# seobbro/TTA-depth-completion

Measured on AMD Instinct MI355X. Metric: TTA frames/sec (fwd+loss+bwd+Adam) at 352x1216, higher is better.
Workload: dtype mixed: real frames' forward (the scored depth) f32 storage + bf16x3 MFMA arithmetic; no_grad proxy pass and all data gradients bf16 storage + single bf16 MFMA; fp32 accumulate everywhere; loss / Adam / adapted parameters fp32 (include/ptta.h PTTA_DTYPE_MIXED)

## Files before the change

include/ptta.h:

```cpp
#ifndef PTTA_H
#define PTTA_H
#include <stdint.h>
#ifdef __cplusplus
extern "C" {
#endif

typedef struct ptta_ctx* ptta_handle;
typedef void* ptta_stream;

enum { PTTA_BACKBONE_MSG_CHN = 0, PTTA_BACKBONE_NLSPN = 1, PTTA_BACKBONE_COSTDCNET = 2 };
enum { PTTA_DTYPE_F32 = 0, PTTA_DTYPE_MIXED = 1,
       PTTA_MIXED_KEEP_PROXY = 0x100, PTTA_MIXED_KEEP_BACKWARD = 0x200, PTTA_MIXED_KEEP_HEADS = 0x400,
       PTTA_MIXED_BWD_ROUNDED_W = 0x800 };
enum { PTTA_META_1LAYER = 0, PTTA_META_2LAYERS = 1, PTTA_META_NONE = 2 };
enum { PTTA_NLSPN_LEGACY_OFFSET = 0x100,
       PTTA_NLSPN_SYNCBN_ADAPT = 0x200,
       PTTA_SYNCBN_ADAPT = 0x200,
       PTTA_ADAPT_META_ONLY = 0x400 };

typedef struct {
    float lr, beta1, beta2, eps, weight_decay;
    float w_sparse_depth, w_smoothness, w_cos;
    float max_input_depth;
    float max_predict_depth;
// ... 47 lines not shown
              const float* validity, float* depth_out, float* loss_info_out, ptta_stream s);

int ptta_outlier_removal(const float* sparse_depth, const float* validity, float* sparse_out, float* validity_out,
                         int n, int height, int width, int kernel_size, float threshold, float* scratch, ptta_stream s);

int ptta_eval_metrics(const float* depth, const float* ground_truth, int64_t numel, float min_evaluate_depth,
                      float max_evaluate_depth, void* scratch, float* metrics_out, ptta_stream s);

int ptta_mdconv_forward(const float* input, const float* weight, const float* bias, const float* offset, const float* mask,
                        float* output, int b, int c, int h, int w, int c_out, int kh, int kw, int sh, int sw, int ph, int pw,
                        int dh, int dw, int group, int deformable_group, ptta_stream s);
int ptta_mdconv_backward(const float* input, const float* weight, const float* bias, const float* offset, const float* mask,
                         const float* grad_output, float* grad_input, float* grad_offset, float* grad_mask, float* grad_weight,
                         float* grad_bias, int b, int c, int h, int w, int c_out, int kh, int kw, int sh, int sw, int ph, int pw,
                         int dh, int dw, int group, int deformable_group, ptta_stream s);

int ptta_set_image_norm(ptta_handle h, float divisor, const float* mean, const float* stdv);

int ptta_head_bind(ptta_handle h, const char* name, float* param, float* exp_avg, float* exp_avg_sq);
int ptta_head_set_hparams(ptta_handle h, float lr, float beta1, float beta2, float eps, float weight_decay, float tau,
                          int adam_step, ptta_stream s);
int ptta_head_reload(ptta_handle h, ptta_stream s);
int ptta_head_forward(ptta_handle h, const float* image, const float* sparse_depth, int reverse, float* emb_out, float* ref_out,
                      ptta_stream s);
int ptta_head_backward(ptta_handle h, float* loss_out, ptta_stream s);
int ptta_head_adam_step(ptta_handle h, ptta_stream s);
int ptta_head_step(ptta_handle h, const float* image, const float* sparse_depth, int reverse, float* loss_out, ptta_stream s);
int ptta_head_get_grad(ptta_handle h, const char* name, float* dst, int64_t capacity, int* has_grad_host, ptta_stream s);

enum { PTTA_HEAD_FORM_PLAIN = 0, PTTA_HEAD_FORM_SYNCBN = 1 };
int ptta_head_set_form(ptta_handle h, int form);

int ptta_crop_flip(const float* src, float* dst, int n, int channels, int height, int width, int crop_height, int crop_width,
                   const int32_t* start_y, const int32_t* start_x, const uint8_t* hflip, const uint8_t* vflip, ptta_stream s);

int ptta_rotate(const float* src, float* dst, int n, int channels, int height, int width, const uint8_t* do_rotate, const float* angle_deg,
                int bilinear, ptta_stream s);
int ptta_resize_crop(const float* src, float* dst, int n, int channels, int height, int width, const uint8_t* do_resize,
                     const int32_t* resize_height, const int32_t* resize_width, const int32_t* start_y, const int32_t* start_x,
                     int bilinear, int scale_depth, ptta_stream s);
int ptta_photometric(const float* src, float* dst, int n, int height, int width, const uint8_t* do_brightness, const float* f_brightness,
                     const uint8_t* do_contrast, const float* f_contrast, const uint8_t* do_saturation, const float* f_saturation,
                     double* scratch, ptta_stream s);

int ptta_photometric_full(const float* src, float* dst, int n, int height, int width, const uint8_t* do_brightness, const float* f_brightness,
                          const uint8_t* do_contrast, const float* f_contrast, const uint8_t* do_gamma, const float* f_gamma,
                          const uint8_t* do_hue, const float* f_hue, const uint8_t* do_saturation, const float* f_saturation,
                          double* scratch, ptta_stream s);
int ptta_add_noise(const float* src, const float* noise, float* dst, int n, int channels, int height, int width, const uint8_t* do_noise,
                   float spread, int uniform, ptta_stream s);
int ptta_remove_patches(const float* src, float* dst, int n, int channels, int height, int width, const uint8_t* do_remove,
                        const uint8_t* selected, const int32_t* patch_height, const int32_t* patch_width, ptta_stream s);
int ptta_crop_pad(const float* src, float* dst, int n, int channels, int height, int width, const uint8_t* do_crop_pad,
                  const int32_t* start_y, const int32_t* start_x, const int32_t* end_y, const int32_t* end_x,
                  const int32_t* pad_top, const int32_t* pad_left, int padding_mode, float fill, ptta_stream s);
int ptta_resize_pad(const float* src, float* dst, int n, int channels, int height, int width, const uint8_t* do_resize_pad,
                    const int32_t* resize_height, const int32_t* resize_width, const int32_t* pad_top, const int32_t* pad_left,
                    int bilinear, int padding_mode, float fill, ptta_stream s);

typedef int (*ptta_allreduce_fn)(void* user, double* exchange_buf, long long count, ptta_stream s);
int ptta_set_stat_sync(ptta_handle h, ptta_allreduce_fn fn, void* user, double* exchange_buf, int64_t capacity, int world_size);

int ptta_rccl_unique_id(void* id128_host);
int ptta_rccl_comm_create(const void* id128_host, int rank, int world_size, void** comm_out_host);
int ptta_rccl_comm_destroy(void* comm);
int ptta_rccl_allreduce_mean_f32(void* comm, float* buf, int64_t count, ptta_stream s);
const char* ptta_rccl_last_error(void);
int ptta_set_stat_sync_rccl(ptta_handle h, void* comm, double* exchange_buf, int64_t capacity, int world_size);
int ptta_set_grad_sync_rccl(ptta_handle h, void* comm);

int ptta_set_graph(ptta_handle h, int enable);

int ptta_set_option(ptta_handle h, const char* key, int value);
int ptta_get_option(ptta_handle h, const char* key, int* value_host);

int ptta_profile(ptta_handle h, int enable);
int ptta_profile_read(ptta_handle h, int klass, double* ms_total_host, double* alg_bytes_host, double* macs_host,
                      int64_t* launches_host, ptta_stream s);

int ptta_debug_tensor(ptta_handle h, const char* name, float* dst, int64_t capacity, int64_t* numel_host, ptta_stream s);
int ptta_op_conv32(const float* in_nhwc, const float* weight, const float* bias, float* out_nhwc,
                   int b, int hin, int win, int mode, int relu_in, int in_major, int flip, int dtype, int naive,
                   ptta_stream s);
int ptta_op_gwgrad(const float* x_nhwc, const float* gy_nhwc, float* gw, float* gb, int b, int h, int w, int ci, int co, int impl,
                   int reps, float* us_per_call_host, ptta_stream s);
#define PTTA_GCONV_S1 0
#define PTTA_GCONV_S2 1
#define PTTA_GCONV_T2 2
#define PTTA_GCONV_VERT 1
#define PTTA_GCONV_X1_W2 2
#define PTTA_GCONV_DGRAD 4
#define PTTA_GCONV_AFF_ACT_FIRST 8
#define PTTA_GCONV_AFF_RES_PLAIN 16
int ptta_op_gconv(const float* x0, int c0, int ld0, const float* x1, int c1, int ld1, const float* weight, const float* bias, float* y,
                  int co, int ldy, int b, int hin, int win, int hout, int wout, int k, int geom, int act, int accumulate, int impl,
                  int flags, int six_b, int x1_from_b, int stat_npass, double* stat_host, int* form_host, ptta_stream s);
int ptta_op_gconv_affine(const float* x0, int c0, int ld0, const float* x1, int c1, int ld1, const float* weight, const float* bias, float* y,
                         int co, int ldy, int b, int hin, int win, int hout, int wout, int k, int geom, int act, int accumulate, int impl,
                         int flags, int six_b, int x1_from_b, int stat_npass, double* stat_host, int* form_host, const float* scale,
                         const float* shift, const float* res, int ld_res, ptta_stream s);
#define PTTA_GBN_TRAIN 0
#define PTTA_GBN_EVAL 1
#define PTTA_GBN_BACKWARD 2
typedef struct ptta_gbn_view { float* p; int c; int ld; } ptta_gbn_view;
typedef struct ptta_gbn_args {
    int mode, b, h, w, npass, act, act_first, res_relu, acc_gx, acc_gres, world, nblocks_in, repeats;
    float eps, momentum;
    ptta_gbn_view x, res, y, g, gx, gres;
    const float* gamma; const float* beta; const float* part_in;
    float* st; float* rm; float* rv; long long* nbt; float* st_eval; float* dgamma; float* dbeta;
} ptta_gbn_args;
int ptta_op_gbn(const ptta_gbn_args* a, ptta_stream s);
typedef struct ptta_cd_sparse ptta_cd_sparse;
int ptta_cd_sparse_create(ptta_cd_sparse** out, int n, int h, int w);
void ptta_cd_sparse_destroy(ptta_cd_sparse* q);
int ptta_cd_sparse_build(ptta_cd_sparse* q, const float* sparse, float z_step, ptta_stream s);
int ptta_cd_sparse_read(ptta_cd_sparse* q, int level, int* cnt_host, int* coords_host, long long coords_cap, int* vol_host, float* feat_in_host,
                        ptta_stream s);
int ptta_op_cd_sparse_conv(ptta_cd_sparse* q, const float* x, const float* wk, float* y, int lin, int lout, int ksize, int ci, int co, int backward,
                           int acc, ptta_stream s);
typedef struct ptta_cd_sbn_args {
    int mode, level, c, relu, repeats, world, acc_res;
    const float* f; const float* res; const float* y; const float* g; const float* gamma; const float* beta;
    float* rm; float* rv; long long* nbt; float* out; float* st; float* dgamma; float* dbeta; float* gx; float* gres;
} ptta_cd_sbn_args;
int ptta_op_cd_sbn(ptta_cd_sparse* q, const ptta_cd_sbn_args* a, ptta_stream s);
int ptta_op_cd_densify(ptta_cd_sparse* q, const float* in, float* out, int c, int backward, int ldv, int c0, ptta_stream s);
#define PTTA_CD_PAD_DUAL 0
#define PTTA_CD_CROP_AVG 1
#define PTTA_CD_SCATTER_DUAL_GRAD 2
#define PTTA_CD_STAGE 3
#define PTTA_CD_CLAMP 4
#define PTTA_CD_FUSION_FWD 5
#define PTTA_CD_FUSION_BWD 6
#define PTTA_CD_POOL_FWD 7
#define PTTA_CD_POOL_BWD 8
#define PTTA_CD_UP_FWD 9
#define PTTA_CD_UP_BWD 10
#define PTTA_CD_REGRESS_FWD 11
#define PTTA_CD_REGRESS_BWD 12
#define PTTA_CD_ROWS_FWD 13
#define PTTA_CD_ROWS_BWD 14
int ptta_op_cd_dense(int op, const float* a, const float* b, float* out, float* out2, const int* d, const float* f, ptta_stream s);
int ptta_op_conv32_chain(const float* in_nhwc, const float* weight, const float* bias, float* buf_a, float* buf_b, const float* aux,
                         int b, int h, int w, int relu_in, int epi_flags, int reps, int replays, float* us_per_launch_host, ptta_stream s);
#define PTTA_ABI_VERSION 2
int ptta_version(void);

#ifdef __cplusplus
}
#endif
#endif
```

tta-depth-completion_amd/csrc/conv32.hip:

```cpp
#include <cstdlib>
#include <cstring>
#include "ptta_common.h"
#include "ptta_kernels.h"

template <typename T>
struct Conv32P {
    const T* in; int in_nb;
    const void* wpack;
    const void* wpack2;
    Epi<T> epi;
    int B, Hin, Win, Hout, Wout;
};

template <typename T> struct Frag;
template <> struct Frag<float> { typedef float4 A; };
template <> struct Frag<bf16_t> { typedef uint4 A; };

__device__ __forceinline__ float4 relu4(float4 v) {
    v.x = fmaxf(v.x, 0.f); v.y = fmaxf(v.y, 0.f); v.z = fmaxf(v.z, 0.f); v.w = fmaxf(v.w, 0.f);
    return v;
}
__device__ __forceinline__ unsigned relu_bf2(unsigned v) {
    unsigned neg = (v >> 15) & 0x00010001u;
    return v & ~(neg * 0xffffu);
}
__device__ __forceinline__ uint4 relu8(uint4 v) {
    v.x = relu_bf2(v.x); v.y = relu_bf2(v.y); v.z = relu_bf2(v.z); v.w = relu_bf2(v.w);
    return v;
}

template <typename T, int MODE, bool RELU, bool UP, bool MASK, bool ADD>
__global__ __launch_bounds__(256) void conv32_mfma_kernel(Conv32P<T> p) {
    constexpr bool F32 = sizeof(T) == 4;
    constexpr int NA = F32 ? 4 : 2;
    typedef typename Frag<T>::A AF;
    const int lane = threadIdx.x & 63;
    const int i = lane & 31, h = lane >> 5;
    const float biasv = epi_bias(p.epi, i);
    const int wave = __builtin_amdgcn_readfirstlane((int)(threadIdx.x >> 6));

    AF w[9][NA];
    {
        const AF* wp = (const AF*)p.wpack;
#pragma unroll
        for (int t = 0; t < 9; ++t)
#pragma unroll
            for (int g = 0; g < NA; ++g) w[t][g] = wp[(t * NA + g) * 64 + lane];
    }

    const int Wt = (MODE == CONV_T2) ? p.Win : p.Wout;
    const int nseg = (Wt + 31) >> 5;
    const int npar = (MODE == CONV_T2) ? 2 : 1;
    const long nitems = (long)p.B * nseg * npar * p.Hout;
    const float sy = up_scale(p.Hout >> 1, p.Hout), sx = up_scale(p.Wout >> 1, p.Wout);

    for (long item = (long)blockIdx.x * 4 + wave; item < nitems; item += (long)gridDim.x * 4) {
        long t_ = item;
        const int y = (int)(t_ % p.Hout); t_ /= p.Hout;
        int xpar = 0;
        if (MODE == CONV_T2) { xpar = (int)(t_ & 1); t_ >>= 1; }
        const int seg = (int)(t_ % nseg);
        const int b = (int)(t_ / nseg);
        const int x0 = seg << 5;
        const bool lane_in = (x0 + i) < Wt;
        const T* inb = p.in + (size_t)(b % p.in_nb) * p.Hin * p.Win * 32;

        f32x16 acc;
#pragma unroll
        for (int r = 0; r < 16; ++r) acc[r] = 0.f;

#pragma unroll
        for (int tap = 0; tap < 9; ++tap) {
            const int ky = tap / 3, kx = tap % 3;
            bool active = true;
            int yi, xi;
            if (MODE == CONV_S1) { yi = y + ky - 1; xi = x0 + i + kx - 1; }
            else if (MODE == CONV_S2) { yi = 2 * y + ky - 1; xi = 2 * (x0 + i) + kx - 1; }
            else {
                const int ty = y + 1 - ky, tx = xpar + 1 - kx;
                active = ((ty & 1) == 0) && ((tx & 1) == 0);
                yi = ty >> 1; xi = x0 + i + (tx >> 1);
            }
            active = active && (yi >= 0) && (yi < p.Hin);
            if (!active) continue;
            const bool ok = lane_in && (xi >= 0) && (xi < p.Win);
            const T* src = inb + ((size_t)yi * p.Win + (ok ? xi : 0)) * 32;
            AF a[NA];
#pragma unroll
            for (int g = 0; g < NA; ++g) {
                if (F32) {
                    float4 v = make_float4(0.f, 0.f, 0.f, 0.f);
                    if (ok) v = *(const float4*)((const float*)src + 8 * g + 4 * h);
                    if (RELU) v = relu4(v);
                    a[g] = *(AF*)&v;
                } else {
                    uint4 v = make_uint4(0, 0, 0, 0);
                    if (ok) v = *(const uint4*)((const bf16_t*)src + 16 * g + 8 * h);
                    if (RELU) v = relu8(v);
                    a[g] = *(AF*)&v;
                }
            }
#pragma unroll
            for (int g = 0; g < NA; ++g) {
                if (F32) {
                    const float4 av = *(float4*)&a[g];
                    const float4 wv = *(float4*)&w[tap][g];
                    acc = __builtin_amdgcn_mfma_f32_32x32x2f32(av.x, wv.x, acc, 0, 0, 0);
                    acc = __builtin_amdgcn_mfma_f32_32x32x2f32(av.y, wv.y, acc, 0, 0, 0);
                    acc = __builtin_amdgcn_mfma_f32_32x32x2f32(av.z, wv.z, acc, 0, 0, 0);
                    acc = __builtin_amdgcn_mfma_f32_32x32x2f32(av.w, wv.w, acc, 0, 0, 0);
                } else {
                    acc = __builtin_amdgcn_mfma_f32_32x32x16_bf16(__builtin_bit_cast(bf16x8, a[g]),
                                                                  __builtin_bit_cast(bf16x8, w[tap][g]),
                                                                  acc, 0, 0, 0);
                }
            }
        }

        epi_tile<T, UP, MASK, ADD>(p.epi, b, y, p.Hout, p.Wout, i, acc, x0, h, Wt, MODE == CONV_T2 ? 2 : 1, xpar, sy, sx, nullptr, 0, 0, &biasv);
    }
}


#define X3_TH 8
#define X3_PW 34
#define X3_PH 10

typedef __bf16 bf16x2_t __attribute__((ext_vector_type(2)));
typedef float float2_t __attribute__((ext_vector_type(2)));
typedef short short2_t __attribute__((ext_vector_type(2)));

__device__ __forceinline__ void split2(float a, float b, unsigned& hi, unsigned& lo) {
    float2_t v = {a, b};
    const bf16x2_t h = __builtin_convertvector(v, bf16x2_t);
    hi = __builtin_bit_cast(unsigned, h);
    float2_t r = {a - __uint_as_float(hi << 16), b - __uint_as_float(hi & 0xffff0000u)};
    lo = __builtin_bit_cast(unsigned, __builtin_convertvector(r, bf16x2_t));
}
__device__ __forceinline__ unsigned relu_pk(unsigned v) {
    const short2_t z = {0, 0};
    return __builtin_bit_cast(unsigned, __builtin_elementwise_max(__builtin_bit_cast(short2_t, v), z));
}

template <typename T> struct Px;
template <> struct Px<float> { float4 a, b; };
template <> struct Px<bf16_t> { uint4 a; };
template <typename T> __device__ __forceinline__ Px<T> px_zero();
template <> __device__ __forceinline__ Px<float> px_zero<float>() { Px<float> r; r.a = make_float4(0.f, 0.f, 0.f, 0.f); r.b = r.a; return r; }
template <> __device__ __forceinline__ Px<bf16_t> px_zero<bf16_t>() { Px<bf16_t> r; r.a = make_uint4(0u, 0u, 0u, 0u); return r; }
__device__ __forceinline__ Px<float> px_load(const float* src) { Px<float> r; r.a = *(const float4*)src; r.b = *(const float4*)(src + 4); return r; }
__device__ __forceinline__ Px<bf16_t> px_load(const bf16_t* src) { Px<bf16_t> r; r.a = *(const uint4*)src; return r; }
template <bool RELU>
__device__ __forceinline__ void px_stage(const Px<float>& v, unsigned char* dst, int lo_off) {
    float4 a0 = v.a, a1 = v.b;
#ifdef X3_TIMING_NOSPLIT
    *(float4*)dst = a0; *(float4*)(dst + lo_off) = a1; return;
#endif
    if (RELU) { a0 = relu4(a0); a1 = relu4(a1); }
    uint4 hi, lo;
    split2(a0.x, a0.y, hi.x, lo.x); split2(a0.z, a0.w, hi.y, lo.y);
    split2(a1.x, a1.y, hi.z, lo.z); split2(a1.z, a1.w, hi.w, lo.w);
    *(uint4*)dst = hi;
    *(uint4*)(dst + lo_off) = lo;
}
template <bool RELU>
__device__ __forceinline__ void px_stage(const Px<bf16_t>& v, unsigned char* dst, int) {
    uint4 hi = v.a;
    if (RELU) { hi.x = relu_pk(hi.x); hi.y = relu_pk(hi.y); hi.z = relu_pk(hi.z); hi.w = relu_pk(hi.w); }
    *(uint4*)dst = hi;
}
template <typename T> struct Geo;
template <> struct Geo<float> { static constexpr int STR = 144, LO = 64, WL = 18 * 64 * 16, UPPX = 128, UPPC = 8; };
template <> struct Geo<bf16_t> { static constexpr int STR = 80, LO = 0, WL = 0, UPPX = 64, UPPC = 4; };

__device__ __forceinline__ int x3_stage_pix(int idx) { return ((idx >> 5) << 3) + (((idx >> 2) & 1) << 2) + ((idx >> 3) & 3); }

template <typename T, bool W2 = false>
__device__ __forceinline__ void mma_step(f32x16& acc, const unsigned char* a, const uint4& wh, const unsigned char* wl) {
    const bf16x8 ah = __builtin_bit_cast(bf16x8, *(const uint4*)a);
    const bf16x8 bh = __builtin_bit_cast(bf16x8, wh);
    if constexpr (sizeof(T) == 2 && W2) {
        const bf16x8 bl = __builtin_bit_cast(bf16x8, *(const uint4*)wl);
        acc = __builtin_amdgcn_mfma_f32_32x32x16_bf16(ah, bl, acc, 0, 0, 0);
    }
    if constexpr (sizeof(T) == 4) {
        const bf16x8 al = __builtin_bit_cast(bf16x8, *(const uint4*)(a + Geo<T>::LO));
        const bf16x8 bl = __builtin_bit_cast(bf16x8, *(const uint4*)wl);
        acc = __builtin_amdgcn_mfma_f32_32x32x16_bf16(al, bh, acc, 0, 0, 0);
        acc = __builtin_amdgcn_mfma_f32_32x32x16_bf16(ah, bl, acc, 0, 0, 0);
    }
    acc = __builtin_amdgcn_mfma_f32_32x32x16_bf16(ah, bh, acc, 0, 0, 0);
}
template <typename T, bool W2 = false>
__device__ __forceinline__ void load_weights(uint4 (&wh)[9][2], unsigned char* wl_lds, const void* wpack, const void* wpack2, int tid, int lane) {
    const uint4* ph = (const uint4*)wpack;
#pragma unroll
    for (int t = 0; t < 9; ++t)
#pragma unroll
        for (int k = 0; k < 2; ++k) wh[t][k] = ph[(t * 2 + k) * 64 + lane];
    if constexpr (sizeof(T) == 4 || W2) {
        const uint4* pl = (const uint4*)wpack2;
        for (int idx = tid; idx < 18 * 64; idx += 256) *(uint4*)(wl_lds + idx * 16) = pl[idx];
    }
}

template <typename T, bool W2> struct FragSet { uint4 ah, al, bl; };
template <typename T, bool W2>
__device__ __forceinline__ void frag_load(FragSet<T, W2>& f, const unsigned char* a, const unsigned char* wl) {
    f.ah = *(const uint4*)a;
    if constexpr (sizeof(T) == 4) { f.al = *(const uint4*)(a + Geo<T>::LO); f.bl = *(const uint4*)wl; }
    else if constexpr (W2) f.bl = *(const uint4*)wl;
}
template <typename T, bool W2>
__device__ __forceinline__ void frag_mma(f32x16& acc, const FragSet<T, W2>& f, const uint4& wh) {
    const bf16x8 ah = __builtin_bit_cast(bf16x8, f.ah), bh = __builtin_bit_cast(bf16x8, wh);
    if constexpr (sizeof(T) == 2 && W2) acc = __builtin_amdgcn_mfma_f32_32x32x16_bf16(ah, __builtin_bit_cast(bf16x8, f.bl), acc, 0, 0, 0);
    if constexpr (sizeof(T) == 4) {
        acc = __builtin_amdgcn_mfma_f32_32x32x16_bf16(__builtin_bit_cast(bf16x8, f.al), bh, acc, 0, 0, 0);
        acc = __builtin_amdgcn_mfma_f32_32x32x16_bf16(ah, __builtin_bit_cast(bf16x8, f.bl), acc, 0, 0, 0);
    }
    acc = __builtin_amdgcn_mfma_f32_32x32x16_bf16(ah, bh, acc, 0, 0, 0);
}

template <typename T, int UPH, int UPW>
__device__ __forceinline__ void up_window_dma(const T* ub, int Hu, int Wu, int uy0, int ux0, unsigned char* up_lds, int tid, int wave) {
    constexpr int PC = Geo<T>::UPPC, N = UPH * UPW * PC;
#pragma unroll
    for (int k = 0; k < (N + 255) / 256; ++k) {
        const int idx = tid + 256 * k;
        if (idx < N) {
            const int q = idx % PC, pix = idx / PC;
            const int r = pix / UPW, cc = pix - r * UPW;
            const int gy = min(uy0 + r, Hu - 1), gx = min(ux0 + cc, Wu - 1);
            __builtin_amdgcn_global_load_lds((const __attribute__((address_space(1))) void*)(ub + ((size_t)gy * Wu + gx) * 32 + (32 / PC) * q),
                                             (__attribute__((address_space(3))) void*)(up_lds + (size_t)(256 * k + 64 * wave) * 16), 16, 0, 0);
        }
    }
}

#define X3STAMP(v) do { if constexpr (TIMING) { unsigned long long t_; asm volatile("s_memtime %0\n\ts_waitcnt lgkmcnt(0)" : "=s"(t_) :: "memory"); v = t_; } } while (0)
template <typename T, bool RELU, bool UP, bool MASK, bool ADD, bool W2 = false, bool TIMING = false>
__global__ __launch_bounds__(256, 2) void conv32_s1_x3_kernel(Conv32P<T> p) {
    unsigned long long T0 = 0, ta = 0, tb = 0, tc = 0, td = 0, te = 0, tf = 0, tg = 0, th = 0;
    unsigned long long dWait = 0, dSplit = 0, dIssue = 0, dBar1 = 0, dMfma = 0, dEpi = 0, dBar2 = 0, dPro = 0;
    int ntl = 0;
    X3STAMP(T0);
    constexpr int STR = Geo<T>::STR, WL = (sizeof(T) == 4 || W2) ? 18 * 64 * 16 : 0;
    constexpr int UPH = 6, UPW = 18;
    __shared__ __attribute__((aligned(16))) unsigned char lds[X3_PH * X3_PW * STR + WL + (UP ? UPH * UPW * Geo<T>::UPPX : 0)];
    unsigned char* const wl_lds = lds + X3_PH * X3_PW * STR;
    unsigned char* const up_lds = wl_lds + WL;
    const int tid = threadIdx.x, lane = tid & 63;
    const int i = lane & 31, h = lane >> 5;
    const float biasv = epi_bias(p.epi, i);
    const int wave = __builtin_amdgcn_readfirstlane(tid >> 6);
    const int H = p.Hout, W = p.Wout;
    const int ntx = (W + 31) >> 5, nty = (H + X3_TH - 1) / X3_TH;
    const long ntiles = (long)p.B * ntx * nty;
// ... 1070 lines not shown
```

tta-depth-completion_amd/csrc/msgchn_backward.hip:

```cpp
#include "msgchn_ctx.h"

using namespace msgchn;

namespace msgchn {

static int meta2_backward(ptta_ctx* c, hipStream_t s) {
    auto& m2 = c->m2;
    ptta_ctx::Adapted* A = c->adapted.data();
    const int H4 = c->H4, W4 = c->W4, Nn = c->Nn;
    const long P = (long)Nn * H4 * W4;
    if (m2.generic) {
        const int npass = 2;
        GView x; x.p = (float*)c->c2; x.B = Nn; x.H = H4; x.W = W4; x.C = 32; x.ld = 32;
        GView hv = x; hv.p = m2.gh; hv.C = 128; hv.ld = 128;
        GView av = hv; av.p = m2.ga1;
        GView tv = x; tv.p = m2.gt;
        GView gm = x; gm.p = c->nar_bwd ? c->dm_f32 : (float*)c->dm_total;
        GView dt = x; dt.p = m2.gdt;
        GView da1 = hv; da1.p = m2.gda1;
        GView dh = hv; dh.p = m2.gdh;
        RUN(ptta_launch_gbn_backward(tv, gm, tv, dt, GView(), npass, GACT_NONE, 0, 0, 0, A[5].p, m2.gst2, m2.gpart, m2.gbw, A[5].g, A[6].g, s, 0, &c->stat_sync));
        RUN(ptta_launch_gwgrad_mfma(av, dt, m2.wgp, A[3].g, A[4].g, s));
        GX3Args a;
        a.x0 = dt.p; a.C0 = 32; a.ld0 = 32; a.B = Nn; a.H = H4; a.W = W4;
// ... 26 lines not shown

int heads_backward(ptta_ctx* c, const float* gref, hipStream_t s) {
    const double esh = (c->nar_heads && heads_v2_on(c)) ? 2.0 : 4.0;
    ProfScope ps_(c, 6, s, (double)c->Rg * 32 * (c->nar_bwd ? 2 : 4) + ((double)c->Rg * (1024 + 512) + 16384.0 + 262144.0) * esh,
                  (double)c->Rg * (16384.0 + 262144.0), 3);
    const Lin& l0 = c->fc["proj.0"]; const Lin& l3 = c->fc["proj.3"]; BNorm& bn = c->bn["proj.1"];
    const int R = (int)c->Rg;
    if (c->nar_heads && heads_v2_on(c)) {
        HnGemmArgs g; g.epi = 3; g.R = R; g.W = l3.Wtsl;
        if (c->cos_in_gemm) { g.pro = 4; g.A = c->emb_n; g.Bref = c->ref_n; g.rowstats = c->loss_ws + ptta_loss_ws_rows_off(c->N); g.coef = c->loss_ws; }
        else { g.pro = 5; g.Af = gref; }
        g.X = c->feat; g.x_bf16 = 0; g.W0 = l0.Whi; g.W0t = l0.Wthi; g.b0 = l0.bias;
        g.escale = bn.scale; g.eshift = bn.shift; g.emean = bn.mean; g.einv = bn.inv; g.part = c->bn_part; g.P = c->headP;
        RUN(ptta_launch_hn_gemm(g, s));
        const int nb = ptta_hn_row_blocks(R);
        RUN(ptta_stat_sync(&c->stat_sync, c->bn_part, nb, 512, 1, s));
        RUN(ptta_launch_bn_bwd_finalize(c->bn_part, nb, R * (c->stat_sync.world > 1 ? c->stat_sync.world : 1), 512, bn.gamma, bn.inv, c->bnb_gscale, c->bnb_c1, c->bnb_c2, s,
                                        nullptr, nullptr, c->head_k12, l0.bias, bn.mean));
        RUN(ptta_launch_head_bwd_finish(c->head_k12, l0.W, c->headP, (const float*)c->feat, R, c->g_feat, s, 1, c->nar_bwd ? 1 : 0));
        return 0;
    }
    if (heads_v2_on(c)) {
        GemmArgs g; g.A = gref; g.W = l3.Wt; g.R = R; g.K = 512; g.N = 512; g.epi = 3;
        if (c->cos_in_gemm) {
            g.A = c->emb; g.Bref = c->ref; g.rowstats = c->loss_ws + ptta_loss_ws_rows_off(c->N); g.coef = c->loss_ws; g.pro = 4;
        }
        g.escale = bn.scale; g.eshift = bn.shift; g.emean = bn.mean; g.einv = bn.inv; g.part = c->bn_part;
        g.x3 = 1; g.Whi = l3.Wthi; g.Wlo = l3.Wtlo; g.Wil = l3.Wtil;
        g.X = (const float*)c->feat; g.b0 = l0.bias; g.W0hi = l0.Whi; g.W0lo = l0.Wlo; g.W0thi = l0.Wthi; g.W0tlo = l0.Wtlo; g.P = c->headP;
        RUN(ptta_launch_gemm(g, s));
        RUN(ptta_stat_sync(&c->stat_sync, c->bn_part, ptta_gemm_part_blocks(g), 512, 1, s));
        RUN(ptta_launch_bn_bwd_finalize(c->bn_part, ptta_gemm_part_blocks(g), R * (c->stat_sync.world > 1 ? c->stat_sync.world : 1), 512, bn.gamma, bn.inv, c->bnb_gscale, c->bnb_c1, c->bnb_c2, s,
                                        nullptr, nullptr, c->head_k12, l0.bias, bn.mean));
        RUN(ptta_launch_head_bwd_finish(c->head_k12, l0.W, c->headP, (const float*)c->feat, R, c->nar_bwd ? c->g_feat_f32 : (float*)c->g_feat, s));
        if (c->nar_bwd) RUN(to_narrow(c, c->g_feat_f32, c->g_feat, c->Rg * 32, s));
        return 0;
    }
    GemmArgs g; g.A = gref; g.W = l3.Wt; g.C = c->gmask; g.R = R; g.K = 512; g.N = 512; g.epi = 2;
    g.eH = c->h1; g.escale = bn.scale; g.eshift = bn.shift; g.emean = bn.mean; g.einv = bn.inv; g.part = c->bn_part;
    g.x3 = c->x3; g.Whi = l3.Wthi; g.Wlo = l3.Wtlo; g.Wil = l3.Wtil;
    RUN(ptta_launch_gemm(g, s));
    RUN(ptta_stat_sync(&c->stat_sync, c->bn_part, ptta_gemm_part_blocks(g), 512, 1, s));
    RUN(ptta_launch_bn_bwd_finalize(c->bn_part, ptta_gemm_part_blocks(g), R * (c->stat_sync.world > 1 ? c->stat_sync.world : 1), 512, bn.gamma, bn.inv, c->bnb_gscale, c->bnb_c1, c->bnb_c2, s));
    GemmArgs g2; g2.A = c->gmask; g2.A2 = c->h1; g2.W = l0.Wt; g2.C = (c->bf16 || c->nar_bwd) ? c->g_feat_f32 : (float*)c->g_feat; g2.R = R; g2.K = 512; g2.N = 32; g2.pro = 2;
    g2.pscale = c->bnb_gscale; g2.pmean = bn.mean; g2.pinv = bn.inv; g2.pc1 = c->bnb_c1; g2.pc2 = c->bnb_c2;
    g2.x3 = c->x3; g2.Whi = l0.Wthi; g2.Wlo = l0.Wtlo;
    RUN(ptta_launch_gemm(g2, s));
    if (c->bf16 || c->nar_bwd) from_f32_launch(c->g_feat_f32, (bf16_t*)c->g_feat, c->Rg * 32, s);
    return 0;
}

int backbone_backward(ptta_ctx* c, const float* g_net, hipStream_t s, bool join_aux) {
    const int Nn = c->Nn, B2 = 2 * Nn;
    const int nbf = c->nar_bwd ? 1 : c->bf16;
    const int H1 = c->Hp, W1 = c->Wp, H2 = c->H2, W2 = c->W2, H4 = c->H4, W4 = c->W4, H8 = c->H8, W8 = c->W8;
    auto out1_args = [&](const std::string& layer, const float* g, const void* mask, void* out, int H, int W) {
        const LOut& lo = c->lout[layer];
        ConvInArgs a; a.cin = 1; a.pl[0].p = g; a.pl[0].nb = Nn; a.pl[0].bstride = (long)H * W;
        a.wfrag = lo.bfrag; a.wcanon = lo.bcanon; a.mask = mask; a.mask_nb = B2; a.out_raw = out;
        a.B = Nn; a.H = H; a.W = W; a.bf16 = c->nar_bwd ? 1 : c->bf16; a.naive = c->naive;
        return a;
    };
    auto dgrad_out1 = [&](const std::string& layer, const float* g, const void* mask, void* out, int H, int W) -> int {
        ConvInArgs a = out1_args(layer, g, mask, out, H, W);
        return conv_in_p(c, a, s);
    };
    auto head_bwd = [&](const std::string& l3, const std::string& l1, const float* g, const void* v, void* dv, int H, int W, const E& e) -> int {
        ConvInArgs a = out1_args(l3, g, v, dv, H, W);
        return conv32_first_bwd(c, s, l1, a, Nn, H, W, e);
    };
    auto dgrad_in_ch1 = [&](const std::string& layer, const void* g, const float* add, float* out, int H, int W) -> int {
        const LIn& li = c->lin_in[layer];
        ConvOut1Args a; a.in = g; a.in_nb = Nn; a.w = li.bw; a.add = add; a.add_nb = Nn; a.out = out;
        a.B = Nn; a.H = H; a.W = W; a.relu_in = 0; a.bf16 = c->nar_bwd ? 1 : c->bf16;
        return conv_out1_p(c, a, s);
    };
    auto em = [](void* raw, const void* mask, int mask_nb) { E e; e.raw = raw; e.mask = mask; e.mask_nb = mask_nb; return e; };
    RUN(head_bwd("depth_decoder3.prdct.3", "depth_decoder3.prdct.1", g_net, c->v3, c->dv3, H1, W1, em(c->ds0_3, c->s0_3, Nn)));
    CV("depth_decoder3.dec1.3", true, CONV_S1, c->ds0_3, Nn, Nn, H1, W1, false, em(c->du3, c->u3, Nn));
    CV("depth_decoder3.dec1.1", true, CONV_S2, c->du3, Nn, Nn, H1, W1, false, em(c->ds1_3, c->s1_3, Nn));
    CV("depth_decoder3.dec2.3", true, CONV_S1, c->ds1_3, Nn, Nn, H2, W2, false, em(c->dt3, c->t3, Nn));
    if (join_aux) HIPCHK(hipStreamWaitEvent(s, c->ev_join, 0));
    { E e; e.raw = c->dw2; e.mask = c->w2; e.mask_nb = B2; e.sum = c->dfeat_tot; e.add1 = c->g_feat; e.add1_nb = Nn;
      CV("depth_decoder3.dec2.1", true, CONV_S2, c->dt3, Nn, Nn, H2, W2, false, e); }
    hipStream_t sd = join_aux ? c->aux(s) : nullptr;
    if (!sd) sd = s;
    CV("depth_encoder3.enc2.3", true, CONV_S1, c->dfeat_tot, Nn, Nn, H4, W4, false, em(c->de3_2a, c->e3_2a, B2));
    { E e; e.sum = c->de3_1; e.mask = c->e3_1; e.mask_nb = B2; e.add1 = c->ds1_3; e.add1_nb = Nn;
      CV("depth_encoder3.enc2.1", true, CONV_T2, c->de3_2a, Nn, Nn, H4, W4, false, e); }
    CV("depth_encoder3.enc1.3", true, CONV_S1, c->de3_1, Nn, Nn, H2, W2, false, em(c->de3_1a, c->e3_1a, B2));
    { E e; e.sum = c->de3_0; e.mask = c->e3_0; e.mask_nb = B2; e.add1 = c->ds0_3; e.add1_nb = Nn;
      CV("depth_encoder3.enc1.1", true, CONV_T2, c->de3_1a, Nn, Nn, H2, W2, false, e); }
    if (sd != s) { HIPCHK(hipEventRecord(c->ev_side[0], s)); HIPCHK(hipStreamWaitEvent(sd, c->ev_side[0], 0)); }
    REST_(sd, ptta_launch_up2T_32(c->de3_0, nullptr, c->up4_t, Nn, H2, W2, nbf, sd));
    REST_(sd, ptta_launch_up2T_32(c->de3_1, nullptr, c->up3_t, Nn, H4, W4, nbf, sd));
    REST_(sd, ptta_launch_up2T_32(c->dfeat_tot, nullptr, c->dz2_up, Nn, H8, W8, nbf, sd));
    if (sd != s) HIPCHK(hipEventRecord(c->ev_side[3], sd));
    if (c->loss_report.on) {
        REST_(sd, ptta_launch_loss_depth_part(final_depth(c), c->loss_report.image, c->loss_report.sparse, c->loss_report.validity, c->hp.max_input_depth,
                                              c->N, c->H, c->W, c->loss_ws, sd));
        REST_(sd, ptta_launch_loss_finalize(c->loss_ws, c->N, c->H, c->W, c->Rg, 1, c->hyper + 5, c->loss_info_dst ? c->loss_info_dst : c->loss_info, sd));
        HIPCHK(hipEventRecord(c->ev_loss, sd));
    }
    CV("depth_encoder3.init.2", true, CONV_S1, c->de3_0, Nn, Nn, H1, W1, false, em(c->de3_0a, c->e3_0a, B2));
    RUN(dgrad_in_ch1("depth_encoder3.init.0", c->de3_0a, g_net, c->dp11, H1, W1));
    REST_(s, ptta_launch_up2T_1ch(c->dp11, c->dq, Nn, H2, W2, s));
    if (sd != s) HIPCHK(hipStreamWaitEvent(s, c->ev_side[3], 0));
    { E e = em(c->ds0_2, c->s0_2, B2); e.sum = c->dz4; e.add1 = c->up4_t; e.add1_nb = Nn;
      RUN(head_bwd("depth_decoder2.prdct.3", "depth_decoder2.prdct.1", c->dq, c->v2, c->dv2, H2, W2, e)); }
    CV("depth_decoder2.dec1.3", true, CONV_S1, c->dz4, Nn, Nn, H2, W2, false, em(c->du2, c->u2, B2));
    { E e = em(c->ds1_2, c->s1_2, B2); e.sum = c->dz3; e.add1 = c->up3_t; e.add1_nb = Nn;
      CV("depth_decoder2.dec1.1", true, CONV_S2, c->du2, Nn, Nn, H2, W2, false, e); }
    CV("depth_decoder2.dec2.3", true, CONV_S1, c->dz3, Nn, Nn, H4, W4, false, em(c->dt2, c->t2, B2));
    { E e; e.sum = c->dz2; e.mask = c->z2; e.mask_nb = B2; e.add1 = c->dz2_up; e.add1_nb = Nn;
      CV("depth_decoder2.dec2.1", true, CONV_S2, c->dt2, Nn, Nn, H4, W4, false, e); }
    CV("depth_encoder2.enc2.3", true, CONV_S1, c->dz2, Nn, Nn, H8, W8, false, em(c->de2_2a, c->e2_2a, B2));
    { E e; e.sum = c->de2_1; e.mask = c->e2_1; e.mask_nb = B2; e.add1 = c->ds1_2; e.add1_nb = Nn;
      CV("depth_encoder2.enc2.1", true, CONV_T2, c->de2_2a, Nn, Nn, H8, W8, false, e); }
    CV("depth_encoder2.enc1.3", true, CONV_S1, c->de2_1, Nn, Nn, H4, W4, false, em(c->de2_1a, c->e2_1a, B2));
    { E e; e.sum = c->de2_0; e.mask = c->e2_0; e.mask_nb = B2; e.add1 = c->ds0_2; e.add1_nb = Nn;
      CV("depth_encoder2.enc1.1", true, CONV_T2, c->de2_1a, Nn, Nn, H4, W4, false, e); }
    CV("depth_encoder2.init.2", true, CONV_S1, c->de2_0, Nn, Nn, H2, W2, false, em(c->de2_0a, c->e2_0a, B2));
    RUN(dgrad_in_ch1("depth_encoder2.init.0", c->de2_0a, c->dq, c->dp12, H2, W2));
    REST_(s, ptta_launch_up2T_1ch(c->dp12, c->dout1, Nn, H4, W4, s));
    RUN(dgrad_out1("depth_decoder1.prdct.3", c->dout1, c->v1, c->dv1, H4, W4));
    { E e; e.sum = c->dm_total; e.mask = c->s0_1; e.mask_nb = B2; e.add1 = c->dw2; e.add1_nb = Nn; e.add2 = c->ds1_2; e.add2_nb = Nn;
      CV("depth_decoder1.prdct.1", true, CONV_S1, c->dv1, Nn, Nn, H4, W4, false, e); }
    if (sd != s && c->loss_report.on) HIPCHK(hipStreamWaitEvent(s, c->ev_loss, 0));
    if (c->nar_bwd && c->meta_mode == PTTA_META_2LAYERS) RUN(to_wide(c, c->dm_total, c->dm_f32, (long)Nn * H4 * W4 * 32, s));
    if (c->meta_mode == PTTA_META_2LAYERS) return meta2_backward(c, s);
    if (!c->bf16 && c->x3 && !c->naive) {
        GView xv; xv.p = (float*)c->c2; xv.B = Nn; xv.H = H4; xv.W = W4; xv.C = 32; xv.ld = 32;
        GView gv; gv.p = (float*)c->dm_total; gv.B = Nn; gv.H = H4; gv.W = W4; gv.C = 32; gv.ld = 32;
        GwAdam ga;
        const bool fuse = c->adam_fuse_req && c->adam_in_wgrad && !c->grad_comm && c->adapted.size() == 2 && c->adapted[0].p && c->adapted[0].m && c->adapted[0].v &&
                          c->adapted[1].p && c->adapted[1].m && c->adapted[1].v && c->adapted[0].g == c->gW && c->adapted[1].g == c->gB;
        if (fuse) { ga.pw = c->adapted[0].p; ga.mw = c->adapted[0].m; ga.vw = c->adapted[0].v; ga.pb = c->adapted[1].p; ga.mb = c->adapted[1].m; ga.vb = c->adapted[1].v;
                    ga.hyper = c->hyper; ga.step = c->step_dev; ga.ticket = c->adam_ticket; }
        REST_(s, ptta_launch_gwgrad_mfma(xv, gv, c->wgrad_part, c->gW, c->gB, s, c->nar_bwd ? 1 : 0, fuse ? &ga : nullptr));
        c->adam_fused = fuse;
        return 0;
    }
    REST_(s, ptta_launch_wgrad32(c->c2, c->dm_total, c->bf16, Nn, H4, W4, c->wgrad_part, c->gW, c->gB, s));
    return 0;
}

}
```

tta-depth-completion_amd/csrc/msgchn_ctx.h:

```cpp
#pragma once
#include <cstdio>
#include <cstdlib>
#include <cstring>
#include <map>
#include <string>
#include <unordered_map>
#include <vector>

#include "../../include/ptta.h"
#include "ptta_common.h"
#include "ptta_kernels.h"
#include "nlspn.h"

#pragma GCC visibility push(hidden)

#define HIPCHK(x) do { hipError_t e_ = (x); if (e_ != hipSuccess) return c->fail(std::string(#x) + ": " + hipGetErrorString(e_), -100 - (int)e_); } while (0)
#define RUN(x) do { int r_ = (x); if (r_ != 0) return c->fail_chain(std::string(#x) + " failed", r_ < 0 ? r_ : -r_); } while (0)

#define NLFWD(call) do { if (c && c->nl) { c->err.clear(); return (call); } } while (0)

struct ImgNorm { int on; float div; float mean[3]; float stdv[3]; };

namespace msgchn {
hipError_t d2d_copy(void* dst, const void* src, size_t bytes, hipStream_t s);
// ... 11 lines not shown
static constexpr unsigned kStepEvent = hipEventDisableTiming | hipEventDisableSystemFence;
struct L32 { ConvW f{}, b{}; float* bias = nullptr; int transposed = 0; };
struct LIn { float *wfrag = nullptr, *wcanon = nullptr, *bias = nullptr, *bw = nullptr; int cin = 1; };
struct LOut { float *w = nullptr, *bias = nullptr, *bfrag = nullptr, *bcanon = nullptr; };
struct Lin { float *W = nullptr, *Wt = nullptr, *bias = nullptr; bf16_t *Whi = nullptr, *Wlo = nullptr, *Wthi = nullptr, *Wtlo = nullptr, *Wil = nullptr, *Wtil = nullptr;
             bf16_t *Wsl = nullptr, *Wtsl = nullptr;
             int N = 0, K = 0; };
struct BNorm { float *gamma = nullptr, *beta = nullptr, *rm = nullptr, *rv = nullptr; long long* nbt = nullptr;
               float *mean = nullptr, *inv = nullptr, *scale = nullptr, *shift = nullptr; };
struct Dbg { const void* p; long numel; int is_act; };

struct PrefixBufs {
    void *c0 = nullptr, *c1 = nullptr, *c2 = nullptr, *c3 = nullptr, *c4 = nullptr, *e1_0a = nullptr, *e1_0 = nullptr, *e1_1a = nullptr;
    void *c0a = nullptr, *c1a = nullptr, *c2a = nullptr, *c3a = nullptr, *c4a = nullptr;
    void *e1_1 = nullptr, *y1 = nullptr, *e1_2a = nullptr, *y2 = nullptr, *t1 = nullptr, *y3 = nullptr, *s1_1 = nullptr, *u1 = nullptr;
    float *dclamp = nullptr, *d12 = nullptr, *d14 = nullptr, *in_image = nullptr, *in_loss_image = nullptr, *in_sparse = nullptr, *in_validity = nullptr;
    bool proxy_valid = false;
};

struct ptta_ctx : PrefixBufs {
    GNet* nl = nullptr;
    int N = 1, H = 0, W = 0, Hp = 0, Wp = 0, pt = 0, pr = 0, dual = 0, Nn = 1;
    int bf16 = 0, naive = 0, es = 4, x3 = 1;
    int mixed = 0;
    int nar_proxy = 0, nar_bwd = 0, nar_heads = 0;
    std::unordered_map<const void*, void*> ntwin;
    void* tw(const void* p) const { auto it = ntwin.find(p); return it == ntwin.end() ? nullptr : it->second; }
    void twin_alloc(const void* p, int nb, int h, int w) { if (nar_proxy && p) ntwin[p] = dalloc((size_t)nb * h * w * 32 * 2); }
    float *dm_f32 = nullptr;
    ptta_hparams hp{};
    std::string err;
    std::vector<void*> allocs;
    std::map<std::string, L32> l32;
    std::map<std::string, LIn> lin_in;
    std::map<std::string, LOut> lout;
    std::map<std::string, Lin> fc;
    std::map<std::string, BNorm> bn;
    std::map<std::string, Dbg> dbg;
    int meta_mode = 0;
    struct Adapted { std::string name; long n = 0; float *p = nullptr, *m = nullptr, *v = nullptr, *g = nullptr; };
    std::vector<Adapted> adapted;
    struct HeadT { bool ready = false; std::vector<Adapted> prm, tgt; bool has_grad[12] = {};
                   float *hyper = nullptr, *tau2 = nullptr, *loss = nullptr, *loss_part = nullptr, *wpart = nullptr, *bpart = nullptr, *dp = nullptr;
                   float *sv_mean = nullptr, *sv_inv = nullptr, *sv_scale = nullptr, *sv_shift = nullptr;
                   int* step = nullptr; unsigned* ticket = nullptr; PttaAdamEntry *tab = nullptr, *etab = nullptr;
                   std::vector<PttaAdamEntry> tab_host, etab_host; int tab_n = 0; long tab_total = 0, etab_total = 0; int tab_mode = -1; bool etab_dirty = true;
                   int reverse = 1; bool fwd_ok = false, bwd_ok = false;
                   float* garena = nullptr; long garena_n = 0;
                   int form = 0; bool stepped = false; } head;
    int skip_dec3 = 0;
    int head_swap = 0;
    float *meta_w = nullptr, *meta_b = nullptr;
    float *gW = nullptr, *gB = nullptr;
    struct Meta2 {
        ConvW w1f[4], w2f[4], w2b[4];
        void *h[4] = {}, *a1[4] = {}, *t = nullptr, *dt = nullptr, *da1 = nullptr, *dh = nullptr;
        float *st1 = nullptr, *st2 = nullptr;
        float *rm1 = nullptr, *rv1 = nullptr, *rm2 = nullptr, *rv2 = nullptr; long long *nbt1 = nullptr, *nbt2 = nullptr;
        float *cs_part = nullptr, *bw = nullptr;
        bool generic = false;
        float *gh = nullptr, *ga1 = nullptr, *gt = nullptr, *gdt = nullptr, *gda1 = nullptr, *gdh = nullptr;
        float *w1c = nullptr, *w2c = nullptr, *w2bc = nullptr;
        bf16_t *w1hi = nullptr, *w1lo = nullptr, *w2hi = nullptr, *w2lo = nullptr, *w2bhi = nullptr, *w2blo = nullptr;
        float *gst1 = nullptr, *gst2 = nullptr, *part1 = nullptr, *part2 = nullptr, *gbw = nullptr, *gpart = nullptr, *wgp = nullptr;
    } m2;
    float* hyper = nullptr;
    float* w3_tmp = nullptr;
    int* step_dev = nullptr; float* stamp_f = nullptr; unsigned long long* stamp_base = nullptr; int stamps = 0;
    void stamp(int i, hipStream_t s) { if (stamps) msgchn::stamp_launch(stamp_f, stamp_base, i, s); }
    PttaAdamEntry* adam_tab = nullptr; unsigned* adam_ticket = nullptr; bool adam_tab_dirty = true;
    std::vector<PttaAdamEntry> adam_host;
    bool fwd_valid = false;
    PttaStatSync stat_sync;
    Lin fused_pp; bool fused_pp_valid = false; int fuse_heads = 1;
    int heads_v2 = 1;
    int thru = 1; bool thru_active = false;
    int adam_in_wgrad = 1; bool adam_fuse_req = false, adam_fused = false;
    int bwd_w2 = 1;
    const float *cnt_sparse = nullptr, *cnt_validity = nullptr;
    struct { const float *image = nullptr, *sparse = nullptr, *validity = nullptr; bool on = false; } loss_report;
    hipEvent_t ev_loss = nullptr;
    hipEvent_t ev_dpart = nullptr;
    int fuse_first = 1, fuse_head_bwd = 1;
    int cos_grad_fused = 1;
    bool cos_in_gemm = false;
    void* w0frag = nullptr; float *hm_part = nullptr, *headP = nullptr; double* head_k12 = nullptr;
    struct ProfClass { std::vector<std::pair<hipEvent_t, hipEvent_t>> ev; size_t used = 0; double bytes = 0, macs = 0; long launches = 0; };
    bool prof_on = false;
    static constexpr int NPROF = 9;
    ProfClass prof[NPROF];
    std::vector<std::pair<int, size_t>> prof_seq;
    int use_graph = 0;
    void* grad_comm = nullptr;
    float* grad_arena = nullptr; long grad_arena_n = 0;
    int pre_sync_graph = -1, pre_sync_aux = -1;
    hipGraphExec_t gexec[4] = {nullptr, nullptr, nullptr, nullptr};
    hipGraph_t graph[4] = {nullptr, nullptr, nullptr, nullptr};
    hipStream_t cap_stream = nullptr;
    struct PreSet : PrefixBufs {
        bool prepared = false, rest_recorded = false;
        uint64_t prep_token = 0;
        uint64_t last_token = 0;
    };
    PreSet pset[2];
    int cur_set = 0, pipe_cur = 0, pipe_last = 0;
    bool pipe_ready = false, pipe_active = false, skip_prefix = false;
    const float *fb_image = nullptr, *fb_sparse = nullptr;
    hipStream_t pre_stream = nullptr;
    hipEvent_t ev_prefix[2] = {nullptr, nullptr}, ev_rest[2] = {nullptr, nullptr}, ev_entry = nullptr;
    hipStream_t pipe_stream = nullptr; bool pipe_stream_set = false;
    hipGraph_t pgraph[2] = {nullptr, nullptr}, rgraph[4][2] = {{nullptr, nullptr}, {nullptr, nullptr}, {nullptr, nullptr}, {nullptr, nullptr}};
    hipGraphExec_t pexec[2] = {nullptr, nullptr}, rexec[4][2] = {{nullptr, nullptr}, {nullptr, nullptr}, {nullptr, nullptr}, {nullptr, nullptr}};
    int use_aux = 1;
    hipStream_t aux_stream = nullptr;
    hipEvent_t ev_fork = nullptr, ev_join = nullptr, ev_real = nullptr;
    hipEvent_t ev_side[4] = {nullptr, nullptr, nullptr, nullptr};
    hipStream_t aux(hipStream_t caller) {
        if (!use_aux) return nullptr;
        if (!aux_stream) {
            if (hipStreamCreateWithFlags(&aux_stream, hipStreamNonBlocking) != hipSuccess) return nullptr;
            if (hipEventCreateWithFlags(&ev_fork, kStepEvent) != hipSuccess ||
                hipEventCreateWithFlags(&ev_join, kStepEvent) != hipSuccess ||
                hipEventCreateWithFlags(&ev_real, kStepEvent) != hipSuccess ||
                hipEventCreateWithFlags(&ev_side[0], kStepEvent) != hipSuccess || hipEventCreateWithFlags(&ev_side[1], kStepEvent) != hipSuccess ||
                hipEventCreateWithFlags(&ev_side[2], kStepEvent) != hipSuccess || hipEventCreateWithFlags(&ev_side[3], kStepEvent) != hipSuccess) { (void)hipStreamDestroy(aux_stream); aux_stream = nullptr; return nullptr; }
        }
        return prof_on ? caller : aux_stream;
    }
    hipEvent_t ev_replay = nullptr;
    void drop_graphs() {
        if (ev_replay) (void)hipEventSynchronize(ev_replay);
        if (pre_stream) (void)hipStreamSynchronize(pre_stream);
        for (int k = 0; k < 4; ++k) {
            if (gexec[k]) { (void)hipGraphExecDestroy(gexec[k]); gexec[k] = nullptr; }
            if (graph[k]) { (void)hipGraphDestroy(graph[k]); graph[k] = nullptr; }
            for (int p = 0; p < 2; ++p) {
                if (rexec[k][p]) { (void)hipGraphExecDestroy(rexec[k][p]); rexec[k][p] = nullptr; }
                if (rgraph[k][p]) { (void)hipGraphDestroy(rgraph[k][p]); rgraph[k][p] = nullptr; }
            }
        }
        for (int p = 0; p < 2; ++p) {
            if (pexec[p]) { (void)hipGraphExecDestroy(pexec[p]); pexec[p] = nullptr; }
            if (pgraph[p]) { (void)hipGraphDestroy(pgraph[p]); pgraph[p] = nullptr; }
            pset[p].prepared = false; pset[p].prep_token = pset[p].last_token = 0;
        }
        fb_image = fb_sparse = nullptr;
    }

    int err_code = 0;
    int fail(const std::string& m, int code) { err = m; err_code = code; return code; }
    int fail_chain(const std::string& m, int code) { err = (err_code == code && !err.empty() && err.size() < 600) ? m + " <- " + err : m; err_code = code; return code; }

    bool oom = false;
    void* dalloc(size_t bytes) {
        void* p = nullptr;
        if (hipMalloc(&p, bytes ? bytes : 16) != hipSuccess) { oom = true; return nullptr; }
        allocs.push_back(p);
        if (hipMemset(p, 0, bytes ? bytes : 16) != hipSuccess) { oom = true; return nullptr; }
        return p;
    }
    float* falloc(size_t n) { return (float*)dalloc(n * sizeof(float)); }
    void* act(const char* name, int nb, int h, int w) {
        void* p = dalloc((size_t)nb * h * w * 32 * es);
        dbg[name] = Dbg{p, (long)nb * h * w * 32, 1};
        if (nar_proxy && nb == 2 * Nn) twin_alloc(p, Nn, h, w);
        return p;
    }
    void* gact(const char* name, int nb, int h, int w) {
        const int e = nar_bwd ? 2 : es;
        void* p = dalloc((size_t)nb * h * w * 32 * e);
        dbg[name] = Dbg{p, (long)nb * h * w * 32, nar_bwd ? 2 : 1};
        return p;
    }
    int mask_bits_on = 1;
    std::unordered_map<const void*, uint32_t*> mbits;
    void mask_plane(const void* map, int nb, int h, int w) {
        if (bf16 || naive) return;
        if (mbits.count(map)) return;
        mbits[map] = (uint32_t*)dalloc((size_t)nb * h * w * sizeof(uint32_t));
    }
    uint32_t* bits_of(const void* map) const {
        if (!map || !mask_bits_on) return nullptr;
        auto it = mbits.find(map);
        return it == mbits.end() ? nullptr : it->second;
    }
    float* map1(const char* name, int nb, int h, int w) {
        float* p = falloc((size_t)nb * h * w);
        dbg[name] = Dbg{p, (long)nb * h * w, 0};
        return p;
    }

    int H2, W2, H4, W4, H8, W8, H16, W16;
    long Rg = 0;
    float *img_pad = nullptr, *sp_pad = nullptr, *zero_plane = nullptr;
    ImgNorm img_norm = ImgNorm{0, 1.f, {0.f, 0.f, 0.f}, {1.f, 1.f, 1.f}};
    float *out1, *p12, *q, *p11, *depth_net, *depth_final, *validity_tmp;
    void *m, *y4, *s0_1, *v1;
    void *e2_0a, *e2_0, *e2_1a, *e2_1, *e2_2a, *z2, *t2, *z3, *s1_2, *u2, *z4, *s0_2, *v2;
    void *e3_0a, *e3_0, *e3_1a, *e3_1, *e3_2a, *feat, *w2, *t3, *s1_3, *u3, *s0_3, *v3;
    float *h1z, *pz, *h2, *emb, *h1, *ref, *gref_buf, *gmask, *bn_part;
    double* hn_msc = nullptr;
    float* hn_rs = nullptr;
    bool cos_rows_done = false;
    bf16_t *emb_n = nullptr, *ref_n = nullptr, *h2_n = nullptr;
    float *bnb_gscale, *bnb_c1, *bnb_c2;
    float *loss_ws, *loss_info, *g_final, *g_net;
    float* loss_info_dst = nullptr;
    void *dv3, *ds0_3, *du3, *ds1_3, *dt3, *dw2, *dfeat_tot, *dz2_up, *de3_2a, *de3_1, *de3_1a, *de3_0, *de3_0a;
    void *up4_t, *up3_t, *dv2, *ds0_2, *dz4, *du2, *ds1_2, *dz3, *dt2, *dz2, *de2_2a, *de2_1, *de2_1a, *de2_0, *de2_0a, *dv1, *dm_total, *g_feat;
    float *dp11, *dq, *dp12, *dout1, *g_feat_f32;
    float* wgrad_part;
};

struct ProfScope {
    ptta_ctx::ProfClass* pc = nullptr; hipStream_t s;
    ProfScope(ptta_ctx* c, int klass, hipStream_t s_, double bytes, double macs, int launches) : s(s_) {
        if (!c->prof_on) return;
        pc = &c->prof[klass];
        if (pc->used == pc->ev.size()) {
            hipEvent_t e0, e1;
            if (hipEventCreate(&e0) != hipSuccess || hipEventCreate(&e1) != hipSuccess) { pc = nullptr; return; }
            pc->ev.push_back({e0, e1});
        }
        pc->bytes += bytes; pc->macs += macs; pc->launches += launches;
        c->prof_seq.push_back({klass, pc->used});
        (void)hipEventRecord(pc->ev[pc->used].first, s);
    }
    ~ProfScope() { if (pc) { (void)hipEventRecord(pc->ev[pc->used].second, s); pc->used++; } }
};
#define REST_(s_, call) do { ProfScope ps_(c, 8, (s_), 0, 0, 1); RUN(call); } while (0)
#define CV(...) RUN(conv32(c, s, __VA_ARGS__))

struct E { const void* up = nullptr; int up_nb = 1; const void* mask = nullptr; int mask_nb = 1;
           const void* add1 = nullptr; int add1_nb = 1; const void* add2 = nullptr; int add2_nb = 1;
           void* raw = nullptr; void* sum = nullptr;
           bool nar = false; };

inline float* st_ptr(float* base, int C, int pass, int kind) { return base + ((size_t)pass * 4 + kind) * C; }

namespace msgchn {
int pad16(int n);
void build_registry(ptta_ctx* c);
void build_workspace(ptta_ctx* c);
int load_weight(ptta_ctx* c, const std::string& name, const void* tensor, const int64_t* shape, int ndim, hipStream_t s);
int conv_in_p(ptta_ctx* c, const ConvInArgs& a_, hipStream_t s);
int conv_out1_p(ptta_ctx* c, const ConvOut1Args& a, hipStream_t s);
int conv32(ptta_ctx* c, hipStream_t s, const std::string& layer, bool bwd, int mode, const void* in, int in_nb,
           int B, int Hin, int Win, bool relu, const E& e);
int conv32w(ptta_ctx* c, hipStream_t s, const ConvW* w, const float* bias, const void* in, int in_nb, int B, int H, int W, const E& e);
int conv32_first_bwd(ptta_ctx* c, hipStream_t s, const std::string& layer, ConvInArgs& f, int B, int H, int W, const E& e);
int to_narrow(ptta_ctx* c, const void* src_f32, void* dst, long n, hipStream_t s);
int to_wide(ptta_ctx* c, const void* src_nar, float* dst, long n, hipStream_t s);
int rgb_encoder(ptta_ctx* c, const float* image, int nb, int boff, int zero_from_b, hipStream_t s);
int ensure_fused_heads(ptta_ctx* c, hipStream_t s);
int ensure_proxy_rgb(ptta_ctx* c, const float* any_image, hipStream_t s);
int enc1_head_fn(ptta_ctx* c, hipStream_t st);
int stage1_independent(ptta_ctx* c, int B2, hipStream_t s);
bool heads_v2_on(const ptta_ctx* c);
int heads_forward(ptta_ctx* c, hipStream_t s, int part = 0);
int push_hparams(ptta_ctx* c, hipStream_t s);
int forward_common(ptta_ctx* c, const float* image, const float* sparse, bool train, hipStream_t s);
const float* final_depth(ptta_ctx* c);
int heads_backward(ptta_ctx* c, const float* gref, hipStream_t s);
int backbone_backward(ptta_ctx* c, const float* g_net, hipStream_t s, bool join_aux);
void pipe_use(ptta_ctx* c, int p);
void pipe_overwritten(ptta_ctx* c, int p);
int pipe_quiesce(ptta_ctx* c);
int ensure_adam_table(ptta_ctx* c, hipStream_t s);
}
#pragma GCC visibility pop
```

tta-depth-completion_amd/csrc/msgchn_forward.hip:

```cpp
#include "msgchn_ctx.h"

using namespace msgchn;

namespace msgchn {

int conv_in_p(ptta_ctx* c, const ConvInArgs& a_, hipStream_t s) {
    ConvInArgs a = a_;
    const double px = (double)a.B * a.H * a.W;
    ProfScope ps(c, 7, s, px * (a.cin * 4 + 32 * (a.bf16 ? 2 : c->es)) + 9.0 * a.cin * 32 * 4, px * 9.0 * a.cin * 32, 1);
    if (!c->mbits.empty()) {
        if (!a.mask_bits) a.mask_bits = c->bits_of(a.mask);
        if (!a.bf16 && !a.a_bits) { a.a_bits = c->bits_of(a.out_raw); a.a_bits_nb = c->Nn; }
    }
    return ptta_launch_conv_in(a, s);
}
int conv_out1_p(ptta_ctx* c, const ConvOut1Args& a, hipStream_t s) {
    const double px = (double)a.B * a.H * a.W;
    ProfScope ps(c, 7, s, px * (32 * (a.bf16 ? 2 : c->es) + 4) + 288 * 4, px * 288.0, 1);
    return ptta_launch_conv_out1(a, s);
}

int conv32(ptta_ctx* c, hipStream_t s, const std::string& layer, bool bwd, int mode, const void* in, int in_nb,
           int B, int Hin, int Win, bool relu, const E& e) {
    auto it = c->l32.find(layer);
    if (it == c->l32.end()) return c->fail("unknown 32->32 layer " + layer, -2);
    Conv32Args a;
    a.in = in; a.in_nb = in_nb; a.w = bwd ? &it->second.b : &it->second.f;
    a.bias = bwd ? nullptr : (layer == "conv1_rgb_meta" ? c->meta_b : it->second.bias);
    a.up = e.up; a.up_nb = e.up_nb; a.mask = e.mask; a.mask_nb = e.mask_nb;
    a.add1 = e.add1; a.add1_nb = e.add1_nb; a.add2 = e.add2; a.add2_nb = e.add2_nb;
    a.out_raw = e.raw; a.out_sum = e.sum;
    const bool nar = e.nar || (bwd && c->nar_bwd);
    const int es_l = nar ? 2 : c->es;
    a.B = B; a.Hin = Hin; a.Win = Win; a.mode = mode; a.relu_in = relu ? 1 : 0; a.bf16 = nar ? 1 : c->bf16; a.naive = c->naive; a.x3 = c->x3;
    a.w2 = (bwd && c->nar_bwd && c->bwd_w2) ? 1 : 0;
    if (!c->mbits.empty()) {
        a.mask_bits = c->bits_of(e.mask);
        if (!bwd && !nar) {
            uint32_t* bs = c->bits_of(e.sum); uint32_t* br = c->bits_of(e.raw);
            if (bs && br) return c->fail("conv32: both outputs of " + layer + " are registered masks", -22);
            if (bs || br) { a.bits_out = bs ? bs : br; a.bits_sum = bs ? 1 : 0; a.bits_nb = c->Nn; }
        }
    }
    const long pin = (long)B * Hin * Win;
    const long pout = mode == CONV_S1 ? pin : (mode == CONV_S2 ? pin / 4 : pin * 4);
    const bool small = (long)Hin * Win <= (long)c->H4 * c->W4 * (mode == CONV_S2 ? 4 : 1);
#ifdef PTTA_EXP_SKIP_PAIRED_S1
    if (mode == CONV_S1 && small && layer.size() > 2 && layer.compare(layer.size() - 2, 2, ".3") == 0 && layer.find("prdct") == std::string::npos) return 0;
#endif
    ProfScope ps(c, (mode == CONV_S1 ? (relu ? 0 : 2) : 4) + (small ? 1 : 0), s, (double)((pin + pout) * 32 + 9216) * es_l,
                 (double)(mode == CONV_T2 ? pin : pout) * 9.0 * 32.0 * 32.0, 1);
    return ptta_launch_conv32(a, s);
}

int conv32w(ptta_ctx* c, hipStream_t s, const ConvW* w, const float* bias, const void* in, int in_nb, int B, int H, int W, const E& e) {
    Conv32Args a;
    a.in = in; a.in_nb = in_nb; a.w = w; a.bias = bias;
    a.add1 = e.add1; a.add1_nb = e.add1_nb; a.out_raw = e.raw; a.out_sum = e.sum;
    a.B = B; a.Hin = H; a.Win = W; a.mode = CONV_S1; a.relu_in = 0; a.bf16 = c->bf16; a.naive = c->naive; a.x3 = c->x3;
    return ptta_launch_conv32(a, s);
}

static int conv32_first(ptta_ctx* c, hipStream_t s, const std::string& layer, ConvInArgs& f, int a_nb, int B, int H, int W, const E& e) {
    auto it = c->l32.find(layer);
    if (it == c->l32.end()) return c->fail("unknown 32->32 layer " + layer, -2);
    const long tiles = (long)B * ((W + 31) / 32) * ((H + 7) / 8);
    const bool nar = e.nar;
    f.bf16 = nar ? 1 : c->bf16;
    if (c->fuse_first >= (f.cin == 3 ? 2 : 1) && !c->bf16 && !c->naive && c->x3 && tiles > 256 && !e.mask && !e.add1 && !e.add2 && !e.sum) {
        Conv32Args a;
        a.in = nullptr; a.in_nb = B; a.w = &it->second.f; a.bias = it->second.bias;
        a.up = e.up; a.up_nb = e.up_nb; a.out_raw = e.raw;
        a.B = B; a.Hin = H; a.Win = W; a.mode = CONV_S1; a.relu_in = 1; a.bf16 = nar ? 1 : 0; a.naive = 0; a.x3 = 1;
        const double px = (double)B * H * W;
        const int es_l = nar ? 2 : c->es;
        ProfScope ps(c, 0, s, (px * f.cin + 9.0 * f.cin * 32) * 4 + (px * 96 + 9216) * es_l, px * 9.0 * (f.cin * 32 + 1024), 1);
        f.a_bits = (a_nb > 0 && !nar) ? c->bits_of(f.out_raw) : nullptr;
        if (!c->mbits.empty() && !nar) { uint32_t* br = c->bits_of(e.raw); if (br) { a.bits_out = br; a.bits_nb = c->Nn; } }
        const int rc = ptta_launch_conv32_first(a, f, (a_nb > 0 && !nar && !f.a_bits) ? f.out_raw : nullptr, a_nb, s);
        return rc == 1 ? c->fail("conv32_first: fused form refused a case its caller accepted", -22) : rc;
    }
    RUN(conv_in_p(c, f, s));
    return conv32(c, s, layer, false, CONV_S1, f.out_raw, B, B, H, W, true, e);
}

int conv32_first_bwd(ptta_ctx* c, hipStream_t s, const std::string& layer, ConvInArgs& f, int B, int H, int W, const E& e) {
    auto it = c->l32.find(layer);
    if (it == c->l32.end()) return c->fail("unknown 32->32 layer " + layer, -2);
    const long tiles = (long)B * ((W + 31) / 32) * ((H + 7) / 8);
    const bool nar = c->nar_bwd != 0;
    f.bf16 = nar ? 1 : c->bf16;
    if (c->fuse_head_bwd && c->bits_of(f.mask) && c->bits_of(e.mask) && c->fuse_first >= 1 && !c->bf16 && !c->naive && c->x3 && tiles > 256 && e.mask && e.raw && (e.add1 != nullptr) == (e.sum != nullptr) && !e.add2 && !e.up) {
        Conv32Args a;
        a.in = nullptr; a.in_nb = B; a.w = &it->second.b; a.bias = nullptr;
        a.mask = e.mask; a.mask_nb = e.mask_nb; a.out_raw = e.raw; a.add1 = e.add1; a.add1_nb = e.add1_nb; a.out_sum = e.sum;
        a.mask_bits = c->bits_of(e.mask); f.mask_bits = c->bits_of(f.mask);
        a.B = B; a.Hin = H; a.Win = W; a.mode = CONV_S1; a.relu_in = 0; a.bf16 = nar ? 1 : 0; a.naive = 0; a.x3 = 1;
        a.w2 = (nar && c->bwd_w2) ? 1 : 0;
        const double px = (double)B * H * W;
        const int es_l = nar ? 2 : c->es;
        ProfScope ps(c, 2, s, (px + 9.0 * 32) * 4 + (px * 96 + 9216) * es_l, px * 9.0 * (32 + 1024), 1);
        const int rc = ptta_launch_conv32_first(a, f, nullptr, 0, s);
        return rc == 1 ? c->fail("conv32_first_bwd: fused form refused a case its caller accepted", -22) : rc;
    }
    RUN(conv_in_p(c, f, s));
    return conv32(c, s, layer, true, CONV_S1, f.out_raw, B, B, H, W, false, e);
}


static int meta_forward(ptta_ctx* c, bool train, int B, hipStream_t s) {
    const int H4 = c->H4, W4 = c->W4, Nn = c->Nn;
    if (c->meta_mode == PTTA_META_1LAYER) {
        E e; e.raw = c->m;
        if (c->nar_proxy && train && B == 2 * Nn) {
            return conv32(c, s, "conv1_rgb_meta", false, CONV_S1, c->c2, Nn, Nn, H4, W4, false, e);
        }
        return conv32(c, s, "conv1_rgb_meta", false, CONV_S1, c->c2, B, B, H4, W4, false, e);
    }
    auto& m2 = c->m2;
    const ptta_ctx::Adapted* A = c->adapted.data();
    const long P = (long)Nn * H4 * W4;
    const int npass = train ? B / Nn : 1;
    if (m2.generic) {
        if (!train && (!m2.rm1 || !m2.rv1 || !m2.rm2 || !m2.rv2)) return c->fail("meta BatchNorm running statistics not loaded", -3);
        GView x; x.p = (float*)c->c2; x.B = B; x.H = H4; x.W = W4; x.C = 32; x.ld = 32;
        GView hv = x; hv.p = m2.gh; hv.C = 128; hv.ld = 128;
        GView av = hv; av.p = m2.ga1;
        GView tv = x; tv.p = m2.gt;
        GView mv = x; mv.p = (float*)c->m;
        const int tiles_pp = ptta_gconv_x3_tiles(B / npass, H4, W4);
        auto finalize = [&](float* part, int C, const float* gamma, const float* beta, float* rm, float* rv, long long* nbt, float* st) -> int {
            if (!train) return ptta_launch_bn_eval_affine(gamma, beta, rm, rv, 1e-5f, st + 2 * C, st + 3 * C, C, s);
            if (ptta_stat_sync(&c->stat_sync, part, tiles_pp, C, npass, s)) return -5;
            const int wmul = c->stat_sync.world > 1 ? c->stat_sync.world : 1;
            for (int pass = 0; pass < npass; ++pass)
// ... 130 lines not shown
            RUN(to_narrow(c, (const float*)m_.p + half, c->tw(m_.p), half, s));
        }
    }
    c->proxy_valid = true;
    return 0;
}

int enc1_head_fn(ptta_ctx* c, hipStream_t st) {
    const int Nn = c->Nn, H4 = c->H4, W4 = c->W4;
    const LIn& li = c->lin_in["depth_encoder1.init.0"];
    ConvInArgs a; a.cin = 1; a.pl[0].p = c->d14; a.pl[0].nb = Nn; a.pl[0].bstride = (long)H4 * W4;
    a.wfrag = li.wfrag; a.wcanon = li.wcanon; a.bias = li.bias; a.out_raw = c->e1_0a;
    a.B = Nn; a.H = H4; a.W = W4; a.bf16 = c->bf16; a.naive = c->naive;
    RUN(conv_in_p(c, a, st));
    { E e; e.raw = c->e1_0; RUN(conv32(c, st, "depth_encoder1.init.2", false, CONV_S1, c->e1_0a, Nn, Nn, H4, W4, true, e)); }
    { E e; e.raw = c->e1_1a; RUN(conv32(c, st, "depth_encoder1.enc1.1", false, CONV_S2, c->e1_0, Nn, Nn, H4, W4, true, e)); }
    return 0;
}

int stage1_independent(ptta_ctx* c, int B2, hipStream_t s) {
    const int Nn = c->Nn, H4 = c->H4, W4 = c->W4, H8 = c->H8, W8 = c->W8, H16 = c->H16, W16 = c->W16;
    const bool two = c->nar_proxy && B2 == 2 * Nn;
    const int Bf = two ? Nn : B2;
    { E e; e.raw = c->e1_1; e.sum = c->y1; e.add1 = c->c3; e.add1_nb = B2;
      RUN(conv32(c, s, "depth_encoder1.enc1.3", false, CONV_S1, c->e1_1a, Nn, Bf, H8, W8, true, e)); }
    { E e; e.raw = c->e1_2a; RUN(conv32(c, s, "depth_encoder1.enc2.1", false, CONV_S2, c->e1_1, B2, Nn, H8, W8, true, e)); }
    { E e; e.sum = c->y2; e.add1 = c->c4; e.add1_nb = B2;
      RUN(conv32(c, s, "depth_encoder1.enc2.3", false, CONV_S1, c->e1_2a, Nn, Bf, H16, W16, true, e)); }
    { E e; e.raw = c->t1; RUN(conv32(c, s, "depth_decoder1.dec2.1", false, CONV_T2, c->y2, B2, Bf, H16, W16, true, e)); }
    { E e; e.raw = c->y3; e.sum = c->s1_1; e.add1 = c->y1; e.add1_nb = B2;
      RUN(conv32(c, s, "depth_decoder1.dec2.3", false, CONV_S1, c->t1, B2, Bf, H8, W8, true, e)); }
    { E e; e.raw = c->u1; RUN(conv32(c, s, "depth_decoder1.dec1.1", false, CONV_T2, c->s1_1, B2, Bf, H8, W8, true, e)); }
    if (!two) return 0;
    RUN(to_narrow(c, c->e1_0, c->tw(c->e1_0), (long)Nn * H4 * W4 * 32, s));
    RUN(to_narrow(c, c->e1_1a, c->tw(c->e1_1a), (long)Nn * H8 * W8 * 32, s));
    RUN(to_narrow(c, c->e1_2a, c->tw(c->e1_2a), (long)Nn * H16 * W16 * 32, s));
    { E e; e.nar = true; e.sum = c->tw(c->y1); e.add1 = c->tw(c->c3); e.add1_nb = Nn;
      RUN(conv32(c, s, "depth_encoder1.enc1.3", false, CONV_S1, c->tw(c->e1_1a), Nn, Nn, H8, W8, true, e)); }
    { E e; e.nar = true; e.sum = c->tw(c->y2); e.add1 = c->tw(c->c4); e.add1_nb = Nn;
      RUN(conv32(c, s, "depth_encoder1.enc2.3", false, CONV_S1, c->tw(c->e1_2a), Nn, Nn, H16, W16, true, e)); }
    { E e; e.nar = true; e.raw = c->tw(c->t1); RUN(conv32(c, s, "depth_decoder1.dec2.1", false, CONV_T2, c->tw(c->y2), Nn, Nn, H16, W16, true, e)); }
    { E e; e.nar = true; e.raw = c->tw(c->y3); e.sum = c->tw(c->s1_1); e.add1 = c->tw(c->y1); e.add1_nb = Nn;
      RUN(conv32(c, s, "depth_decoder1.dec2.3", false, CONV_S1, c->tw(c->t1), Nn, Nn, H8, W8, true, e)); }
    { E e; e.nar = true; e.raw = c->tw(c->u1); RUN(conv32(c, s, "depth_decoder1.dec1.1", false, CONV_T2, c->tw(c->s1_1), Nn, Nn, H8, W8, true, e)); }
    return 0;
}

static int backbone(ptta_ctx* c, const float* image, bool train, hipStream_t s) {
    hipStream_t s2 = train ? c->aux(s) : nullptr;
    const int Nn = c->Nn, B2 = train ? 2 * Nn : Nn;
    const bool two = train && c->nar_proxy;
    const int H1 = c->Hp, W1 = c->Wp, H2 = c->H2, W2 = c->W2, H4 = c->H4, W4 = c->W4, H8 = c->H8, W8 = c->W8, H16 = c->H16, W16 = c->W16;
    auto e_raw = [](void* raw) { E e; e.raw = raw; return e; };
    if (!c->skip_prefix) RUN(rgb_encoder(c, image, Nn, 0, Nn, s));
    RUN(meta_forward(c, train, B2, s));
    if (!c->skip_prefix) { RUN(enc1_head_fn(c, s)); RUN(stage1_independent(c, B2, s)); }

    auto region = [&](hipStream_t st, int b0, int Bl, bool nar) -> int {
        auto A = [&](void* p_, int h, int w) -> void* { return nar ? c->tw(p_) : (void*)((char*)p_ + (size_t)b0 * h * w * 32 * c->es); };
        auto P1 = [&](float* p_, int h, int w) { return p_ + (size_t)b0 * h * w; };
        auto raw = [&](void* r) { E e; e.raw = r; e.nar = nar; return e; };
        const void* e1_0 = nar ? c->tw(c->e1_0) : c->e1_0;
#define CR(...) RUN(conv32(c, st, __VA_ARGS__))
        { E e; e.nar = nar; e.raw = A(c->y4, H4, W4); e.sum = A(c->s0_1, H4, W4); e.add1 = e1_0; e.add1_nb = Nn; e.add2 = A(c->m, H4, W4); e.add2_nb = Bl;
          CR("depth_decoder1.dec1.3", false, CONV_S1, A(c->u1, H4, W4), Bl, Bl, H4, W4, true, e); }
        CR("depth_decoder1.prdct.1", false, CONV_S1, A(c->s0_1, H4, W4), Bl, Bl, H4, W4, true, raw(A(c->v1, H4, W4)));
        {
            const LOut& lo = c->lout["depth_decoder1.prdct.3"];
            ConvOut1Args a; a.in = A(c->v1, H4, W4); a.in_nb = Bl; a.w = lo.w; a.bias = lo.bias; a.out = P1(c->out1, H4, W4);
            a.B = Bl; a.H = H4; a.W = W4; a.relu_in = 1; a.bf16 = nar ? 1 : c->bf16;
            RUN(conv_out1_p(c, a, st));
        }
        REST_(st, ptta_launch_up2_1ch(P1(c->out1, H4, W4), P1(c->p12, H2, W2), Bl, H4, W4, st));
        {
            const LIn& li = c->lin_in["depth_encoder2.init.0"];
            ConvInArgs a; a.cin = 2;
            a.pl[0].p = c->d12; a.pl[0].nb = Nn; a.pl[0].bstride = (long)H2 * W2;
            a.pl[1].p = P1(c->p12, H2, W2); a.pl[1].nb = Bl; a.pl[1].bstride = (long)H2 * W2;
            a.wfrag = li.wfrag; a.wcanon = li.wcanon; a.bias = li.bias; a.out_raw = A(c->e2_0a, H2, W2);
            a.B = Bl; a.H = H2; a.W = W2; a.bf16 = c->bf16; a.naive = c->naive;
            E e; e.nar = nar; e.raw = A(c->e2_0, H2, W2); e.up = A(c->y4, H4, W4); e.up_nb = Bl;
            RUN(conv32_first(c, st, "depth_encoder2.init.2", a, (b0 == 0 && !nar) ? Nn : 0, Bl, H2, W2, e));
        }
        CR("depth_encoder2.enc1.1", false, CONV_S2, A(c->e2_0, H2, W2), Bl, Bl, H2, W2, true, raw(A(c->e2_1a, H4, W4)));
        { E e; e.nar = nar; e.raw = A(c->e2_1, H4, W4); e.up = A(c->y3, H8, W8); e.up_nb = Bl; CR("depth_encoder2.enc1.3", false, CONV_S1, A(c->e2_1a, H4, W4), Bl, Bl, H4, W4, true, e); }
        CR("depth_encoder2.enc2.1", false, CONV_S2, A(c->e2_1, H4, W4), Bl, Bl, H4, W4, true, raw(A(c->e2_2a, H8, W8)));
        { E e; e.nar = nar; e.sum = A(c->z2, H8, W8); e.up = A(c->y2, H16, W16); e.up_nb = Bl; e.add1 = A(c->c3, H8, W8); e.add1_nb = Bl;
          CR("depth_encoder2.enc2.3", false, CONV_S1, A(c->e2_2a, H8, W8), Bl, Bl, H8, W8, true, e); }
        CR("depth_decoder2.dec2.1", false, CONV_T2, A(c->z2, H8, W8), Bl, Bl, H8, W8, true, raw(A(c->t2, H4, W4)));
        { E e; e.nar = nar; e.raw = A(c->z3, H4, W4); e.sum = A(c->s1_2, H4, W4); e.add1 = A(c->e2_1, H4, W4); e.add1_nb = Bl; e.add2 = A(c->m, H4, W4); e.add2_nb = Bl;
          CR("depth_decoder2.dec2.3", false, CONV_S1, A(c->t2, H4, W4), Bl, Bl, H4, W4, true, e); }
        CR("depth_decoder2.dec1.1", false, CONV_T2, A(c->s1_2, H4, W4), Bl, Bl, H4, W4, true, raw(A(c->u2, H2, W2)));
        { E e; e.nar = nar; e.raw = A(c->z4, H2, W2); e.sum = A(c->s0_2, H2, W2); e.add1 = A(c->e2_0, H2, W2); e.add1_nb = Bl; e.add2 = A(c->c1, H2, W2); e.add2_nb = Bl;
          CR("depth_decoder2.dec1.3", false, CONV_S1, A(c->u2, H2, W2), Bl, Bl, H2, W2, true, e); }
        CR("depth_decoder2.prdct.1", false, CONV_S1, A(c->s0_2, H2, W2), Bl, Bl, H2, W2, true, raw(A(c->v2, H2, W2)));
        {
            const LOut& lo = c->lout["depth_decoder2.prdct.3"];
            ConvOut1Args a; a.in = A(c->v2, H2, W2); a.in_nb = Bl; a.w = lo.w; a.bias = lo.bias; a.add = P1(c->p12, H2, W2); a.add_nb = Bl; a.out = P1(c->q, H2, W2);
            a.B = Bl; a.H = H2; a.W = W2; a.relu_in = 1; a.bf16 = nar ? 1 : c->bf16;
            RUN(conv_out1_p(c, a, st));
        }
        REST_(st, ptta_launch_up2_1ch(P1(c->q, H2, W2), P1(c->p11, H1, W1), Bl, H2, W2, st));
        {
            const LIn& li = c->lin_in["depth_encoder3.init.0"];
            ConvInArgs a; a.cin = 2;
            a.pl[0].p = c->dclamp; a.pl[0].nb = Nn; a.pl[0].bstride = (long)H1 * W1;
            a.pl[1].p = P1(c->p11, H1, W1); a.pl[1].nb = Bl; a.pl[1].bstride = (long)H1 * W1;
            a.wfrag = li.wfrag; a.wcanon = li.wcanon; a.bias = li.bias; a.out_raw = A(c->e3_0a, H1, W1);
            a.B = Bl; a.H = H1; a.W = W1; a.bf16 = c->bf16; a.naive = c->naive;
            E e; e.nar = nar; e.raw = A(c->e3_0, H1, W1); e.up = A(c->z4, H2, W2); e.up_nb = Bl;
            RUN(conv32_first(c, st, "depth_encoder3.init.2", a, (b0 == 0 && !nar) ? Nn : 0, Bl, H1, W1, e));
        }
        CR("depth_encoder3.enc1.1", false, CONV_S2, A(c->e3_0, H1, W1), Bl, Bl, H1, W1, true, raw(A(c->e3_1a, H2, W2)));
        { E e; e.nar = nar; e.raw = A(c->e3_1, H2, W2); e.up = A(c->z3, H4, W4); e.up_nb = Bl; CR("depth_encoder3.enc1.3", false, CONV_S1, A(c->e3_1a, H2, W2), Bl, Bl, H2, W2, true, e); }
        CR("depth_encoder3.enc2.1", false, CONV_S2, A(c->e3_1, H2, W2), Bl, Bl, H2, W2, true, raw(A(c->e3_2a, H4, W4)));
        { E e; e.nar = nar; e.raw = A(c->feat, H4, W4); e.up = A(c->z2, H8, W8); e.up_nb = Bl; e.add1 = A(c->m, H4, W4); e.add1_nb = Bl;
          if (!nar) e.sum = A(c->w2, H4, W4); else e.add1 = nullptr;
          CR("depth_encoder3.enc2.3", false, CONV_S1, A(c->e3_2a, H4, W4), Bl, Bl, H4, W4, true, e); }
#undef CR
        return 0;
    };
    if (two) {
        hipStream_t sp = s2 ? s2 : s;
        if (s2) { HIPCHK(hipEventRecord(c->ev_fork, s)); HIPCHK(hipStreamWaitEvent(s2, c->ev_fork, 0)); }
        c->stamp(3, sp);
        if (s2 && c->thru_active && c->cnt_sparse) REST_(s2, ptta_launch_loss_valid_count(c->cnt_sparse, c->cnt_validity, c->N, c->H, c->W, c->loss_ws, s2));
        RUN(meta_forward_proxy(c, sp));
        c->stamp(1, s);
        RUN(region(s, 0, Nn, false));
        c->stamp(2, s);
        RUN(region(sp, Nn, Nn, true));
        c->stamp(4, sp);
        const bool hn = c->nar_heads && heads_v2_on(c);
        if (!hn) RUN(to_wide(c, c->tw(c->feat), (float*)c->feat + (size_t)c->Rg * 32, c->Rg * 32, sp));
        if (s2) {
            if (hn) RUN(heads_forward(c, s2, 1));
            c->stamp(5, s2);
            HIPCHK(hipEventRecord(c->ev_real, s)); HIPCHK(hipStreamWaitEvent(s2, c->ev_real, 0));
            RUN(heads_forward(c, s2, hn ? 2 : 0));
            c->stamp(6, s2);
            HIPCHK(hipEventRecord(c->ev_join, s2));
        }
    } else {
        RUN(region(s, 0, B2, false));
        if (train && s2) {
            HIPCHK(hipEventRecord(c->ev_fork, s)); HIPCHK(hipStreamWaitEvent(s2, c->ev_fork, 0));
            if (c->thru_active && c->cnt_sparse) REST_(s2, ptta_launch_loss_valid_count(c->cnt_sparse, c->cnt_validity, c->N, c->H, c->W, c->loss_ws, s2));
            RUN(heads_forward(c, s2));
            HIPCHK(hipEventRecord(c->ev_join, s2));
        }
    }
    if (!c->skip_dec3) {
    CV("depth_decoder3.dec2.1", false, CONV_T2, c->w2, B2, Nn, H4, W4, true, e_raw(c->t3));
    { E e; e.sum = c->s1_3; e.add1 = c->e3_1; e.add1_nb = B2; e.add2 = c->c1; e.add2_nb = B2;
      CV("depth_decoder3.dec2.3", false, CONV_S1, c->t3, Nn, Nn, H2, W2, true, e); }
    CV("depth_decoder3.dec1.1", false, CONV_T2, c->s1_3, Nn, Nn, H2, W2, true, e_raw(c->u3));
    { E e; e.sum = c->s0_3; e.add1 = c->e3_0; e.add1_nb = B2; e.add2 = c->c0; e.add2_nb = B2;
      CV("depth_decoder3.dec1.3", false, CONV_S1, c->u3, Nn, Nn, H1, W1, true, e); }
    CV("depth_decoder3.prdct.1", false, CONV_S1, c->s0_3, Nn, Nn, H1, W1, true, e_raw(c->v3));
    {
        const LOut& lo = c->lout["depth_decoder3.prdct.3"];
        ConvOut1Args a; a.in = c->v3; a.in_nb = Nn; a.w = lo.w; a.bias = lo.bias; a.add = c->p11; a.add_nb = B2; a.out = c->depth_net;
        a.B = Nn; a.H = H1; a.W = W1; a.relu_in = 1; a.bf16 = c->bf16;
        RUN(conv_out1_p(c, a, s));
    }
    }
    c->stamp(7, s);
    if (train) {
        if (s2) { if (!c->thru_active) HIPCHK(hipStreamWaitEvent(s, c->ev_join, 0)); }
        else RUN(heads_forward(c, s));
    }
    return 0;
}

bool heads_v2_on(const ptta_ctx* c) {
    return c->heads_v2 && c->fuse_heads && c->fused_pp_valid && c->x3 && !c->bf16 && !c->naive && !c->skip_dec3 && !c->head_swap;
}

static int mlp_forward(ptta_ctx* c, const std::string& name, const void* A, int a_bf16, int K, float* hidden, float* out, hipStream_t s) {
    const Lin& l0 = c->fc[name + ".0"]; const Lin& l3 = c->fc[name + ".3"]; BNorm& bn = c->bn[name + ".1"];
    const int R = (int)c->Rg;
    GemmArgs g; g.A = A; g.a_bf16 = a_bf16; g.W = l0.W; g.bias = l0.bias; g.C = hidden; g.R = R; g.K = K; g.N = 512; g.epi = 1; g.part = c->bn_part;
    g.x3 = c->x3; g.Whi = l0.Whi; g.Wlo = l0.Wlo; g.Wil = l0.Wil;
    RUN(ptta_launch_gemm(g, s));
    RUN(ptta_stat_sync(&c->stat_sync, c->bn_part, ptta_gemm_part_blocks(g), 512, 1, s));
    RUN(ptta_launch_bn_finalize(c->bn_part, ptta_gemm_part_blocks(g), R * (c->stat_sync.world > 1 ? c->stat_sync.world : 1), 512, bn.gamma, bn.beta, 1e-5f, 0.1f, bn.rm, bn.rv, bn.nbt,
                                bn.mean, bn.inv, bn.scale, bn.shift, s));
    GemmArgs g2; g2.A = hidden; g2.W = l3.W; g2.bias = l3.bias; g2.C = out; g2.R = R; g2.K = 512; g2.N = 512; g2.pro = 1;
    g2.pscale = bn.scale; g2.pshift = bn.shift;
    g2.x3 = c->x3; g2.Whi = l3.Whi; g2.Wlo = l3.Wlo; g2.Wil = l3.Wil;
    RUN(ptta_launch_gemm(g2, s));
    return 0;
}

int heads_forward(ptta_ctx* c, hipStream_t s, int part) {
    if (part != 1) c->cos_rows_done = false;
    const double esh = (c->nar_heads && heads_v2_on(c)) ? 2.0 : 4.0;
    ProfScope ps_(c, 6, s, (double)c->Rg * 2 * 32 * 4 + ((double)c->Rg * (2 * 512 + 4 * 1024) + 2 * 16384.0 + 4 * 262144.0) * esh,
                  (double)c->Rg * (2 * 16384.0 + 4 * 262144.0), heads_v2_on(c) ? 7 : 8);
    const size_t half = (size_t)c->Rg * 32 * c->es;
    const void* feat_zero = (const char*)c->feat + half;
// ... 171 lines not shown
```

tta-depth-completion_amd/csrc/msgchn_step.hip:

```cpp
#include "msgchn_ctx.h"

using namespace msgchn;

namespace msgchn {

void pipe_overwritten(ptta_ctx* c, int p) {
    ptta_ctx::PreSet& P = c->pset[p];
    if (c->pipe_cur == p) { P.prepared = false; P.prep_token = 0; }
    P.last_token = 0;
}

static void pipe_save(ptta_ctx* c, ptta_ctx::PreSet& P) { static_cast<PrefixBufs&>(P) = *c; }
void pipe_use(ptta_ctx* c, int p) {
    if (p == c->cur_set) return;
    pipe_save(c, c->pset[c->cur_set]);
    static_cast<PrefixBufs&>(*c) = c->pset[p];
    c->cur_set = p;
}
static int pipe_init(ptta_ctx* c) {
    if (c->pipe_ready) return 0;
    const int Nn = c->Nn, B2 = 2 * Nn, H1 = c->Hp, W1 = c->Wp;
    const size_t es = c->es;
    auto A = [&](int nb, int h, int w) { return c->dalloc((size_t)nb * h * w * 32 * es); };
    pipe_save(c, c->pset[c->cur_set]);
// ... 42 lines not shown
    c->stamp(12, s);
    RUN(enc1_head_fn(c, s));
    RUN(stage1_independent(c, 2 * c->Nn, s));
    c->stamp(13, s);
    return 0;
}
template <class F>
static int pipe_capture(ptta_ctx* c, hipGraph_t* g_out, hipGraphExec_t* e_out, F body) {
    if (!c->cap_stream) HIPCHK(hipStreamCreateWithFlags(&c->cap_stream, hipStreamNonBlocking));
    HIPCHK(hipStreamBeginCapture(c->cap_stream, hipStreamCaptureModeThreadLocal));
    const int rc = body(c->cap_stream);
    hipGraph_t g = nullptr;
    const hipError_t e = hipStreamEndCapture(c->cap_stream, &g);
    if (rc != 0) { if (g) (void)hipGraphDestroy(g); return rc; }
    if (e != hipSuccess || !g) return c->fail(std::string("hipStreamEndCapture: ") + hipGetErrorString(e), -100 - (int)e);
    *g_out = g;
    HIPCHK(hipGraphInstantiate(e_out, g, nullptr, nullptr, 0));
    return 0;
}

}

static int step_tail(ptta_handle c, const float* loss_image, const float* sparse, const float* validity, ptta_stream s_) {
    hipStream_t s = (hipStream_t)s_;
    auto sync_and_adam = [&](bool stamp9) -> int {
        if (c->grad_comm && ptta_rccl_allreduce_mean_f32(c->grad_comm, c->grad_arena, c->grad_arena_n, s_)) return c->fail(std::string("gradient all-reduce: ") + ptta_rccl_last_error(), -5);
        if (stamp9) c->stamp(9, s);
        if (!c->adam_fused) RUN(ptta_adam_step(c, nullptr, nullptr, s_));
        return 0;
    };
    if (c->thru_active) {
        hipStream_t s2 = c->aux(s);
        if (!c->ev_dpart) HIPCHK(hipEventCreateWithFlags(&c->ev_dpart, kStepEvent));
        if (!(c->nar_heads && heads_v2_on(c) && c->cos_rows_done)) REST_(s2, ptta_launch_loss_cos_part(c->emb, c->ref, c->Rg, 512, c->N, c->loss_ws, s2));
        HIPCHK(hipEventRecord(c->ev_dpart, s2));
        REST_(s2, ptta_launch_loss_cos_coef(c->loss_ws, c->N, c->Rg, c->hyper + 5, s2));
        HIPCHK(hipStreamWaitEvent(s, c->ev_dpart, 0));
        if (!c->ev_loss) HIPCHK(hipEventCreateWithFlags(&c->ev_loss, kStepEvent));
        c->loss_report.image = loss_image; c->loss_report.sparse = sparse; c->loss_report.validity = validity; c->loss_report.on = true;
        REST_(s, ptta_launch_loss_backward(final_depth(c), loss_image, sparse, validity, c->hp.max_input_depth, nullptr, nullptr, c->Rg, 512,
                                           c->N, c->H, c->W, c->loss_ws, c->g_final, nullptr, s, c->hyper + 5, nullptr, 1, 1));
        c->cos_in_gemm = true;
        const int rc_h = heads_backward(c, c->gref_buf, s2);
        c->cos_in_gemm = false;
        if (rc_h) return rc_h;
        c->stamp(8, s2);
        HIPCHK(hipEventRecord(c->ev_join, s2));
        const float* g_net = c->g_final;
        if (c->dual) {
            scatter_dual_grad_launch(c->g_final, c->g_net, c->N, c->H, c->W, c->Hp, c->Wp, c->pt, c->pr, s);
            g_net = c->g_net;
        }
        c->adam_fuse_req = true; c->adam_fused = false;
        const int rc_bb = backbone_backward(c, g_net, s, true);
        c->adam_fuse_req = false;
        if (rc_bb) return rc_bb;
        const int rc_a = sync_and_adam(true);
        if (rc_a) return rc_a;
        c->stamp(10, s);
        return 0;
    }
    if (c->nar_heads && heads_v2_on(c)) {
        RUN(ptta_launch_hn_untile(c->emb_n, c->emb, c->Rg, s));
        RUN(ptta_launch_hn_untile(c->ref_n, c->ref, c->Rg, s));
    }
    REST_(s, ptta_launch_loss_forward(final_depth(c), loss_image, sparse, validity, c->hp.max_input_depth, c->emb, c->ref, c->Rg, 512,
                                      c->hyper + 5, c->N, c->H, c->W, c->loss_ws, c->loss_info_dst ? c->loss_info_dst : c->loss_info, s, 1));
    const bool cig = c->cos_grad_fused && heads_v2_on(c) && c->N <= 16;
    REST_(s, ptta_launch_loss_backward(final_depth(c), loss_image, sparse, validity, c->hp.max_input_depth, c->emb, c->ref, c->Rg, 512,
                                       c->N, c->H, c->W, c->loss_ws, c->g_final, cig ? nullptr : c->gref_buf, s, c->hyper + 5, c->loss_info_dst ? c->loss_info_dst : c->loss_info));
    c->cos_in_gemm = cig;
    c->adam_fuse_req = true; c->adam_fused = false;
    const int rc_b = ptta_backward(c, c->g_final, c->gref_buf, nullptr, nullptr, s_);
    c->cos_in_gemm = false; c->adam_fuse_req = false;
    if (rc_b) return rc_b;
    return sync_and_adam(false);
}

static bool thru_ok(ptta_ctx* c, hipStream_t s) {
    return c->thru && c->cos_grad_fused && heads_v2_on(c) && c->N <= 16 && c->aux(s) != nullptr;
}
static int step_body(ptta_handle c, const float* image, const float* loss_image, const float* sparse, const float* validity,
                     ptta_stream s_) {
    RUN(ensure_fused_heads(c, (hipStream_t)s_));
    c->thru_active = thru_ok(c, (hipStream_t)s_);
    c->cnt_sparse = c->thru_active ? sparse : nullptr; c->cnt_validity = validity;
    const int rc = ptta_forward_train(c, image, sparse, nullptr, nullptr, nullptr, s_);
    if (rc) { c->thru_active = false; c->cnt_sparse = nullptr; return rc; }
    const int rc2 = step_tail(c, loss_image, sparse, validity, s_);
    c->thru_active = false; c->cnt_sparse = nullptr; c->loss_report.on = false;
    return rc2;
}

extern "C" {

int ptta_step(ptta_handle c, const float* image, const float* loss_image, const float* sparse, const float* validity,
              float* depth_out, float* loss_info_out, ptta_stream s_) {
    if (c) c->err_code = 0;
    if (!c || !image || !sparse) return -1;
    if (c->nl) return c->nl->step(image, loss_image, sparse, validity, depth_out, loss_info_out, (hipStream_t)s_);
    RUN(pipe_quiesce(c));
    hipStream_t s = (hipStream_t)s_;
    if (!loss_image) loss_image = image;
    const size_t ibytes = (size_t)c->N * 3 * c->H * c->W * 4, pbytes = (size_t)c->N * c->H * c->W * 4;
    if (c->use_graph && !c->prof_on) {
        const int key = (validity ? 2 : 0) | (loss_image != image ? 1 : 0);
        HIPCHK(d2d_copy(c->in_image, image, ibytes, s));
        HIPCHK(d2d_copy(c->in_sparse, sparse, pbytes, s));
        if (key & 1) HIPCHK(d2d_copy(c->in_loss_image, loss_image, ibytes, s));
        if (key & 2) HIPCHK(d2d_copy(c->in_validity, validity, pbytes, s));
        RUN(ensure_fused_heads(c, s));
        if (!c->gexec[key]) {
            RUN(ensure_proxy_rgb(c, c->in_image, s));
            RUN(ensure_adam_table(c, s));
            const int rc = pipe_capture(c, &c->graph[key], &c->gexec[key], [&](hipStream_t cs) {
                return step_body(c, c->in_image, (key & 1) ? c->in_loss_image : c->in_image, c->in_sparse, (key & 2) ? c->in_validity : nullptr, (ptta_stream)cs);
            });
            if (rc) return rc;
        }
        HIPCHK(hipGraphLaunch(c->gexec[key], s));
        if (!c->ev_replay) HIPCHK(hipEventCreateWithFlags(&c->ev_replay, hipEventDisableTiming));
        HIPCHK(hipEventRecord(c->ev_replay, s));
        c->fwd_valid = true;
    } else {
        c->loss_info_dst = loss_info_out;
        const int rc = step_body(c, image, loss_image, sparse, validity, s_);
        c->loss_info_dst = nullptr;
        if (rc) return rc;
        if (depth_out) HIPCHK(d2d_copy(depth_out, final_depth(c), pbytes, s));
        return 0;
    }
    if (depth_out) HIPCHK(d2d_copy(depth_out, final_depth(c), pbytes, s));
    if (loss_info_out) HIPCHK(d2d_copy(loss_info_out, c->loss_info, 16, s));
    return 0;
}

int ptta_pipeline_stream(ptta_handle c, ptta_stream* out) {
    if (!c || !out) return -1;
    if (c->nl) return c->fail("frame pipelining is built for MSG_CHN handles", -38);
    RUN(pipe_init(c));
    *out = (ptta_stream)c->pre_stream;
    return 0;
}

int ptta_step_pipelined(ptta_handle c, const float* image, const float* loss_image, const float* sparse, const float* validity, uint64_t frame_token,
                        const float* next_image, const float* next_sparse, uint64_t next_token, float* depth_out, float* loss_info_out, ptta_stream s_) {
    if (c) c->err_code = 0;
    if (!c || !image || !sparse) return -1;
    if (c->nl || c->prof_on || c->dual || c->stat_sync.on() || c->grad_comm || c->naive || c->bf16) {
        const int rc = ptta_step(c, image, loss_image, sparse, validity, depth_out, loss_info_out, s_);
        if (!c->nl) { c->fb_image = rc ? nullptr : image; c->fb_sparse = rc ? nullptr : sparse; }
        return rc;
    }
    hipStream_t s = (hipStream_t)s_;
    if (!loss_image) loss_image = image;
    RUN(pipe_init(c));
    c->pipe_active = true;
    const size_t ibytes = (size_t)c->N * 3 * c->H * c->W * 4, pbytes = (size_t)c->N * c->H * c->W * 4;
    const int p = c->pipe_cur, q = 1 - p;
    const int key = (validity ? 2 : 0) | (loss_image != image ? 1 : 0);
    if (c->pipe_stream_set && c->pipe_stream != s) { HIPCHK(hipEventRecord(c->ev_rest[0], c->pipe_stream)); HIPCHK(hipStreamWaitEvent(s, c->ev_rest[0], 0)); }
    c->pipe_stream = s; c->pipe_stream_set = true;
    HIPCHK(hipEventRecord(c->ev_entry, s));
    pipe_use(c, p);
    RUN(ensure_fused_heads(c, s));
    if (!c->proxy_valid) RUN(ensure_proxy_rgb(c, c->in_image, s));
// ... 67 lines not shown
```

tta-depth-completion_amd/csrc/ptta_api.hip:

```cpp
#include "msgchn_ctx.h"

using namespace msgchn;

int msgchn::ensure_adam_table(ptta_ctx* c, hipStream_t s) {
    if (!c->adam_tab_dirty) return 0;
    for (auto& ad : c->adapted) if (!ad.p || !ad.m || !ad.v) return 0;
    c->adam_host.resize(c->adapted.size());
    long off = 0;
    for (size_t k = 0; k < c->adapted.size(); ++k) { auto& ad = c->adapted[k]; c->adam_host[k] = PttaAdamEntry{ad.p, ad.m, ad.v, ad.g, ad.n, off}; off += ad.n; }
    HIPCHK(hipMemcpyAsync(c->adam_tab, c->adam_host.data(), c->adam_host.size() * sizeof(PttaAdamEntry), hipMemcpyHostToDevice, s));
    c->adam_tab_dirty = false;
    return 0;
}

extern "C" {

int ptta_version(void) { return PTTA_ABI_VERSION; }

static thread_local std::string g_create_err;
static int create_refused(const std::string& why) { g_create_err = why; return -38; }

const char* ptta_last_error(ptta_handle h) {
    if (!h) return g_create_err.empty() ? "null handle" : g_create_err.c_str();
    return h->nl && h->err.empty() ? h->nl->err.c_str() : h->err.c_str();
// ... 302 lines not shown
    for (auto& ad : c->adapted) if (!ad.p || !ad.m || !ad.v) return c->fail("Adam state of " + ad.name + " not bound", -3);
    if ((gw || gb) && c->meta_mode != PTTA_META_1LAYER) return c->fail("explicit gradients are a 1layer convenience; use the internal ones", -22);
    hipStream_t s = (hipStream_t)s_;
    if (!gw && !gb) {
        RUN(ensure_adam_table(c, s));
        long total = 0; for (auto& ad : c->adapted) total += ad.n;
        REST_(s, ptta_launch_adam_multi(c->adam_tab, (int)c->adapted.size(), total, c->hyper, c->step_dev, c->adam_ticket, s));
        return 0;
    }
    RUN(ptta_launch_step_inc(c->step_dev, s));
    for (size_t k = 0; k < c->adapted.size(); ++k) {
        auto& ad = c->adapted[k];
        const float* g = ad.g;
        if (c->meta_mode == PTTA_META_1LAYER) { if (k == 0 && gw) g = gw; if (k == 1 && gb) g = gb; }
        RUN(ptta_launch_adam(ad.p, ad.m, ad.v, g, ad.n, c->hyper, c->step_dev, s));
    }
    return 0;
}

int ptta_set_image_norm(ptta_handle c, float divisor, const float* mean, const float* stdv) {
    NLFWD(c->nl->set_image_norm(divisor, mean, stdv));

    if (!c) return -1;
    if (!(divisor > 0.f)) return c->fail("ptta_set_image_norm: divisor must be positive", -22);
    ImgNorm nm = ImgNorm{0, divisor, {0.f, 0.f, 0.f}, {1.f, 1.f, 1.f}};
    for (int k = 0; k < 3; ++k) {
        if (mean) nm.mean[k] = mean[k];
        if (stdv) { if (!(stdv[k] > 0.f)) return c->fail("ptta_set_image_norm: std must be positive", -22); nm.stdv[k] = stdv[k]; }
    }
    nm.on = !(divisor == 1.f && nm.mean[0] == 0.f && nm.mean[1] == 0.f && nm.mean[2] == 0.f && nm.stdv[0] == 1.f &&
              nm.stdv[1] == 1.f && nm.stdv[2] == 1.f);
    c->img_norm = nm;
    c->drop_graphs();
    return 0;
}

static int set_stat_sync(ptta_ctx* c, const PttaStatSync& sy, bool on, bool keeps_graph) {
    if (c->nl && !c->nl->one_rank_why.empty()) { c->err.clear(); return c->nl->fail(c->nl->one_rank_why, -38); }
    if (c->nl && c->nl->meta_only) { c->err.clear(); return c->nl->fail("the SyncBatchNorm form of the meta-only adaptation mode is not offered (PTTA_ADAPT_META_ONLY)", -38); }
    if (c->nl) { c->err.clear(); c->nl->drop_graphs(); c->nl->stat_sync = sy; return 0; }
    if (on && c->meta_mode == PTTA_META_2LAYERS && !c->m2.generic) return c->fail("SyncBatchNorm needs the default arithmetic for the 2layers meta layer", -38);
    c->stat_sync = sy;
    c->drop_graphs();
    if (on) {
        if (c->pre_sync_graph < 0) { c->pre_sync_graph = c->use_graph; c->pre_sync_aux = c->use_aux; }
        else if (keeps_graph) c->use_graph = c->pre_sync_graph;
        if (!keeps_graph) c->use_graph = 0;
        c->use_aux = 0;
    } else if (c->pre_sync_graph >= 0) {
        c->use_graph = c->pre_sync_graph; c->use_aux = c->pre_sync_aux; c->pre_sync_graph = c->pre_sync_aux = -1;
    }
    return 0;
}

int ptta_set_stat_sync(ptta_handle c, ptta_allreduce_fn fn, void* user, double* exchange_buf, int64_t capacity, int world_size) {
    if (!c || world_size < 1 || (world_size > 1 && (!fn || !exchange_buf || capacity < 2 * 1024))) return -22;
    PttaStatSync sy; sy.fn = (ptta_allreduce_cb)fn; sy.user = user; sy.buf = exchange_buf; sy.cap = (long)capacity; sy.world = world_size;
    return set_stat_sync(c, sy, world_size > 1, false);
}

int ptta_set_stat_sync_rccl(ptta_handle c, void* comm, double* exchange_buf, int64_t capacity, int world_size) {
    if (!c || world_size < 1 || (comm && (!exchange_buf || capacity < 2 * 1024))) return -22;
    PttaStatSync sy; sy.comm = comm; sy.buf = exchange_buf; sy.cap = (long)capacity; sy.world = world_size;
    return set_stat_sync(c, sy, comm != nullptr, true);
}

int ptta_set_grad_sync_rccl(ptta_handle c, void* comm) {
    if (!c) return -1;
    if (c->nl && !c->nl->one_rank_why.empty()) { c->err.clear(); return c->nl->fail(c->nl->one_rank_why, -38); }
    if (c->nl && c->nl->meta_only) { c->err.clear(); return c->nl->fail("no gradient exchange in the meta-only adaptation mode: more than one rank is not offered (PTTA_ADAPT_META_ONLY)", -38); }
    if (c->nl) { c->nl->drop_graphs(); c->nl->grad_comm = comm; return 0; }
    c->grad_comm = comm;
    c->drop_graphs();
    return 0;
}

struct Option { const char* key; int ptta_ctx::*member; int hi; bool mixed_free; };
static const Option kOptions[] = {
    {"aux_stream", &ptta_ctx::use_aux, 1, true},        {"thru", &ptta_ctx::thru, 1, true},
    {"adam_in_wgrad", &ptta_ctx::adam_in_wgrad, 1, true}, {"bwd_w2", &ptta_ctx::bwd_w2, 1, true},
    {"fuse_first", &ptta_ctx::fuse_first, 2, false},    {"fuse_head_bwd", &ptta_ctx::fuse_head_bwd, 1, false},
    {"fuse_heads", &ptta_ctx::fuse_heads, 1, false},    {"heads_v2", &ptta_ctx::heads_v2, 1, false},
    {"cos_in_gemm", &ptta_ctx::cos_grad_fused, 1, false}, {"mask_bits", &ptta_ctx::mask_bits_on, 1, false},
    {"stamps", &ptta_ctx::stamps, 1, true},
};
static const Option* find_option(const std::string& k) {
    for (const Option& o : kOptions) if (k == o.key) return &o;
    return nullptr;
}
int ptta_set_option(ptta_handle c, const char* key, int value) {
    if (!c || !key) return -1;
    const std::string k(key);
    if (k == "graph") return ptta_set_graph(c, value);
    if (k == "eval_bn_fused") {
        if (!c->nl || !c->nl->meta_only) return c->nl ? (c->err.clear(), c->nl->fail("ptta_set_option: 'eval_bn_fused' belongs to PTTA_ADAPT_META_ONLY handles", -38))
                                                      : c->fail("ptta_set_option: 'eval_bn_fused' belongs to PTTA_ADAPT_META_ONLY handles", -38);
        c->err.clear();
        if (value < 0 || value > 1) return c->nl->fail("ptta_set_option: value out of range for 'eval_bn_fused'", -22);
        if (c->nl->eval_bn_fused != value) { c->nl->drop_graphs(); c->nl->eval_bn_fused = value; }
        return 0;
    }
    if (k == "head_bn_fused" || k == "head_bn_fused_count") {
        if (!c->nl) return c->fail("ptta_set_option: '" + k + "' belongs to the generic engine's handles (MSG_CHN has no BatchNorm2d)", -38);
        c->err.clear();
        if (k == "head_bn_fused_count") return c->nl->fail("ptta_set_option: 'head_bn_fused_count' is read-only", -22);
        if (value < 0 || value > 1) return c->nl->fail("ptta_set_option: value out of range for 'head_bn_fused'", -22);
        if (c->nl->head_bn_fused != value) { c->nl->drop_graphs(); c->nl->head_bn_fused = value; }
        return 0;
    }
    if (c->nl) return -38;
    const Option* o = find_option(k);
    if (!o) return c->fail("ptta_set_option: unknown key '" + k + "'", -22);
    int* f = &(c->*(o->member));
    if (value < 0 || value > o->hi) return c->fail("ptta_set_option: value out of range for '" + k + "'", -22);
    if (c->mixed && !o->mixed_free && value != 1)
        return c->fail("ptta_set_option: the mixed mode is defined on the default kernels ('" + k + "' stays 1)", -38);
    if (k == "aux_stream" && c->pre_sync_graph >= 0) { c->pre_sync_aux = value; return 0; }
    if (*f == value) return 0;
    RUN(pipe_quiesce(c));
    c->drop_graphs();
    *f = value;
    return 0;
}

int ptta_get_option(ptta_handle c, const char* key, int* value) {
    if (!c || !key || !value) return -1;
    const std::string k(key);
    if (k == "pipelined_active") { *value = !(c->nl || c->prof_on || c->dual || c->stat_sync.on() || c->grad_comm || c->naive || c->bf16); return 0; }
    if (k == "thru_active") { *value = c->nl ? 0 : (c->thru && c->cos_grad_fused && heads_v2_on(c) && c->use_aux); return 0; }
    if (k == "eval_bn_fused") { if (!c->nl || !c->nl->meta_only) return -38; *value = c->nl->eval_bn_fused; return 0; }
    if (k == "head_bn_fused" || k == "head_bn_fused_count") {
        if (!c->nl) return -38;
        *value = k == "head_bn_fused" ? c->nl->head_bn_fused : c->nl->head_bn_fused_count();
        return 0;
    }
    if (c->nl) { if (k != "graph") return -38; *value = c->nl->use_graph; return 0; }
    if (k == "graph") { *value = c->use_graph; return 0; }
    const Option* o = find_option(k);
    if (!o) return -22;
    *value = c->*(o->member);
    return 0;
}

int ptta_set_graph(ptta_handle c, int enable) {
    if (c && c->nl) { c->nl->use_graph = enable ? 1 : 0; if (!enable) c->nl->drop_graphs(); return 0; }

    if (!c) return -1;
    if (enable && c->stat_sync.on() && !c->stat_sync.comm) return c->fail("graph replay is not available with SyncBatchNorm exchange (ptta_set_stat_sync)", -38);
    c->use_graph = enable ? 1 : 0;
    if (!enable) c->drop_graphs();
    return 0;
}

int ptta_profile(ptta_handle c, int enable) {
    if (c && c->nl) return c->fail("not available for the NLSPN / CostDCNet backbones: use ptta_step / ptta_forward_*", -38);

    if (!c) return -1;
    c->prof_on = enable != 0;
    for (auto& pc : c->prof) { pc.used = 0; pc.bytes = 0; pc.macs = 0; pc.launches = 0; }
    c->prof_seq.clear();
    return 0;
}

int ptta_profile_read(ptta_handle c, int klass, double* ms_total, double* alg_bytes, double* macs, int64_t* launches, ptta_stream s_) {
    if (c && c->nl) return c->fail("not available for the NLSPN / CostDCNet backbones: use ptta_step / ptta_forward_*", -38);

    if (!c || klass < 0 || klass >= ptta_ctx::NPROF) return -1;
    HIPCHK(hipStreamSynchronize((hipStream_t)s_));
    ptta_ctx::ProfClass& pc = c->prof[klass];
    double ms = 0;
    for (size_t k = 0; k < pc.used; ++k) {
        float t = 0.f;
        HIPCHK(hipEventElapsedTime(&t, pc.ev[k].first, pc.ev[k].second));
        ms += t;
    }
    if (ms_total) *ms_total = ms;
    if (alg_bytes) *alg_bytes = pc.bytes;
    if (macs) *macs = pc.macs;
    if (launches) *launches = (int64_t)pc.launches;
    return 0;
}

int ptta_debug_tensor(ptta_handle c, const char* name, float* dst, int64_t capacity, int64_t* numel_host, ptta_stream s_) {
    NLFWD(c->nl->debug_tensor(name, dst, capacity, numel_host, (hipStream_t)s_));

    if (!c || !name) return -1;
    if (std::string(name) == "prof_seq") {
        HIPCHK(hipStreamSynchronize((hipStream_t)s_));
        const int64_t n = 2 * (int64_t)c->prof_seq.size();
        if (numel_host) *numel_host = n;
        if (!dst) return 0;
        if (capacity < n) return c->fail("capacity too small", -22);
        std::vector<float> h((size_t)n);
        for (size_t k = 0; k < c->prof_seq.size(); ++k) {
            const auto& q = c->prof_seq[k];
            float t = 0.f;
            HIPCHK(hipEventElapsedTime(&t, c->prof[q.first].ev[q.second].first, c->prof[q.first].ev[q.second].second));
            h[2 * k] = (float)q.first; h[2 * k + 1] = 1e3f * t;
        }
        HIPCHK(hipMemcpy(dst, h.data(), (size_t)n * 4, hipMemcpyHostToDevice));
        return 0;
    }
    auto it = c->dbg.find(name);
    if (it == c->dbg.end()) return c->fail(std::string("no debug tensor ") + name, -2);
    if (numel_host) *numel_host = it->second.numel;
    if (!dst) return 0;
    if (capacity < it->second.numel) return c->fail("capacity too small", -22);
    hipStream_t s = (hipStream_t)s_;
    const long n = it->second.numel;
    if (it->second.is_act == 3) RUN(ptta_launch_hn_untile(it->second.p, dst, n / 512, s));
    else if ((it->second.is_act == 1 && c->bf16) || it->second.is_act == 2) to_f32_launch((const bf16_t*)it->second.p, dst, n, s);
    else HIPCHK(hipMemcpyAsync(dst, it->second.p, (size_t)n * 4, hipMemcpyDeviceToDevice, s));
    return 0;
}

}
```

tta-depth-completion_amd/csrc/ptta_common.h:

```cpp
#pragma once
#include <hip/hip_runtime.h>
#include <stdint.h>

typedef unsigned short bf16_t;
typedef float f32x16 __attribute__((ext_vector_type(16)));
typedef float f32x4 __attribute__((ext_vector_type(4)));
typedef __bf16 bf16x8 __attribute__((ext_vector_type(8)));

#define PTTA_WAVE 64

__device__ __forceinline__ float bf2f(bf16_t v) { return __uint_as_float(((unsigned)v) << 16); }
__device__ __forceinline__ bf16_t f2bf(float f) {
    unsigned u = __float_as_uint(f);
    if ((u & 0x7fffffffu) > 0x7f800000u) return (bf16_t)((u >> 16) | 0x40);
    return (bf16_t)((u + 0x7fffu + ((u >> 16) & 1u)) >> 16);
}
template <typename T> __device__ __forceinline__ float ld(const T* p);
template <> __device__ __forceinline__ float ld<float>(const float* p) { return *p; }
template <> __device__ __forceinline__ float ld<bf16_t>(const bf16_t* p) { return bf2f(*p); }
template <typename T> __device__ __forceinline__ void st(T* p, float v);
template <> __device__ __forceinline__ void st<float>(float* p, float v) { *p = v; }
template <> __device__ __forceinline__ void st<bf16_t>(bf16_t* p, float v) { *p = f2bf(v); }

typedef __bf16 cbf16x2 __attribute__((ext_vector_type(2)));
// ... 289 lines not shown
                if (two) { const float4 a2 = bf4_to_f4(t2[g]); a.x += a2.x; a.y += a2.y; a.z += a2.z; a.w += a2.w; }
                val.x += a.x; val.y += a.y; val.z += a.z; val.w += a.w;
            }
            if (e.out_sum && okg[g]) *(uint2*)(osum + xq[g]) = f4_to_bf4(val);
        }
        return;
    }
    if (MASK) {
        const T* mrow = e.mask + ((size_t)(b % e.mask_nb) * H * W + rowoff) * 32 + ch;
        float m[16];
#pragma unroll
        for (int r = 0; r < 16; ++r) m[r] = ld(mrow + (size_t)xo[r] * 32);
#pragma unroll
        for (int r = 0; r < 16; ++r) v[r] = m[r] > 0.0f ? v[r] : 0.0f;
    }
    const size_t obase = ((size_t)b * H * W + rowoff) * 32 + ch;
    if (e.out_raw) {
#pragma unroll
        for (int r = 0; r < 16; ++r)
            if (ok[r]) st(e.out_raw + obase + (size_t)xo[r] * 32, v[r]);
    }
    if (ADD) {
        const T* a1 = e.add1 + ((size_t)(b % e.add1_nb) * H * W + rowoff) * 32 + ch;
        float t1[16];
#pragma unroll
        for (int r = 0; r < 16; ++r) t1[r] = ld(a1 + (size_t)xo[r] * 32);
        if (e.add2) {
            const T* a2 = e.add2 + ((size_t)(b % e.add2_nb) * H * W + rowoff) * 32 + ch;
            float t2[16];
#pragma unroll
            for (int r = 0; r < 16; ++r) t2[r] = ld(a2 + (size_t)xo[r] * 32);
#pragma unroll
            for (int r = 0; r < 16; ++r) t1[r] += t2[r];
        }
#pragma unroll
        for (int r = 0; r < 16; ++r) v[r] += t1[r];
    }
    if (e.out_sum) {
#pragma unroll
        for (int r = 0; r < 16; ++r)
            if (ok[r]) st(e.out_sum + obase + (size_t)xo[r] * 32, v[r]);
    }
}

__device__ __forceinline__ float cos_grad_elem(float coef, float e, float r, float ie, float ir, float proj) {
    return coef * (e * ie - proj * r * ir) * ir;
}
__device__ __forceinline__ int acc_row(int r, int h) { return (r & 3) + 8 * (r >> 2) + 4 * h; }

enum { CONV_S1 = 0, CONV_S2 = 1, CONV_T2 = 2 };

struct Corner { int h0, w0; float lh, lw; bool inside; };
__device__ __forceinline__ Corner corner_of(float h, float w, int H, int W) {
    Corner c;
    c.inside = (h > -1.f) && (w > -1.f) && (h < (float)H) && (w < (float)W);
    const float fh = floorf(h), fw = floorf(w);
    c.h0 = (int)fh; c.w0 = (int)fw; c.lh = h - fh; c.lw = w - fw;
    return c;
}
__device__ __forceinline__ float bilinear_at(const float* __restrict__ im, int H, int W, const Corner& c) {
    if (!c.inside) return 0.f;
    const int h1 = c.h0 + 1, w1 = c.w0 + 1;
    const float v1 = (c.h0 >= 0 && c.w0 >= 0) ? im[c.h0 * W + c.w0] : 0.f;
    const float v2 = (c.h0 >= 0 && w1 <= W - 1) ? im[c.h0 * W + w1] : 0.f;
    const float v3 = (h1 <= H - 1 && c.w0 >= 0) ? im[h1 * W + c.w0] : 0.f;
    const float v4 = (h1 <= H - 1 && w1 <= W - 1) ? im[h1 * W + w1] : 0.f;
    const float hh = 1.f - c.lh, hw = 1.f - c.lw;
    return hh * hw * v1 + hh * c.lw * v2 + c.lh * hw * v3 + c.lh * c.lw * v4;
}



__device__ __forceinline__ unsigned xcd_swizzle(unsigned orig, unsigned nwg) {
    const unsigned xcd = orig & 7u, q = nwg >> 3, r = nwg & 7u;
    return (xcd < r ? xcd * (q + 1) : r * (q + 1) + (xcd - r) * q) + (orig >> 3);
}

__device__ __forceinline__ void lds_barrier() {
    asm volatile("s_waitcnt lgkmcnt(0)" ::: "memory");
    __builtin_amdgcn_s_barrier();
    asm volatile("" ::: "memory");
}

#define PTTA_CHECK_LAUNCH() do { hipError_t e_ = hipGetLastError(); if (e_ != hipSuccess) return (int)e_; } while (0)
```

tta-depth-completion_amd/csrc/ptta_kernels.h:

```cpp
#pragma once
#include <hip/hip_runtime.h>
#include <cstdlib>
#include <cstring>
#include "ptta_common.h"

struct PttaCreateEnv { int naive = 0, exact = 0, graph = -1; };
inline PttaCreateEnv ptta_create_env() {
    PttaCreateEnv e;
    const char* v = getenv("PTTA_CONV_IMPL"); e.naive = (v && strcmp(v, "naive") == 0) ? 1 : 0;
    v = getenv("PTTA_ARITH"); e.exact = (v && strcmp(v, "exact") == 0) ? 1 : 0;
    v = getenv("PTTA_GRAPH"); e.graph = (v && (strcmp(v, "0") == 0 || strcmp(v, "1") == 0)) ? (v[0] - '0') : -1;
    return e;
}

struct ConvW {
    float* mf32;
    bf16_t* mbf16;
    bf16_t* mlo;
    float* canon;
};
struct Conv32Args {
    const void* in = nullptr; int in_nb = 1;
    const ConvW* w = nullptr;
    const float* bias = nullptr;
    const void* up = nullptr; int up_nb = 1;
    const void* mask = nullptr; int mask_nb = 1;
    const void* add1 = nullptr; int add1_nb = 1;
    const void* add2 = nullptr; int add2_nb = 1;
    void* out_raw = nullptr; void* out_sum = nullptr;
    int B = 1, Hin = 0, Win = 0;
    int mode = CONV_S1; int relu_in = 0; int bf16 = 0; int naive = 0;
    int x3 = 0;
    int w2 = 0;
    const uint32_t* mask_bits = nullptr;
    uint32_t* bits_out = nullptr; int bits_nb = 0; int bits_sum = 0;
};
void ptta_pack_conv32(const float* src, const ConvW& w, int in_major, int flip, hipStream_t s, int row_stride = 32, int col_off = 0);
int ptta_launch_conv32(const Conv32Args& a, hipStream_t s);
int ptta_launch_conv32_loop(const Conv32Args& a, void* buf_a, void* buf_b, int reps, unsigned* ctr, unsigned* base_io, int* err, int variant, hipStream_t s);

struct Plane { const float* p = nullptr; int nb = 1; long bstride = 0;
               int norm = 0; float div = 1.f, mean = 0.f, stdv = 1.f; };
struct ConvInArgs {
    Plane pl[3]; int cin = 1; int zero_from_b = 1 << 30;
    const float* wfrag = nullptr;
    const float* wcanon = nullptr;
    const float* bias = nullptr;
    const void* up = nullptr; int up_nb = 1;
    const void* mask = nullptr; int mask_nb = 1;
    const void* add1 = nullptr; int add1_nb = 1;
    void* out_raw = nullptr; void* out_sum = nullptr;
    int B = 1, H = 0, W = 0; int bf16 = 0; int naive = 0;
    const uint32_t* mask_bits = nullptr; uint32_t* a_bits = nullptr;
    int a_bits_nb = 0;
};
void ptta_pack_conv_in(const float* src, int cin_total, int cin_first, int cin, int transpose_flip,
                       float* wfrag, float* wcanon, hipStream_t s);
int ptta_launch_conv_in(const ConvInArgs& a, hipStream_t s);
int ptta_launch_conv32_first(const Conv32Args& a, const ConvInArgs& f, void* a_out, int a_nb, hipStream_t s);

struct ConvOut1Args {
    const void* in = nullptr; int in_nb = 1;
    const float* w = nullptr;
    const float* bias = nullptr;
    const float* add = nullptr; int add_nb = 1;
    float* out = nullptr;
    int B = 1, H = 0, W = 0; int relu_in = 0; int bf16 = 0;
};
void ptta_pack_conv_out1(const float* src, int src_cin_total, int src_cin_index, int from_conv_in, float* w, hipStream_t s);
int ptta_launch_conv_out1(const ConvOut1Args& a, hipStream_t s);

int ptta_launch_prep(const float* sparse, float max_input_depth, float* dclamp, float* d12, float* d14,
                     int N, int H, int W, hipStream_t s);
int ptta_launch_up2_1ch(const float* in, float* out, int B, int Hin, int Win, hipStream_t s);
int ptta_launch_up2T_1ch(const float* gout, float* gin, int B, int Hin, int Win, hipStream_t s);
int ptta_launch_up2T_32(const void* gout, const void* add, void* gin, int B, int Hin, int Win, int bf16, hipStream_t s);

int ptta_launch_outlier_removal(const float* sparse, const float* validity, float* sparse_out, float* validity_out,
                                int N, int H, int W, int ksize, float threshold, float* scratch, hipStream_t s);

typedef int (*ptta_allreduce_cb)(void* user, double* dev_buf, long long count, void* stream);
int ptta_rccl_sum_f64(void* comm, double* buf, long long count, hipStream_t s);
struct PttaStatSync {
    ptta_allreduce_cb fn = nullptr; void* user = nullptr;
    void* comm = nullptr;
    double* buf = nullptr; long cap = 0; int world = 1;
    bool on() const { return (fn || comm) && (world > 1 || comm); }
    int exchange(long long count, hipStream_t s) const {
        if (comm) return ptta_rccl_sum_f64(comm, buf, count, s);
        const int rc = fn(user, buf, count, (void*)s);
        return rc ? (rc < 0 ? rc : -rc) : 0;
    }
};
int ptta_stat_sync(const PttaStatSync* sy, float* part, int nblocks, int C, int npass, hipStream_t s);
int ptta_grad_mean_sync(const PttaStatSync* sy, float* g, long n, hipStream_t s);

struct GemmArgs {
    const void* A = nullptr; int a_bf16 = 0;
    const float* A2 = nullptr;
    const float* W = nullptr;
    const float* bias = nullptr;
    float* C = nullptr;
    int R = 0, K = 0, N = 0;
    int pro = 0;
    const float* pscale = nullptr; const float* pshift = nullptr;
    const float* pmean = nullptr; const float* pinv = nullptr;
    const float* pc1 = nullptr; const float* pc2 = nullptr;
    int epi = 0;
    const float* eH = nullptr;
    const float* escale = nullptr; const float* eshift = nullptr; const float* emean = nullptr; const float* einv = nullptr;
    float* part = nullptr;
    int x3 = 0; const bf16_t* Whi = nullptr; const bf16_t* Wlo = nullptr;
    const bf16_t* Wil = nullptr;
    const float* X = nullptr;
    const void* W0frag = nullptr;
    const float* b0 = nullptr;
    const bf16_t* W0hi = nullptr; const bf16_t* W0lo = nullptr;
    const bf16_t* W0thi = nullptr; const bf16_t* W0tlo = nullptr;
    float* P = nullptr;
    const float* Bref = nullptr; const float* rowstats = nullptr; const float* coef = nullptr;
};
// ... 206 lines not shown
```

tta-depth-completion_amd/csrc/ptta_ops.hip:

```cpp
#include "msgchn_ctx.h"
#include "gnet.h"
#include "costdc.h"

using namespace msgchn;

namespace {
struct ScratchConvW {
    ConvW w{};
    bool ok;
    ScratchConvW() {
        ok = hipMalloc((void**)&w.mf32, 9 * 4 * 64 * 4 * 4) == hipSuccess && hipMalloc((void**)&w.mbf16, 9 * 2 * 64 * 8 * 2) == hipSuccess &&
             hipMalloc((void**)&w.canon, 9216 * 4) == hipSuccess && hipMalloc((void**)&w.mlo, 9 * 2 * 64 * 8 * 2) == hipSuccess;
    }
    ~ScratchConvW() { (void)hipFree(w.mf32); (void)hipFree(w.mbf16); (void)hipFree(w.mlo); (void)hipFree(w.canon); }
    ScratchConvW(const ScratchConvW&) = delete;
    ScratchConvW& operator=(const ScratchConvW&) = delete;
};

__global__ void op_scale_f64_kernel(double* buf, long long n, double f) {
    for (long long i = (long long)blockIdx.x * blockDim.x + threadIdx.x; i < n; i += (long long)gridDim.x * blockDim.x) buf[i] *= f;
}
int op_gbn_exchange(void* user, double* buf, long long count, void* stream) {
    long long blocks = (count + 255) / 256; if (blocks > 1024) blocks = 1024; if (blocks < 1) blocks = 1;
    hipLaunchKernelGGL(op_scale_f64_kernel, dim3((int)blocks), dim3(256), 0, (hipStream_t)stream, buf, count, (double)*(const int*)user);
    return hipGetLastError() == hipSuccess ? 0 : -5;
}
}

extern "C" {

int ptta_outlier_removal(const float* sparse, const float* validity, float* sparse_out, float* validity_out, int n, int height,
                         int width, int kernel_size, float threshold, float* scratch, ptta_stream s) {
    if (!sparse || !validity || !sparse_out || !validity_out || !scratch || n < 1 || height < 1 || width < 1 || kernel_size < 1 ||
        (kernel_size & 1) == 0) return -22;
    return ptta_launch_outlier_removal(sparse, validity, sparse_out, validity_out, n, height, width, kernel_size, threshold, scratch,
                                       (hipStream_t)s);
}

int ptta_eval_metrics(const float* depth, const float* ground_truth, int64_t numel, float min_evaluate_depth, float max_evaluate_depth,
                      void* scratch, float* metrics_out, ptta_stream s) {
    if (!depth || !ground_truth || !scratch || !metrics_out || numel < 1) return -22;
    return ptta_launch_eval_metrics(depth, ground_truth, numel, min_evaluate_depth, max_evaluate_depth, (double*)scratch, metrics_out,
                                    (hipStream_t)s);
}

static void dcn_args(DcnArgs& a, const float* input, const float* weight, const float* bias, const float* offset, const float* mask,
                     int b, int c, int h, int w, int c_out, int kh, int kw, int sh, int sw, int ph, int pw, int dh, int dw, int group, int dg) {
    a.in = input; a.weight = weight; a.bias = bias; a.offset = offset; a.mask = mask;
    a.B = b; a.C = c; a.H = h; a.W = w; a.Co = c_out; a.kh = kh; a.kw = kw; a.sh = sh; a.sw = sw; a.ph = ph; a.pw = pw;
    a.dh = dh; a.dw = dw; a.group = group; a.dg = dg;
}

int ptta_mdconv_forward(const float* input, const float* weight, const float* bias, const float* offset, const float* mask, float* output,
                        int b, int c, int h, int w, int c_out, int kh, int kw, int sh, int sw, int ph, int pw, int dh, int dw,
                        int group, int deformable_group, ptta_stream s) {
    if (!input || !weight || !offset || !mask || !output) return -22;
    DcnArgs a; dcn_args(a, input, weight, bias, offset, mask, b, c, h, w, c_out, kh, kw, sh, sw, ph, pw, dh, dw, group, deformable_group);
    a.out = output;
    return ptta_launch_dcn_forward(a, (hipStream_t)s);
}

int ptta_mdconv_backward(const float* input, const float* weight, const float* bias, const float* offset, const float* mask,
                         const float* grad_output, float* grad_input, float* grad_offset, float* grad_mask, float* grad_weight,
                         float* grad_bias, int b, int c, int h, int w, int c_out, int kh, int kw, int sh, int sw, int ph, int pw,
                         int dh, int dw, int group, int deformable_group, ptta_stream s) {
    if (!input || !weight || !offset || !mask || !grad_output) return -22;
    DcnArgs a; dcn_args(a, input, weight, bias, offset, mask, b, c, h, w, c_out, kh, kw, sh, sw, ph, pw, dh, dw, group, deformable_group);
    a.gout = grad_output; a.gin = grad_input; a.goff = grad_offset; a.gmask = grad_mask; a.gweight = grad_weight; a.gbias = grad_bias;
    return ptta_launch_dcn_backward(a, (hipStream_t)s);
}

int ptta_op_conv32(const float* in, const float* weight, const float* bias, float* out, int b, int hin, int win, int mode,
                   int relu_in, int in_major, int flip, int dtype, int naive, ptta_stream s_) {
    hipStream_t s = (hipStream_t)s_;
    ScratchConvW sw; ConvW& w = sw.w;
    void *tin = nullptr, *tout = nullptr;
    const int ho = mode == CONV_S1 ? hin : (mode == CONV_S2 ? hin / 2 : hin * 2), wo = mode == CONV_S1 ? win : (mode == CONV_S2 ? win / 2 : win * 2);
    const long nin = (long)b * hin * win * 32, nout = (long)b * ho * wo * 32;
    int rc = 0;
    if (!sw.ok || hipMalloc(&tin, nin * 2) != hipSuccess || hipMalloc(&tout, nout * 2) != hipSuccess) rc = -12;
    if (rc == 0) {
        ptta_pack_conv32(weight, w, in_major, flip, s);
        Conv32Args a; a.w = &w; a.bias = bias; a.B = b; a.Hin = hin; a.Win = win; a.mode = mode; a.relu_in = relu_in; a.naive = naive & 1; a.x3 = (naive >> 1) & 1;
        if (dtype != PTTA_DTYPE_F32) {
            from_f32_launch(in, (bf16_t*)tin, nin, s);
            a.in = tin; a.in_nb = b; a.out_raw = tout; a.bf16 = 1;
            rc = ptta_launch_conv32(a, s);
            to_f32_launch((const bf16_t*)tout, out, nout, s);
        } else {
            a.in = in; a.in_nb = b; a.out_raw = out; a.bf16 = 0;
            rc = ptta_launch_conv32(a, s);
        }
        (void)hipStreamSynchronize(s);
    }
    (void)hipFree(tin); (void)hipFree(tout);
    return rc;
}

int ptta_op_gwgrad(const float* x, const float* gy, float* gw, float* gb, int b, int h, int w, int ci, int co, int impl, int reps,
                   float* us_per_call_host, ptta_stream s_) {
    hipStream_t s = (hipStream_t)s_;
    if (!x || !gy || !gw || b < 1 || h < 1 || w < 1 || ci < 1 || co < 1 || ci > 256 || co > 256 || impl < 0 || impl > 2 || reps < 0 ||
        (reps > 0 && !us_per_call_host)) return -22;
    GView xv, gv;
    xv.p = (float*)x; xv.B = b; xv.H = h; xv.W = w; xv.C = ci; xv.ld = ci;
    gv.p = (float*)gy; gv.B = b; gv.H = h; gv.W = w; gv.C = co; gv.ld = co;
    const long P = (long)b * h * w;
    const size_t nm = (size_t)ptta_gwgrad_mfma_part_floats(P, ci, co), nn = (size_t)ptta_gwgrad_slabs(P) * (9 * ci * co + co);
    float* part = nullptr;
    if (hipMalloc((void**)&part, (impl == 2 ? nn : nm) * 4) != hipSuccess) return -12;
    auto run = [&]() {
        return impl == 0 ? ptta_launch_gwgrad_mfma(xv, gv, part, gw, gb, s)
                         : (impl == 1 ? ptta_launch_gwgrad_f32mfma(xv, gv, part, gw, gb, s) : ptta_launch_gwgrad(xv, gv, part, gw, gb, s));
    };
    int rc = run();
    if (!rc && reps > 0) {
        hipEvent_t e0 = nullptr, e1 = nullptr;
        if (hipEventCreate(&e0) != hipSuccess || hipEventCreate(&e1) != hipSuccess) rc = -5;
        if (!rc) {
            (void)hipEventRecord(e0, s);
            for (int r = 0; r < reps && !rc; ++r) rc = run();
            (void)hipEventRecord(e1, s);
            (void)hipEventSynchronize(e1);
            float ms = 0.f; (void)hipEventElapsedTime(&ms, e0, e1);
            *us_per_call_host = 1e3f * ms / (float)reps;
        }
        if (e0) (void)hipEventDestroy(e0);
        if (e1) (void)hipEventDestroy(e1);
    }
    if (hipStreamSynchronize(s) != hipSuccess && !rc) rc = -5;
    (void)hipFree(part);
    return rc;
}

static int op_gconv(const float* x0, int c0, int ld0, const float* x1, int c1, int ld1, const float* weight, const float* bias, float* y, int co,
                    int ldy, int b, int hin, int win, int hout, int wout, int k, int geom, int act, int accumulate, int impl, int flags,
                    int six_b, int x1_from_b, int stat_npass, double* stat_host, int* form_host, bool affine, const float* scale, const float* shift,
                    const float* res, int ld_res, ptta_stream s_) {
    hipStream_t s = (hipStream_t)s_;
    if (affine) {
        const int cm = geom == PTTA_GCONV_S1 ? 7 : 15;
        if (!scale || !shift || (((size_t)scale | (size_t)shift) & 15) || (res != nullptr) != (ld_res != 0) || (res && ld_res < co) ||
            impl != 0 || accumulate || stat_npass || six_b < 0 || six_b > b || (flags & PTTA_GCONV_DGRAD) || (act != GACT_NONE && act != GACT_RELU && act != GACT_LRELU) ||
            c0 < 1 || c1 < 0 || (c0 & cm) || (c1 & cm)) return -22;
        const bool af = flags & PTTA_GCONV_AFF_ACT_FIRST, rp = flags & PTTA_GCONV_AFF_RES_PLAIN;
        if ((af && rp) || (af && (!res || act != GACT_RELU || (flags & PTTA_GCONV_VERT))) || (rp && (!res || act != GACT_NONE))) return -22;
        if (geom == PTTA_GCONV_T2 && (af || six_b > 0)) return -22;
    } else if (flags & (PTTA_GCONV_AFF_ACT_FIRST | PTTA_GCONV_AFF_RES_PLAIN)) return -22;
    const bool vert = flags & PTTA_GCONV_VERT, dgrad = flags & PTTA_GCONV_DGRAD;
    if (!x0 || !weight || !y || b < 1 || hin < 1 || win < 1 || hout < 1 || wout < 1 || c0 < 1 || c1 < 0 || co < 1 || ld0 < c0 || ldy < co ||
        (c1 > 0) != (x1 != nullptr) || (c1 > 0 && ld1 < c1) || (k != 1 && k != 3) || geom < PTTA_GCONV_S1 || geom > PTTA_GCONV_T2 ||
        act < GACT_NONE || act > GACT_SIGMOID || impl < 0 || impl > 1 || (flags & ~31) || six_b < 0 || six_b > b || x1_from_b < 0 ||
        stat_npass < 0 || stat_npass > 2 || (accumulate & ~1)) return -22;
    if (vert && (k != 3 || geom != PTTA_GCONV_S1)) return -22;
    if (dgrad && (c1 > 0 || six_b > 0)) return -22;
    if (stat_npass > 0 && (!stat_host || geom != PTTA_GCONV_S1 || impl != 0 || dgrad || (b % stat_npass))) return -22;
    const int run = !dgrad ? geom : (geom == PTTA_GCONV_S2 ? PTTA_GCONV_T2 : (geom == PTTA_GCONV_T2 ? PTTA_GCONV_S2 : PTTA_GCONV_S1));
    const bool size_ok = run == PTTA_GCONV_S1 ? (hout == hin && wout == win)
                       : run == PTTA_GCONV_S2 ? (hout == (hin + 1) / 2 && wout == (win + 1) / 2)
                       : ((hout == 2 * hin || (dgrad && hout == 2 * hin - 1)) && (wout == 2 * win || (dgrad && wout == 2 * win - 1)));
    if (!size_ok) return -22;
    if (impl == 0 && ((((size_t)x0 | (size_t)x1) & 15) || (ld0 & 3) || (ld1 & 3))) return -22;
    if (form_host) *form_host = -1;

    gnet::GConvW cw;
    cw.k = k; cw.stride = geom == PTTA_GCONV_S1 ? 1 : 2; cw.transposed = geom == PTTA_GCONV_T2 ? 1 : 0; cw.vcol = vert ? 1 : 0;
    if (!dgrad) { cw.Ci = c0 + c1; cw.Co = co; cw.C0 = c0; cw.C1 = c1; }
    else { cw.Ci = co; cw.Co = c0; cw.C0 = co; cw.C1 = 0; }
    cw.mf = impl == 0 && !dgrad; cw.mb = impl == 0 && dgrad;
    const int KK = k * k;
    const size_t nw = (size_t)KK * cw.Ci * cw.Co;
    const size_t nfrag = cw.mf ? (size_t)ptta_gfrag_elems(KK, cw.C0, cw.C1, cw.Co) : (cw.mb ? (size_t)ptta_gfrag_elems(KK, cw.Co, 0, cw.Ci) : 0);
    const int tiles_pp = stat_npass ? ptta_gconv_x3_tiles(b / stat_npass, hout, wout) : 0;
    const size_t nstat = (size_t)stat_npass * tiles_pp * 2 * co;
    float* wbuf = nullptr; bf16_t* fbuf = nullptr; float* stat = nullptr;
    int rc = 0;
    if (hipMalloc((void**)&wbuf, 2 * nw * sizeof(float)) != hipSuccess || (nfrag && hipMalloc((void**)&fbuf, 3 * nfrag * sizeof(bf16_t)) != hipSuccess) ||
        (nstat && hipMalloc((void**)&stat, nstat * sizeof(float)) != hipSuccess)) rc = -12;
// ... 390 lines not shown
```

tta-depth-completion_amd/proxytta/_lib.py:

```python
import ctypes
import os
from ctypes import POINTER, byref, c_char_p, c_float, c_int, c_int64, c_uint64, c_void_p


_HERE = os.path.dirname(os.path.abspath(__file__))
LIB_PATH = os.path.join(_HERE, 'libptta_hip.so')

PTTA_BACKBONE_MSG_CHN = 0
PTTA_BACKBONE_NLSPN = 1
PTTA_BACKBONE_COSTDCNET = 2
PTTA_NLSPN_LEGACY_OFFSET = 0x100
PTTA_NLSPN_SYNCBN_ADAPT = 0x200
PTTA_SYNCBN_ADAPT = 0x200
PTTA_ADAPT_META_ONLY = 0x400
PTTA_META_1LAYER = 0
PTTA_META_2LAYERS = 1
PTTA_META_NONE = 2
PTTA_DTYPE_F32 = 0
PTTA_DTYPE_MIXED = 1
PTTA_HEAD_FORM_PLAIN = 0
PTTA_HEAD_FORM_SYNCBN = 1
PTTA_GCONV_VERT = 1
PTTA_GCONV_X1_W2 = 2
PTTA_GCONV_DGRAD = 4
# ... 14 lines not shown


class GbnArgs(ctypes.Structure):
    _fields_ = ([(n, c_int) for n in ('mode', 'b', 'h', 'w', 'npass', 'act', 'act_first', 'res_relu', 'acc_gx', 'acc_gres', 'world',
                                      'nblocks_in', 'repeats')] + [('eps', c_float), ('momentum', c_float)] +
                [(n, GbnView) for n in ('x', 'res', 'y', 'g', 'gx', 'gres')] +
                [(n, c_void_p) for n in ('gamma', 'beta', 'part_in', 'st', 'rm', 'rv', 'nbt', 'st_eval', 'dgamma', 'dbeta')])


class CdSbnArgs(ctypes.Structure):
    _fields_ = ([(n, c_int) for n in ('mode', 'level', 'c', 'relu', 'repeats', 'world', 'acc_res')] +
                [(n, c_void_p) for n in ('f', 'res', 'y', 'g', 'gamma', 'beta', 'rm', 'rv', 'nbt', 'out', 'st', 'dgamma', 'dbeta', 'gx', 'gres')])


CD_OPS = {'pad_dual': 0, 'crop_avg': 1, 'scatter_dual_grad': 2, 'stage': 3, 'clamp': 4, 'fusion_fwd': 5, 'fusion_bwd': 6, 'pool_fwd': 7,
          'pool_bwd': 8, 'up_fwd': 9, 'up_bwd': 10, 'regress_fwd': 11, 'regress_bwd': 12, 'rows_fwd': 13, 'rows_bwd': 14}

_P = c_void_p
SIGNATURES = [
    ('ptta_create', c_int, [POINTER(c_void_p), c_int, c_int, c_int, c_int, c_int, c_int, POINTER(Hparams)]),
    ('ptta_destroy', None, [_P]),
    ('ptta_last_error', c_char_p, [_P]),
    ('ptta_set_hparams', c_int, [_P, POINTER(Hparams), _P]),
    ('ptta_load_weights', c_int, [_P, c_char_p, _P, POINTER(c_int64), c_int, _P]),
    ('ptta_bind_adapted', c_int, [_P, c_char_p, _P, _P, _P]),
    ('ptta_set_adam_step', c_int, [_P, c_int, _P]),
    ('ptta_get_adam_step', c_int, [_P, POINTER(c_int), _P]),
    ('ptta_forward_train', c_int, [_P, _P, _P, _P, _P, _P, _P]),
    ('ptta_embedding_rows', c_int64, [_P]),
    ('ptta_forward_eval', c_int, [_P, _P, _P, _P, _P]),
    ('ptta_loss_forward', c_int, [_P, _P, _P, _P, _P, _P, _P, c_int64, c_float, c_float, c_float, _P, _P]),
    ('ptta_loss_backward', c_int, [_P, _P, _P, _P, _P, _P, _P, c_int64, _P, _P, _P]),
    ('ptta_backward', c_int, [_P, _P, _P, _P, _P, _P]),
    ('ptta_set_grad', c_int, [_P, c_char_p, _P, c_int64, _P]),
    ('ptta_get_grad', c_int, [_P, c_char_p, _P, c_int64, _P]),
    ('ptta_adapted_count', c_int, [_P]),
    ('ptta_adapted_name', c_char_p, [_P, c_int, POINTER(c_int64)]),
    ('ptta_adapted_repeat', c_int, [_P, c_int]),
    ('ptta_adam_step', c_int, [_P, _P, _P, _P]),
    ('ptta_step', c_int, [_P, _P, _P, _P, _P, _P, _P, _P]),
    ('ptta_step_pipelined', c_int, [_P] * 5 + [c_uint64] + [_P] * 2 + [c_uint64] + [_P] * 3),
    ('ptta_pipeline_stream', c_int, [_P, POINTER(c_void_p)]),
    ('ptta_forward_eval_last', c_int, [_P, _P, _P]),
    ('ptta_outlier_removal', c_int, [_P, _P, _P, _P, c_int, c_int, c_int, c_int, c_float, _P, _P]),
    ('ptta_eval_metrics', c_int, [_P, _P, c_int64, c_float, c_float, _P, _P, _P]),
    ('ptta_mdconv_forward', c_int, [_P] * 6 + [c_int] * 15 + [_P]),
    ('ptta_mdconv_backward', c_int, [_P] * 11 + [c_int] * 15 + [_P]),
    ('ptta_set_image_norm', c_int, [_P, c_float, POINTER(c_float), POINTER(c_float)]),
    ('ptta_head_bind', c_int, [_P, c_char_p, _P, _P, _P]),
    ('ptta_head_set_hparams', c_int, [_P, c_float, c_float, c_float, c_float, c_float, c_float, c_int, _P]),
    ('ptta_head_reload', c_int, [_P, _P]),
    ('ptta_head_forward', c_int, [_P, _P, _P, c_int, _P, _P, _P]),
    ('ptta_head_backward', c_int, [_P, _P, _P]),
    ('ptta_head_adam_step', c_int, [_P, _P]),
    ('ptta_head_step', c_int, [_P, _P, _P, c_int, _P, _P]),
    ('ptta_head_get_grad', c_int, [_P, c_char_p, _P, c_int64, POINTER(c_int), _P]),
    ('ptta_head_set_form', c_int, [_P, c_int]),
    ('ptta_crop_flip', c_int, [_P, _P] + [c_int] * 6 + [_P] * 5),
    ('ptta_rotate', c_int, [_P, _P, c_int, c_int, c_int, c_int, _P, _P, c_int, _P]),
    ('ptta_resize_crop', c_int, [_P, _P, c_int, c_int, c_int, c_int, _P, _P, _P, _P, _P, c_int, c_int, _P]),
    ('ptta_photometric', c_int, [_P, _P, c_int, c_int, c_int, _P, _P, _P, _P, _P, _P, _P, _P]),
    ('ptta_photometric_full', c_int, [_P, _P, c_int, c_int, c_int] + [_P] * 12),
    ('ptta_add_noise', c_int, [_P, _P, _P, c_int, c_int, c_int, c_int, _P, c_float, c_int, _P]),
    ('ptta_remove_patches', c_int, [_P, _P, c_int, c_int, c_int, c_int, _P, _P, _P, _P, _P]),
    ('ptta_crop_pad', c_int, [_P, _P, c_int, c_int, c_int, c_int] + [_P] * 7 + [c_int, c_float, _P]),
    ('ptta_resize_pad', c_int, [_P, _P, c_int, c_int, c_int, c_int] + [_P] * 5 + [c_int, c_int, c_float, _P]),
    ('ptta_set_stat_sync', c_int, [_P, _P, _P, _P, c_int64, c_int]),
    ('ptta_rccl_unique_id', c_int, [_P]),
    ('ptta_rccl_comm_create', c_int, [_P, c_int, c_int, POINTER(c_void_p)]),
    ('ptta_rccl_comm_destroy', c_int, [_P]),
    ('ptta_rccl_allreduce_mean_f32', c_int, [_P, _P, c_int64, _P]),
    ('ptta_rccl_last_error', c_char_p, []),
    ('ptta_set_stat_sync_rccl', c_int, [_P, _P, _P, c_int64, c_int]),
    ('ptta_set_grad_sync_rccl', c_int, [_P, _P]),
    ('ptta_set_graph', c_int, [_P, c_int]),
    ('ptta_set_option', c_int, [_P, c_char_p, c_int]),
    ('ptta_get_option', c_int, [_P, c_char_p, POINTER(c_int)]),
    ('ptta_profile', c_int, [_P, c_int]),
    ('ptta_profile_read', c_int, [_P, c_int, POINTER(ctypes.c_double), POINTER(ctypes.c_double), POINTER(ctypes.c_double),
                                  POINTER(c_int64), _P]),
    ('ptta_debug_tensor', c_int, [_P, c_char_p, _P, c_int64, POINTER(c_int64), _P]),
    ('ptta_op_conv32', c_int, [_P, _P, _P, _P, c_int, c_int, c_int, c_int, c_int, c_int, c_int, c_int, c_int, _P]),
    ('ptta_op_conv32_chain', c_int, [_P] * 6 + [c_int] * 7 + [POINTER(c_float), _P]),
    ('ptta_op_gwgrad', c_int, [_P, _P, _P, _P] + [c_int] * 7 + [POINTER(c_float), _P]),
    ('ptta_op_gconv', c_int, [_P, c_int, c_int, _P, c_int, c_int, _P, _P, _P] + [c_int] * 16 + [POINTER(ctypes.c_double), POINTER(c_int), _P]),
    ('ptta_op_gconv_affine', c_int, [_P, c_int, c_int, _P, c_int, c_int, _P, _P, _P] + [c_int] * 16 + [POINTER(ctypes.c_double), POINTER(c_int),
                                     _P, _P, _P, c_int, _P]),
    ('ptta_op_gbn', c_int, [POINTER(GbnArgs), _P]),
    ('ptta_cd_sparse_create', c_int, [POINTER(c_void_p), c_int, c_int, c_int]),
    ('ptta_cd_sparse_destroy', None, [_P]),
    ('ptta_cd_sparse_build', c_int, [_P, _P, c_float, _P]),
    ('ptta_cd_sparse_read', c_int, [_P, c_int, POINTER(c_int), _P, ctypes.c_longlong, _P, _P, _P]),
    ('ptta_op_cd_sparse_conv', c_int, [_P, _P, _P, _P] + [c_int] * 7 + [_P]),
    ('ptta_op_cd_sbn', c_int, [_P, POINTER(CdSbnArgs), _P]),
    ('ptta_op_cd_densify', c_int, [_P, _P, _P, c_int, c_int, c_int, c_int, _P]),
    ('ptta_op_cd_dense', c_int, [c_int, _P, _P, _P, _P, POINTER(c_int), POINTER(c_float), _P]),
    ('ptta_version', c_int, []),
]

_lib = None


def load():
    global _lib
    if _lib is not None:
        return _lib
    import torch
    if not os.path.exists(LIB_PATH):
        raise RuntimeError('libptta_hip.so not found at %s: build it with `python -c "import '
                           '__graft_entry__ as g; g.build()"` — there is no CPU fallback' % LIB_PATH)
    lib = ctypes.CDLL(LIB_PATH)
    for name, res, args in SIGNATURES:
        fn = getattr(lib, name)
        fn.restype = res
        fn.argtypes = args
    have = lib.ptta_version()
    if have != PTTA_ABI_VERSION:
        raise RuntimeError('%s has ABI version %d, this binding is written against %d (include/ptta.h PTTA_ABI_VERSION): rebuild it with '
                           '`make -C tta-depth-completion_amd/csrc`' % (LIB_PATH, have, PTTA_ABI_VERSION))
    _lib = lib
    return lib


def check(lib, handle, rc, what):
    if rc != 0:
        msg = lib.ptta_last_error(handle).decode() if handle else ''
        raise RuntimeError('%s failed (%d): %s' % (what, rc, msg))


def ptr(t):
    if t is None:
        return None
    assert t.is_contiguous()
    return c_void_p(t.data_ptr())


__all__ = ['load', 'check', 'ptr', 'Hparams', 'GbnArgs', 'GbnView', 'CdSbnArgs', 'CD_OPS', 'SIGNATURES', 'LIB_PATH', 'byref']
```

Measured before the change: 826.8.

## Fuse strided conv32 with following 3x3 conv in one pair kernel

```diff
diff --git a/include/ptta.h b/include/ptta.h
--- a/include/ptta.h
+++ b/include/ptta.h
@@ -153,6 +153,11 @@
 int ptta_op_conv32(const float* in_nhwc, const float* weight, const float* bias, float* out_nhwc,
                    int b, int hin, int win, int mode, int relu_in, int in_major, int flip, int dtype, int naive,
                    ptta_stream s);
+int ptta_op_conv32_pair(const float* in_nhwc, const float* weight1, const float* bias1, const float* weight2, const float* bias2,
+                        const float* up_nhwc, const float* add0_nhwc, const float* add1_nhwc, const float* add2_nhwc,
+                        const uint32_t* mask1_bits, const uint32_t* mask2_bits, float* out_raw, float* out_sum, float* mid_raw,
+                        float* mid_sum, uint32_t* mid_bits, int b, int in_nb, int hin, int win, int first_mode, int relu1, int relu2,
+                        int in_major, int flip, int dtype, int w2, int fused, int* fused_host, ptta_stream s);
 int ptta_op_gwgrad(const float* x_nhwc, const float* gy_nhwc, float* gw, float* gb, int b, int h, int w, int ci, int co, int impl,
                    int reps, float* us_per_call_host, ptta_stream s);
 #define PTTA_GCONV_S1 0
diff --git a/tta-depth-completion_amd/csrc/conv32.hip b/tta-depth-completion_amd/csrc/conv32.hip
--- a/tta-depth-completion_amd/csrc/conv32.hip
+++ b/tta-depth-completion_amd/csrc/conv32.hip
@@ -3,23 +3,11 @@
 #include "ptta_common.h"
 #include "ptta_kernels.h"
 
-template <typename T>
-struct Conv32P {
-    const T* in; int in_nb;
-    const void* wpack;
-    const void* wpack2;
-    Epi<T> epi;
-    int B, Hin, Win, Hout, Wout;
-};
 
 template <typename T> struct Frag;
 template <> struct Frag<float> { typedef float4 A; };
 template <> struct Frag<bf16_t> { typedef uint4 A; };
 
-__device__ __forceinline__ float4 relu4(float4 v) {
-    v.x = fmaxf(v.x, 0.f); v.y = fmaxf(v.y, 0.f); v.z = fmaxf(v.z, 0.f); v.w = fmaxf(v.w, 0.f);
-    return v;
-}
 __device__ __forceinline__ unsigned relu_bf2(unsigned v) {
     unsigned neg = (v >> 15) & 0x00010001u;
     return v & ~(neg * 0xffffu);
@@ -122,58 +110,6 @@
 }
 
 
-#define X3_TH 8
-#define X3_PW 34
-#define X3_PH 10
-
-typedef __bf16 bf16x2_t __attribute__((ext_vector_type(2)));
-typedef float float2_t __attribute__((ext_vector_type(2)));
-typedef short short2_t __attribute__((ext_vector_type(2)));
-
-__device__ __forceinline__ void split2(float a, float b, unsigned& hi, unsigned& lo) {
-    float2_t v = {a, b};
-    const bf16x2_t h = __builtin_convertvector(v, bf16x2_t);
-    hi = __builtin_bit_cast(unsigned, h);
-    float2_t r = {a - __uint_as_float(hi << 16), b - __uint_as_float(hi & 0xffff0000u)};
-    lo = __builtin_bit_cast(unsigned, __builtin_convertvector(r, bf16x2_t));
-}
-__device__ __forceinline__ unsigned relu_pk(unsigned v) {
-    const short2_t z = {0, 0};
-    return __builtin_bit_cast(unsigned, __builtin_elementwise_max(__builtin_bit_cast(short2_t, v), z));
-}
-
-template <typename T> struct Px;
-template <> struct Px<float> { float4 a, b; };
-template <> struct Px<bf16_t> { uint4 a; };
-template <typename T> __device__ __forceinline__ Px<T> px_zero();
-template <> __device__ __forceinline__ Px<float> px_zero<float>() { Px<float> r; r.a = make_float4(0.f, 0.f, 0.f, 0.f); r.b = r.a; return r; }
-template <> __device__ __forceinline__ Px<bf16_t> px_zero<bf16_t>() { Px<bf16_t> r; r.a = make_uint4(0u, 0u, 0u, 0u); return r; }
-__device__ __forceinline__ Px<float> px_load(const float* src) { Px<float> r; r.a = *(const float4*)src; r.b = *(const float4*)(src + 4); return r; }
-__device__ __forceinline__ Px<bf16_t> px_load(const bf16_t* src) { Px<bf16_t> r; r.a = *(const uint4*)src; return r; }
-template <bool RELU>
-__device__ __forceinline__ void px_stage(const Px<float>& v, unsigned char* dst, int lo_off) {
-    float4 a0 = v.a, a1 = v.b;
-#ifdef X3_TIMING_NOSPLIT
-    *(float4*)dst = a0; *(float4*)(dst + lo_off) = a1; return;
-#endif
-    if (RELU) { a0 = relu4(a0); a1 = relu4(a1); }
-    uint4 hi, lo;
-    split2(a0.x, a0.y, hi.x, lo.x); split2(a0.z, a0.w, hi.y, lo.y);
-    split2(a1.x, a1.y, hi.z, lo.z); split2(a1.z, a1.w, hi.w, lo.w);
-    *(uint4*)dst = hi;
-    *(uint4*)(dst + lo_off) = lo;
-}
-template <bool RELU>
-__device__ __forceinline__ void px_stage(const Px<bf16_t>& v, unsigned char* dst, int) {
-    uint4 hi = v.a;
-    if (RELU) { hi.x = relu_pk(hi.x); hi.y = relu_pk(hi.y); hi.z = relu_pk(hi.z); hi.w = relu_pk(hi.w); }
-    *(uint4*)dst = hi;
-}
-template <typename T> struct Geo;
-template <> struct Geo<float> { static constexpr int STR = 144, LO = 64, WL = 18 * 64 * 16, UPPX = 128, UPPC = 8; };
-template <> struct Geo<bf16_t> { static constexpr int STR = 80, LO = 0, WL = 0, UPPX = 64, UPPC = 4; };
-
-__device__ __forceinline__ int x3_stage_pix(int idx) { return ((idx >> 5) << 3) + (((idx >> 2) & 1) << 2) + ((idx >> 3) & 3); }
 
 template <typename T, bool W2 = false>
 __device__ __forceinline__ void mma_step(f32x16& acc, const unsigned char* a, const uint4& wh, const unsigned char* wl) {
diff --git a/tta-depth-completion_amd/csrc/conv_pair.hip b/tta-depth-completion_amd/csrc/conv_pair.hip
--- /dev/null
+++ b/tta-depth-completion_amd/csrc/conv_pair.hip
@@ -0,0 +1,293 @@
+#include "ptta_common.h"
+#include "ptta_kernels.h"
+
+#define PR_TH 4
+#define PR_TW 32
+#define PR_MH (PR_TH + 2)
+#define PR_NG ((PR_MH * X3_PW + 31) / 32)
+#define PR_WH (2 * PR_MH + 1)
+#define PR_WW (2 * X3_PW + 1)
+#define PR_NT 512
+static_assert(PR_TW + 2 == X3_PW && PR_NG * 64 <= PR_NT, "one wave per group of the intermediate tile");
+
+template <typename T, int FIRST, bool W2, bool RELU, bool M1, bool A1, bool UP, bool ADD, bool M2>
+__global__ __launch_bounds__(PR_NT, 1) void conv32_pair_small_kernel(Conv32P<T> p1, Conv32P<T> p2) {
+    static_assert(FIRST == CONV_S2, "instantiated forms: see the head of this file");
+    constexpr bool F32 = sizeof(T) == 4, LO = F32 || W2;
+    static_assert(!(W2 && F32) && !((M1 || A1) && F32), "the masked / summed first half exists for the narrow data gradients");
+    constexpr int STR = Geo<T>::STR;
+    constexpr int WSTR = F32 ? 80 : 48;
+    constexpr int NWPIX = PR_WH * PR_WW, NIT = (NWPIX * 2 + PR_NT - 1) / PR_NT;
+    constexpr int WFR = 18 * 64, NWI = (WFR + PR_NT - 1) / PR_NT;
+    constexpr int UPH = 4, UPW = 18, NUP = UPH * UPW * Geo<T>::UPPC, NUI = UP ? (NUP + PR_NT - 1) / PR_NT : 1;
+    constexpr int WIN_B = NWPIX * WSTR + 16, MID_B = PR_MH * X3_PW * STR, W1_B = (LO ? 2 : 1) * WFR * 16, W2L_B = LO ? WFR * 16 : 0;
+    static_assert(!UP || UPH * UPW * Geo<T>::UPPX <= WIN_B, "the bilinear window takes the input window's place once phase 1 is over");
+    __shared__ __attribute__((aligned(16))) unsigned char lds[WIN_B + MID_B + W1_B + W2L_B];
+    unsigned char* const win = lds;
+    unsigned char* const mid = lds + WIN_B;
+    unsigned char* const w1_lds = mid + MID_B;
+    unsigned char* const w2l_lds = w1_lds + W1_B;
+    unsigned char* const up_lds = win;
+    const int tid = threadIdx.x, lane = tid & 63;
+    const int i = lane & 31, h = lane >> 5;
+    const float bias1 = epi_bias(p1.epi, i), bias2 = epi_bias(p2.epi, i);
+    const int wave = __builtin_amdgcn_readfirstlane(tid >> 6);
+    const int Hin = p1.Hin, Win = p1.Win, Hm = p2.Hout, Wm = p2.Wout;
+    const int ntx = (Wm + PR_TW - 1) / PR_TW, nty = (Hm + PR_TH - 1) / PR_TH;
+    const int tile = blockIdx.x;
+    const int ty = tile % nty, tx = (tile / nty) % ntx, b = tile / (nty * ntx);
+    const int y0 = ty * PR_TH, x0 = tx * PR_TW;
+    const float sy = up_scale(Hm >> 1, Hm), sx = up_scale(Wm >> 1, Wm);
+
+    const T* inb = p1.in + (size_t)(b % p1.in_nb) * Hin * Win * 32;
+    Px<T> v[2][NIT];
+    unsigned vok = 0;
+#pragma unroll
+    for (int it = 0; it < NIT; ++it) {
+        const int idx = tid + PR_NT * it;
+        const int g = idx & 1, pix = idx >> 1;
+        const int py = pix / PR_WW, px = pix - py * PR_WW;
+        const int gy = 2 * y0 - 3 + py, gx = 2 * x0 - 3 + px;
+        if (pix < NWPIX && gy >= 0 && gy < Hin && gx >= 0 && gx < Win) vok |= 1u << it;
+        const T* src = inb + ((size_t)min(max(gy, 0), Hin - 1) * Win + min(max(gx, 0), Win - 1)) * 32 + 8 * g;
+        v[0][it] = px_load(src);
+        v[1][it] = px_load(src + 16);
+    }
+    uint4 w1h[NWI], w1l[LO ? NWI : 1], w2l[LO ? NWI : 1];
+#pragma unroll
+    for (int k = 0; k < NWI; ++k) {
+        const int idx = min(tid + PR_NT * k, WFR - 1);
+        w1h[k] = ((const uint4*)p1.wpack)[idx];
+        if constexpr (LO) { w1l[k] = ((const uint4*)p1.wpack2)[idx]; w2l[k] = ((const uint4*)p2.wpack2)[idx]; }
+    }
+    uint4 wh2[9][2];
+#pragma unroll
+    for (int t = 0; t < 9; ++t)
+#pragma unroll
+        for (int k = 0; k < 2; ++k) wh2[t][k] = ((const uint4*)p2.wpack)[(t * 2 + k) * 64 + lane];
+    int uy0 = 0, ux0 = 0;
+    uint4 upv0 = make_uint4(0u, 0u, 0u, 0u), upv1 = upv0;
+    static_assert(NUI <= 2, "bilinear window pieces per thread");
+    auto up_src = [&](const int idx_) {
+        constexpr int PC = Geo<T>::UPPC;
+        const int Hu = Hm >> 1, Wu = Wm >> 1;
+        const int idx = min(idx_, NUP - 1);
+        const int q = idx % PC, pix = idx / PC;
+        const int r = pix / UPW, cc = pix - r * UPW;
+        const int gy = min(uy0 + r, Hu - 1), gx = min(ux0 + cc, Wu - 1);
+        return (const uint4*)(p2.epi.up + (size_t)(b % p2.epi.up_nb) * Hu * Wu * 32 + ((size_t)gy * Wu + gx) * 32 + (32 / PC) * q);
+    };
+    if constexpr (UP) {
+        uy0 = lerp_coef(y0, Hm >> 1, sy).i0; ux0 = lerp_coef(x0, Wm >> 1, sx).i0;
+        upv0 = *up_src(tid);
+        if constexpr (NUI > 1) upv1 = *up_src(tid + PR_NT);
+    }
+
+    uint32_t mw1[M1 ? 4 : 1];
+    uint2 a1v[A1 ? 4 : 1];
+    if constexpr (M1 || A1) {
+        const int tq_ = (i & 3) + 4 * h;
+#pragma unroll
+        for (int j = 0; j < 4; ++j) {
+            const int pp = min(32 * min(wave, PR_NG - 1) + 8 * j + tq_, PR_MH * X3_PW - 1);
+            const int row = pp / X3_PW, col = pp - row * X3_PW;
+            const size_t cpix = (size_t)min(max(y0 - 1 + row, 0), Hm - 1) * Wm + min(max(x0 - 1 + col, 0), Wm - 1);
+            if constexpr (M1) mw1[j] = p1.epi.mask_bits[(size_t)(b % p1.epi.mask_nb) * Hm * Wm + cpix];
+            if constexpr (A1) a1v[j] = *(const uint2*)((const bf16_t*)p1.epi.add1 + ((size_t)(b % p1.epi.add1_nb) * Hm * Wm + cpix) * 32 + 4 * (i >> 2));
+        }
+    }
+
+    auto stage_window = [&](const int q) {
+#pragma unroll
+        for (int it = 0; it < NIT; ++it) {
+            const int idx = tid + PR_NT * it;
+            const int pix = idx >> 1;
+            Px<T> x = v[q][it];
+            if (!((vok >> it) & 1u)) x = px_zero<T>();
+            if (pix < NWPIX) px_stage<RELU>(x, win + pix * WSTR + 16 * (idx & 1), 32);
+        }
+    };
+    f32x16 acc;
+#pragma unroll
+    for (int r = 0; r < 16; ++r) acc[r] = 0.f;
+    const int pm = min(32 * wave + i, PR_MH * X3_PW - 1);
+    const unsigned char* const abase = win + ((2 * (pm / X3_PW)) * PR_WW + 2 * (pm % X3_PW)) * WSTR + 16 * h;
+    auto first_kstep = [&](const int q) {
+#pragma unroll
+        for (int tap = 0; tap < 9; ++tap) {
+            const int ky = tap / 3, kx = tap % 3;
+            const unsigned char* a = abase + (ky * PR_WW + kx) * WSTR;
+            const bf16x8 ah = __builtin_bit_cast(bf16x8, *(const uint4*)a);
+            const bf16x8 bh = __builtin_bit_cast(bf16x8, *(const uint4*)(w1_lds + ((tap * 2 + q) * 64 + lane) * 16));
+            if constexpr (F32) {
+                const bf16x8 al = __builtin_bit_cast(bf16x8, *(const uint4*)(a + 32));
+                const bf16x8 bl = __builtin_bit_cast(bf16x8, *(const uint4*)(w1_lds + ((WFR + (tap * 2 + q) * 64) + lane) * 16));
+                acc = __builtin_amdgcn_mfma_f32_32x32x16_bf16(al, bh, acc, 0, 0, 0);
+                acc = __builtin_amdgcn_mfma_f32_32x32x16_bf16(ah, bl, acc, 0, 0, 0);
+            } else if constexpr (W2) {
+                const bf16x8 bl = __builtin_bit_cast(bf16x8, *(const uint4*)(w1_lds + ((WFR + (tap * 2 + q) * 64) + lane) * 16));
+                acc = __builtin_amdgcn_mfma_f32_32x32x16_bf16(ah, bl, acc, 0, 0, 0);
+            }
+            acc = __builtin_amdgcn_mfma_f32_32x32x16_bf16(ah, bh, acc, 0, 0, 0);
+        }
+    };
+
+    stage_window(0);
+#pragma unroll
+    for (int k = 0; k < NWI; ++k) {
+        const int idx = tid + PR_NT * k;
+        if (idx < WFR) {
+            *(uint4*)(w1_lds + idx * 16) = w1h[k];
+            if constexpr (LO) { *(uint4*)(w1_lds + (WFR + idx) * 16) = w1l[k]; *(uint4*)(w2l_lds + idx * 16) = w2l[k]; }
+        }
+    }
+    lds_barrier();
+    if (wave < PR_NG) first_kstep(0);
+    lds_barrier();
+    stage_window(1);
+    lds_barrier();
+    if (wave < PR_NG) {
+        first_kstep(1);
+        f32x16 t;
+#pragma unroll
+        for (int r = 0; r < 16; ++r) t[r] = acc[r] + bias1;
+        quad_transpose(t, lane);
+        const int tq = (i & 3) + 4 * h, c4 = 4 * (i >> 2);
+        const bool wbits = F32 && p1.epi.bits_out != nullptr && b < p1.epi.bits_nb;
+#pragma unroll
+        for (int j = 0; j < 4; ++j) {
+            const int pp = 32 * wave + 8 * j + tq;
+            const int row = pp / X3_PW, col = pp - row * X3_PW;
+            const int my = y0 - 1 + row, mx = x0 - 1 + col;
+            const bool inimg = pp < PR_MH * X3_PW && my >= 0 && my < Hm && mx >= 0 && mx < Wm;
+            const bool own = inimg && row >= 1 && row <= PR_TH && col >= 1 && col <= PR_TW;
+            const size_t opix = inimg ? ((size_t)b * Hm + my) * Wm + mx : 0;
+            const float4 val = make_float4(t[4 * j], t[4 * j + 1], t[4 * j + 2], t[4 * j + 3]);
+            unsigned char* dst = mid + min(pp, PR_MH * X3_PW - 1) * STR + 2 * c4;
+            if constexpr (F32) {
+                if (p1.epi.out_raw && own) *(float4*)((float*)p1.epi.out_raw + opix * 32 + c4) = val;
+                if (wbits) {
+                    const uint32_t word = mask_word_from_quads(val.x, val.y, val.z, val.w, i, h);
+                    if (i < 4 && own) p1.epi.bits_out[opix] = word;
+                }
+                float4 r = RELU ? relu4(val) : val;
+                if (!inimg) r = make_float4(0.f, 0.f, 0.f, 0.f);
+                uint2 hi, lo;
+                split2(r.x, r.y, hi.x, lo.x); split2(r.z, r.w, hi.y, lo.y);
+                if (pp < PR_MH * X3_PW) { *(uint2*)dst = hi; *(uint2*)(dst + Geo<T>::LO) = lo; }
+            } else {
+                float4 mv = val;
+                if constexpr (M1) {
+                    const uint32_t nib = mw1[j] >> c4;
+                    mv.x = (nib & 1u) ? mv.x : 0.0f; mv.y = (nib & 2u) ? mv.y : 0.0f; mv.z = (nib & 4u) ? mv.z : 0.0f; mv.w = (nib & 8u) ? mv.w : 0.0f;
+                }
+                uint2 pk = f4_to_bf4(mv);
+                if (p1.epi.out_raw && own) *(uint2*)((bf16_t*)p1.epi.out_raw + opix * 32 + c4) = pk;
+                if constexpr (A1) {
+                    const float4 a = bf4_to_f4(a1v[j]);
+                    mv.x += a.x; mv.y += a.y; mv.z += a.z; mv.w += a.w;
+                    pk = f4_to_bf4(mv);
+                    if (p1.epi.out_sum && own) *(uint2*)((bf16_t*)p1.epi.out_sum + opix * 32 + c4) = pk;
+                }
+                if constexpr (RELU) { pk.x = relu_pk(pk.x); pk.y = relu_pk(pk.y); }
+                if (!inimg) pk = make_uint2(0u, 0u);
+                if (pp < PR_MH * X3_PW) *(uint2*)dst = pk;
+            }
+        }
+    }
+    lds_barrier();
+    if constexpr (UP) {
+        if (tid < NUP) *(uint4*)(up_lds + (size_t)tid * 16) = upv0;
+        if constexpr (NUI > 1) { if (tid + PR_NT < NUP) *(uint4*)(up_lds + (size_t)(tid + PR_NT) * 16) = upv1; }
+    }
+
+    const int y = y0 + wave;
+    const bool rowon = wave < PR_TH && y < Hm;
+#pragma unroll
+    for (int r = 0; r < 16; ++r) acc[r] = 0.f;
+    if (rowon) {
+#pragma unroll
+        for (int tap = 0; tap < 9; ++tap) {
+            const int ky = tap / 3, kx = tap % 3;
+            const unsigned char* a = mid + ((wave + ky) * X3_PW + i + kx) * STR + 16 * h;
+#pragma unroll
+            for (int k = 0; k < 2; ++k) {
+                const bf16x8 ah = __builtin_bit_cast(bf16x8, *(const uint4*)(a + 32 * k));
+                const bf16x8 bh = __builtin_bit_cast(bf16x8, wh2[tap][k]);
+                if constexpr (F32) {
+                    const bf16x8 al = __builtin_bit_cast(bf16x8, *(const uint4*)(a + 32 * k + 64));
+                    const bf16x8 bl = __builtin_bit_cast(bf16x8, *(const uint4*)(w2l_lds + ((tap * 2 + k) * 64 + lane) * 16));
+                    acc = __builtin_amdgcn_mfma_f32_32x32x16_bf16(al, bh, acc, 0, 0, 0);
+                    acc = __builtin_amdgcn_mfma_f32_32x32x16_bf16(ah, bl, acc, 0, 0, 0);
+                } else if constexpr (W2) {
+                    const bf16x8 bl = __builtin_bit_cast(bf16x8, *(const uint4*)(w2l_lds + ((tap * 2 + k) * 64 + lane) * 16));
+                    acc = __builtin_amdgcn_mfma_f32_32x32x16_bf16(ah, bl, acc, 0, 0, 0);
+                }
+                acc = __builtin_amdgcn_mfma_f32_32x32x16_bf16(ah, bh, acc, 0, 0, 0);
+            }
+        }
+    }
+    if constexpr (UP) lds_barrier();
+    if (rowon) {
+        if (UP) epi_tile<T, false, M2, ADD, true, UPW>(p2.epi, b, y, Hm, Wm, i, acc, x0, h, Wm, 1, 0, sy, sx, up_lds, uy0, ux0, &bias2);
+        else epi_tile<T, false, M2, ADD>(p2.epi, b, y, Hm, Wm, i, acc, x0, h, Wm, 1, 0, sy, sx, nullptr, 0, 0, &bias2);
+    }
+}
+
+template <typename T>
+static Conv32P<T> pair_params(const Conv32Args& a, int Hout, int Wout) {
+    Conv32P<T> p;
+    p.in = (const T*)a.in; p.in_nb = a.in_nb > 0 ? a.in_nb : 1;
+    p.wpack = a.w->mbf16; p.wpack2 = (sizeof(T) == 4 || a.w2) ? a.w->mlo : nullptr;
+    p.epi.bias = a.bias;
+    p.epi.up = (const T*)a.up; p.epi.up_nb = a.up_nb > 0 ? a.up_nb : 1;
+    p.epi.mask = (const T*)a.mask; p.epi.mask_nb = a.mask_nb > 0 ? a.mask_nb : 1;
+    p.epi.add1 = (const T*)a.add1; p.epi.add1_nb = a.add1_nb > 0 ? a.add1_nb : 1;
+    p.epi.add2 = (const T*)a.add2; p.epi.add2_nb = a.add2_nb > 0 ? a.add2_nb : 1;
+    p.epi.out_raw = (T*)a.out_raw; p.epi.out_sum = (T*)a.out_sum;
+    p.epi.mask_bits = a.mask_bits; p.epi.bits_out = a.bits_out; p.epi.bits_nb = a.bits_nb; p.epi.bits_sum = a.bits_sum;
+    p.B = a.B; p.Hin = a.Hin; p.Win = a.Win; p.Hout = Hout; p.Wout = Wout;
+    return p;
+}
+
+template <typename T>
+static int launch_pair_t(const Conv32Args& f, const Conv32Args& g, hipStream_t s) {
+    const int Hm = f.Hin / 2, Wm = f.Win / 2;
+    const Conv32P<T> p1 = pair_params<T>(f, Hm, Wm), p2 = pair_params<T>(g, Hm, Wm);
+    const long tiles = (long)f.B * ((Wm + PR_TW - 1) / PR_TW) * ((Hm + PR_TH - 1) / PR_TH);
+    if constexpr (sizeof(T) == 2) {
+        if (f.w2) {
+            hipLaunchKernelGGL((conv32_pair_small_kernel<T, CONV_S2, true, false, true, true, false, false, true>), dim3((unsigned)tiles), dim3(PR_NT), 0, s, p1, p2);
+            PTTA_CHECK_LAUNCH();
+            return 0;
+        }
+    }
+    if (g.add1) hipLaunchKernelGGL((conv32_pair_small_kernel<T, CONV_S2, false, true, false, false, true, true, false>), dim3((unsigned)tiles), dim3(PR_NT), 0, s, p1, p2);
+    else hipLaunchKernelGGL((conv32_pair_small_kernel<T, CONV_S2, false, true, false, false, true, false, false>), dim3((unsigned)tiles), dim3(PR_NT), 0, s, p1, p2);
+    PTTA_CHECK_LAUNCH();
+    return 0;
+}
+
+bool ptta_conv32_pair_applies(const Conv32Args& first, const Conv32Args& second) {
+    const Conv32Args &f = first, &g = second;
+    if (!f.w || !g.w || !f.in) return false;
+    if (f.mode != CONV_S2 || g.mode != CONV_S1 || f.bf16 != g.bf16 || f.naive || g.naive || (!f.bf16 && (!f.x3 || !g.x3)) || f.w2 != g.w2) return false;
+    if (f.bits_out && (f.bits_sum || f.bf16)) return false;
+    if (g.bits_out && g.bf16) return false;
+    if (f.w2) {
+        if (!f.bf16 || f.relu_in || g.relu_in || f.up || g.up || f.bits_out || g.bits_out) return false;
+        if (!f.mask || !f.mask_bits || !f.add1 || f.add2 || !f.out_sum) return false;
+        if (!g.mask || !g.mask_bits || g.add1 || g.add2 || g.out_sum || !g.out_raw) return false;
+    } else {
+        if (!f.relu_in || f.up || f.mask || f.add1 || f.add2 || f.out_sum || f.mask_bits) return false;
+        if (!g.relu_in || !g.up || g.mask || g.mask_bits || (g.add2 && !g.add1) || (!g.out_raw && !g.out_sum)) return false;
+    }
+    const int Hm = f.Hin / 2, Wm = f.Win / 2;
+    if (Hm < 2 || Wm < 2 || g.Hin != Hm || g.Win != Wm || g.B != f.B || f.B < 1) return false;
+    const long tiles8 = (long)g.B * ((Wm + 31) / 32) * ((Hm + X3_TH - 1) / X3_TH);
+    return tiles8 <= 256;
+}
+int ptta_launch_conv32_pair(const Conv32Args& first, const Conv32Args& second, hipStream_t s) {
+    if (!ptta_conv32_pair_applies(first, second)) return 1;
+    return first.bf16 ? launch_pair_t<bf16_t>(first, second, s) : launch_pair_t<float>(first, second, s);
+}
diff --git a/tta-depth-completion_amd/csrc/msgchn_backward.hip b/tta-depth-completion_amd/csrc/msgchn_backward.hip
--- a/tta-depth-completion_amd/csrc/msgchn_backward.hip
+++ b/tta-depth-completion_amd/csrc/msgchn_backward.hip
@@ -132,10 +132,9 @@
     CV("depth_decoder3.dec2.3", true, CONV_S1, c->ds1_3, Nn, Nn, H2, W2, false, em(c->dt3, c->t3, Nn));
     if (join_aux) HIPCHK(hipStreamWaitEvent(s, c->ev_join, 0));
     { E e; e.raw = c->dw2; e.mask = c->w2; e.mask_nb = B2; e.sum = c->dfeat_tot; e.add1 = c->g_feat; e.add1_nb = Nn;
-      CV("depth_decoder3.dec2.1", true, CONV_S2, c->dt3, Nn, Nn, H2, W2, false, e); }
+      RUN(conv32_pair(c, s, true, "depth_decoder3.dec2.1", c->dt3, Nn, Nn, H2, W2, e, "depth_encoder3.enc2.3", Nn, em(c->de3_2a, c->e3_2a, B2))); }
     hipStream_t sd = join_aux ? c->aux(s) : nullptr;
     if (!sd) sd = s;
-    CV("depth_encoder3.enc2.3", true, CONV_S1, c->dfeat_tot, Nn, Nn, H4, W4, false, em(c->de3_2a, c->e3_2a, B2));
     { E e; e.sum = c->de3_1; e.mask = c->e3_1; e.mask_nb = B2; e.add1 = c->ds1_3; e.add1_nb = Nn;
       CV("depth_encoder3.enc2.1", true, CONV_T2, c->de3_2a, Nn, Nn, H4, W4, false, e); }
     CV("depth_encoder3.enc1.3", true, CONV_S1, c->de3_1, Nn, Nn, H2, W2, false, em(c->de3_1a, c->e3_1a, B2));
@@ -160,11 +159,9 @@
       RUN(head_bwd("depth_decoder2.prdct.3", "depth_decoder2.prdct.1", c->dq, c->v2, c->dv2, H2, W2, e)); }
     CV("depth_decoder2.dec1.3", true, CONV_S1, c->dz4, Nn, Nn, H2, W2, false, em(c->du2, c->u2, B2));
     { E e = em(c->ds1_2, c->s1_2, B2); e.sum = c->dz3; e.add1 = c->up3_t; e.add1_nb = Nn;
-      CV("depth_decoder2.dec1.1", true, CONV_S2, c->du2, Nn, Nn, H2, W2, false, e); }
-    CV("depth_decoder2.dec2.3", true, CONV_S1, c->dz3, Nn, Nn, H4, W4, false, em(c->dt2, c->t2, B2));
+      RUN(conv32_pair(c, s, true, "depth_decoder2.dec1.1", c->du2, Nn, Nn, H2, W2, e, "depth_decoder2.dec2.3", Nn, em(c->dt2, c->t2, B2))); }
     { E e; e.sum = c->dz2; e.mask = c->z2; e.mask_nb = B2; e.add1 = c->dz2_up; e.add1_nb = Nn;
-      CV("depth_decoder2.dec2.1", true, CONV_S2, c->dt2, Nn, Nn, H4, W4, false, e); }
-    CV("depth_encoder2.enc2.3", true, CONV_S1, c->dz2, Nn, Nn, H8, W8, false, em(c->de2_2a, c->e2_2a, B2));
+      RUN(conv32_pair(c, s, true, "depth_decoder2.dec2.1", c->dt2, Nn, Nn, H4, W4, e, "depth_encoder2.enc2.3", Nn, em(c->de2_2a, c->e2_2a, B2))); }
     { E e; e.sum = c->de2_1; e.mask = c->e2_1; e.mask_nb = B2; e.add1 = c->ds1_2; e.add1_nb = Nn;
       CV("depth_encoder2.enc2.1", true, CONV_T2, c->de2_2a, Nn, Nn, H8, W8, false, e); }
     CV("depth_encoder2.enc1.3", true, CONV_S1, c->de2_1, Nn, Nn, H4, W4, false, em(c->de2_1a, c->e2_1a, B2));
diff --git a/tta-depth-completion_amd/csrc/msgchn_ctx.h b/tta-depth-completion_amd/csrc/msgchn_ctx.h
--- a/tta-depth-completion_amd/csrc/msgchn_ctx.h
+++ b/tta-depth-completion_amd/csrc/msgchn_ctx.h
@@ -117,6 +117,8 @@
     hipEvent_t ev_loss = nullptr;
     hipEvent_t ev_dpart = nullptr;
     int fuse_first = 1, fuse_head_bwd = 1;
+    int pair_fuse = 1;
+    int pair_fuse_count = 0;
     int cos_grad_fused = 1;
     bool cos_in_gemm = false;
     void* w0frag = nullptr; float *hm_part = nullptr, *headP = nullptr; double* head_k12 = nullptr;
@@ -282,6 +284,8 @@
 int conv_out1_p(ptta_ctx* c, const ConvOut1Args& a, hipStream_t s);
 int conv32(ptta_ctx* c, hipStream_t s, const std::string& layer, bool bwd, int mode, const void* in, int in_nb,
            int B, int Hin, int Win, bool relu, const E& e);
+int conv32_pair(ptta_ctx* c, hipStream_t s, bool bwd, const std::string& first, const void* in, int in_nb, int B, int Hin, int Win, const E& fe,
+                const std::string& second, int mid_nb, const E& se);
 int conv32w(ptta_ctx* c, hipStream_t s, const ConvW* w, const float* bias, const void* in, int in_nb, int B, int H, int W, const E& e);
 int conv32_first_bwd(ptta_ctx* c, hipStream_t s, const std::string& layer, ConvInArgs& f, int B, int H, int W, const E& e);
 int to_narrow(ptta_ctx* c, const void* src_f32, void* dst, long n, hipStream_t s);
diff --git a/tta-depth-completion_amd/csrc/msgchn_forward.hip b/tta-depth-completion_amd/csrc/msgchn_forward.hip
--- a/tta-depth-completion_amd/csrc/msgchn_forward.hip
+++ b/tta-depth-completion_amd/csrc/msgchn_forward.hip
@@ -20,18 +20,16 @@
     return ptta_launch_conv_out1(a, s);
 }
 
-int conv32(ptta_ctx* c, hipStream_t s, const std::string& layer, bool bwd, int mode, const void* in, int in_nb,
-           int B, int Hin, int Win, bool relu, const E& e) {
+static int conv32_args(ptta_ctx* c, Conv32Args& a, const std::string& layer, bool bwd, int mode, const void* in, int in_nb,
+                       int B, int Hin, int Win, bool relu, const E& e) {
     auto it = c->l32.find(layer);
     if (it == c->l32.end()) return c->fail("unknown 32->32 layer " + layer, -2);
-    Conv32Args a;
     a.in = in; a.in_nb = in_nb; a.w = bwd ? &it->second.b : &it->second.f;
     a.bias = bwd ? nullptr : (layer == "conv1_rgb_meta" ? c->meta_b : it->second.bias);
     a.up = e.up; a.up_nb = e.up_nb; a.mask = e.mask; a.mask_nb = e.mask_nb;
     a.add1 = e.add1; a.add1_nb = e.add1_nb; a.add2 = e.add2; a.add2_nb = e.add2_nb;
     a.out_raw = e.raw; a.out_sum = e.sum;
     const bool nar = e.nar || (bwd && c->nar_bwd);
-    const int es_l = nar ? 2 : c->es;
     a.B = B; a.Hin = Hin; a.Win = Win; a.mode = mode; a.relu_in = relu ? 1 : 0; a.bf16 = nar ? 1 : c->bf16; a.naive = c->naive; a.x3 = c->x3;
     a.w2 = (bwd && c->nar_bwd && c->bwd_w2) ? 1 : 0;
     if (!c->mbits.empty()) {
@@ -42,6 +40,22 @@
             if (bs || br) { a.bits_out = bs ? bs : br; a.bits_sum = bs ? 1 : 0; a.bits_nb = c->Nn; }
         }
     }
+    return 0;
+}
+
+static void conv32_cost(int mode, int B, int Hin, int Win, int es_l, double& bytes, double& macs) {
+    const long pin = (long)B * Hin * Win;
+    const long pout = mode == CONV_S1 ? pin : (mode == CONV_S2 ? pin / 4 : pin * 4);
+    bytes = (double)((pin + pout) * 32 + 9216) * es_l;
+    macs = (double)(mode == CONV_T2 ? pin : pout) * 9.0 * 32.0 * 32.0;
+}
+
+int conv32(ptta_ctx* c, hipStream_t s, const std::string& layer, bool bwd, int mode, const void* in, int in_nb,
+           int B, int Hin, int Win, bool relu, const E& e) {
+    Conv32Args a;
+    { const int rc = conv32_args(c, a, layer, bwd, mode, in, in_nb, B, Hin, Win, relu, e); if (rc) return rc; }
+    const bool nar = e.nar || (bwd && c->nar_bwd);
+    const int es_l = nar ? 2 : c->es;
     const long pin = (long)B * Hin * Win;
     const long pout = mode == CONV_S1 ? pin : (mode == CONV_S2 ? pin / 4 : pin * 4);
     const bool small = (long)Hin * Win <= (long)c->H4 * c->W4 * (mode == CONV_S2 ? 4 : 1);
@@ -51,6 +65,31 @@
     ProfScope ps(c, (mode == CONV_S1 ? (relu ? 0 : 2) : 4) + (small ? 1 : 0), s, (double)((pin + pout) * 32 + 9216) * es_l,
                  (double)(mode == CONV_T2 ? pin : pout) * 9.0 * 32.0 * 32.0, 1);
     return ptta_launch_conv32(a, s);
+}
+
+int conv32_pair(ptta_ctx* c, hipStream_t s, bool bwd, const std::string& first, const void* in, int in_nb, int B, int Hin, int Win, const E& fe,
+                const std::string& second, int mid_nb, const E& se) {
+    const int Hm = Hin / 2, Wm = Win / 2;
+    const bool relu = !bwd;
+    void* const mid = fe.sum ? fe.sum : fe.raw;
+    const bool nar = fe.nar || (bwd && c->nar_bwd);
+    if (c->pair_fuse && !c->naive && (c->x3 || c->bf16 || nar) && fe.nar == se.nar && mid) {
+        Conv32Args f, g;
+        { const int rc = conv32_args(c, f, first, bwd, CONV_S2, in, in_nb, B, Hin, Win, relu, fe); if (rc) return rc; }
+        { const int rc = conv32_args(c, g, second, bwd, CONV_S1, mid, mid_nb, B, Hm, Wm, relu, se); if (rc) return rc; }
+        if (mid_nb == B && ptta_conv32_pair_applies(f, g)) {
+            const int es_l = nar ? 2 : c->es;
+            double b1, m1, b2, m2;
+            conv32_cost(CONV_S2, B, Hin, Win, es_l, b1, m1); conv32_cost(CONV_S1, B, Hm, Wm, es_l, b2, m2);
+            ProfScope ps(c, 5, s, b1 + b2, m1 + m2, 1);
+            const int rc = ptta_launch_conv32_pair(f, g, s);
+            if (rc == 1) return c->fail("conv32_pair: fused form refused a case its own test accepted", -22);
+            if (rc == 0) c->pair_fuse_count++;
+            return rc;
+        }
+    }
+    { const int rc = conv32(c, s, first, bwd, CONV_S2, in, in_nb, B, Hin, Win, relu, fe); if (rc) return rc; }
+    return conv32(c, s, second, bwd, CONV_S1, mid, mid_nb, B, Hm, Wm, relu, se);
 }
 
 int conv32w(ptta_ctx* c, hipStream_t s, const ConvW* w, const float* bias, const void* in, int in_nb, int B, int H, int W, const E& e) {
@@ -347,11 +386,10 @@
             E e; e.nar = nar; e.raw = A(c->e2_0, H2, W2); e.up = A(c->y4, H4, W4); e.up_nb = Bl;
             RUN(conv32_first(c, st, "depth_encoder2.init.2", a, (b0 == 0 && !nar) ? Nn : 0, Bl, H2, W2, e));
         }
-        CR("depth_encoder2.enc1.1", false, CONV_S2, A(c->e2_0, H2, W2), Bl, Bl, H2, W2, true, raw(A(c->e2_1a, H4, W4)));
-        { E e; e.nar = nar; e.raw = A(c->e2_1, H4, W4); e.up = A(c->y3, H8, W8); e.up_nb = Bl; CR("depth_encoder2.enc1.3", false, CONV_S1, A(c->e2_1a, H4, W4), Bl, Bl, H4, W4, true, e); }
-        CR("depth_encoder2.enc2.1", false, CONV_S2, A(c->e2_1, H4, W4), Bl, Bl, H4, W4, true, raw(A(c->e2_2a, H8, W8)));
+        { E e; e.nar = nar; e.raw = A(c->e2_1, H4, W4); e.up = A(c->y3, H8, W8); e.up_nb = Bl;
+          RUN(conv32_pair(c, st, false, "depth_encoder2.enc1.1", A(c->e2_0, H2, W2), Bl, Bl, H2, W2, raw(A(c->e2_1a, H4, W4)), "depth_encoder2.enc1.3", Bl, e)); }
         { E e; e.nar = nar; e.sum = A(c->z2, H8, W8); e.up = A(c->y2, H16, W16); e.up_nb = Bl; e.add1 = A(c->c3, H8, W8); e.add1_nb = Bl;
-          CR("depth_encoder2.enc2.3", false, CONV_S1, A(c->e2_2a, H8, W8), Bl, Bl, H8, W8, true, e); }
+          RUN(conv32_pair(c, st, false, "depth_encoder2.enc2.1", A(c->e2_1, H4, W4), Bl, Bl, H4, W4, raw(A(c->e2_2a, H8, W8)), "depth_encoder2.enc2.3", Bl, e)); }
         CR("depth_decoder2.dec2.1", false, CONV_T2, A(c->z2, H8, W8), Bl, Bl, H8, W8, true, raw(A(c->t2, H4, W4)));
         { E e; e.nar = nar; e.raw = A(c->z3, H4, W4); e.sum = A(c->s1_2, H4, W4); e.add1 = A(c->e2_1, H4, W4); e.add1_nb = Bl; e.add2 = A(c->m, H4, W4); e.add2_nb = Bl;
           CR("depth_decoder2.dec2.3", false, CONV_S1, A(c->t2, H4, W4), Bl, Bl, H4, W4, true, e); }
@@ -378,10 +416,9 @@
         }
         CR("depth_encoder3.enc1.1", false, CONV_S2, A(c->e3_0, H1, W1), Bl, Bl, H1, W1, true, raw(A(c->e3_1a, H2, W2)));
         { E e; e.nar = nar; e.raw = A(c->e3_1, H2, W2); e.up = A(c->z3, H4, W4); e.up_nb = Bl; CR("depth_encoder3.enc1.3", false, CONV_S1, A(c->e3_1a, H2, W2), Bl, Bl, H2, W2, true, e); }
-        CR("depth_encoder3.enc2.1", false, CONV_S2, A(c->e3_1, H2, W2), Bl, Bl, H2, W2, true, raw(A(c->e3_2a, H4, W4)));
         { E e; e.nar = nar; e.raw = A(c->feat, H4, W4); e.up = A(c->z2, H8, W8); e.up_nb = Bl; e.add1 = A(c->m, H4, W4); e.add1_nb = Bl;
           if (!nar) e.sum = A(c->w2, H4, W4); else e.add1 = nullptr;
-          CR("depth_encoder3.enc2.3", false, CONV_S1, A(c->e3_2a, H4, W4), Bl, Bl, H4, W4, true, e); }
+          RUN(conv32_pair(c, st, false, "depth_encoder3.enc2.1", A(c->e3_1, H2, W2), Bl, Bl, H2, W2, raw(A(c->e3_2a, H4, W4)), "depth_encoder3.enc2.3", Bl, e)); }
 #undef CR
         return 0;
     };
diff --git a/tta-depth-completion_amd/csrc/msgchn_step.hip b/tta-depth-completion_amd/csrc/msgchn_step.hip
--- a/tta-depth-completion_amd/csrc/msgchn_step.hip
+++ b/tta-depth-completion_amd/csrc/msgchn_step.hip
@@ -148,6 +148,7 @@
 }
 static int step_body(ptta_handle c, const float* image, const float* loss_image, const float* sparse, const float* validity,
                      ptta_stream s_) {
+    c->pair_fuse_count = 0;
     RUN(ensure_fused_heads(c, (hipStream_t)s_));
     c->thru_active = thru_ok(c, (hipStream_t)s_);
     c->cnt_sparse = c->thru_active ? sparse : nullptr; c->cnt_validity = validity;
diff --git a/tta-depth-completion_amd/csrc/ptta_api.hip b/tta-depth-completion_amd/csrc/ptta_api.hip
--- a/tta-depth-completion_amd/csrc/ptta_api.hip
+++ b/tta-depth-completion_amd/csrc/ptta_api.hip
@@ -408,7 +408,7 @@
     {"fuse_first", &ptta_ctx::fuse_first, 2, false},    {"fuse_head_bwd", &ptta_ctx::fuse_head_bwd, 1, false},
     {"fuse_heads", &ptta_ctx::fuse_heads, 1, false},    {"heads_v2", &ptta_ctx::heads_v2, 1, false},
     {"cos_in_gemm", &ptta_ctx::cos_grad_fused, 1, false}, {"mask_bits", &ptta_ctx::mask_bits_on, 1, false},
-    {"stamps", &ptta_ctx::stamps, 1, true},
+    {"stamps", &ptta_ctx::stamps, 1, true},             {"pair_fuse", &ptta_ctx::pair_fuse, 1, true},
 };
 static const Option* find_option(const std::string& k) {
     for (const Option& o : kOptions) if (k == o.key) return &o;
@@ -435,6 +435,7 @@
         return 0;
     }
     if (c->nl) return -38;
+    if (k == "pair_fuse_count") return c->fail("ptta_set_option: 'pair_fuse_count' is read-only", -22);
     const Option* o = find_option(k);
     if (!o) return c->fail("ptta_set_option: unknown key '" + k + "'", -22);
     int* f = &(c->*(o->member));
@@ -462,6 +463,7 @@
     }
     if (c->nl) { if (k != "graph") return -38; *value = c->nl->use_graph; return 0; }
     if (k == "graph") { *value = c->use_graph; return 0; }
+    if (k == "pair_fuse_count") { *value = c->pair_fuse_count; return 0; }
     const Option* o = find_option(k);
     if (!o) return -22;
     *value = c->*(o->member);
diff --git a/tta-depth-completion_amd/csrc/ptta_common.h b/tta-depth-completion_amd/csrc/ptta_common.h
--- a/tta-depth-completion_amd/csrc/ptta_common.h
+++ b/tta-depth-completion_amd/csrc/ptta_common.h
@@ -395,4 +395,70 @@
     asm volatile("" ::: "memory");
 }
 
+template <typename T>
+struct Conv32P {
+    const T* in; int in_nb;
+    const void* wpack;
+    const void* wpack2;
+    Epi<T> epi;
+    int B, Hin, Win, Hout, Wout;
+};
+
+__device__ __forceinline__ float4 relu4(float4 v) {
+    v.x = fmaxf(v.x, 0.f); v.y = fmaxf(v.y, 0.f); v.z = fmaxf(v.z, 0.f); v.w = fmaxf(v.w, 0.f);
+    return v;
+}
+#define X3_TH 8
+#define X3_PW 34
+#define X3_PH 10
+
+typedef __bf16 bf16x2_t __attribute__((ext_vector_type(2)));
+typedef float float2_t __attribute__((ext_vector_type(2)));
+typedef short short2_t __attribute__((ext_vector_type(2)));
+
+__device__ __forceinline__ void split2(float a, float b, unsigned& hi, unsigned& lo) {
+    float2_t v = {a, b};
+    const bf16x2_t h = __builtin_convertvector(v, bf16x2_t);
+    hi = __builtin_bit_cast(unsigned, h);
+    float2_t r = {a - __uint_as_float(hi << 16), b - __uint_as_float(hi & 0xffff0000u)};
+    lo = __builtin_bit_cast(unsigned, __builtin_convertvector(r, bf16x2_t));
+}
+__device__ __forceinline__ unsigned relu_pk(unsigned v) {
+    const short2_t z = {0, 0};
+    return __builtin_bit_cast(unsigned, __builtin_elementwise_max(__builtin_bit_cast(short2_t, v), z));
+}
+
+template <typename T> struct Px;
+template <> struct Px<float> { float4 a, b; };
+template <> struct Px<bf16_t> { uint4 a; };
+template <typename T> __device__ __forceinline__ Px<T> px_zero();
+template <> __device__ __forceinline__ Px<float> px_zero<float>() { Px<float> r; r.a = make_float4(0.f, 0.f, 0.f, 0.f); r.b = r.a; return r; }
+template <> __device__ __forceinline__ Px<bf16_t> px_zero<bf16_t>() { Px<bf16_t> r; r.a = make_uint4(0u, 0u, 0u, 0u); return r; }
+__device__ __forceinline__ Px<float> px_load(const float* src) { Px<float> r; r.a = *(const float4*)src; r.b = *(const float4*)(src + 4); return r; }
+__device__ __forceinline__ Px<bf16_t> px_load(const bf16_t* src) { Px<bf16_t> r; r.a = *(const uint4*)src; return r; }
+template <bool RELU>
+__device__ __forceinline__ void px_stage(const Px<float>& v, unsigned char* dst, int lo_off) {
+    float4 a0 = v.a, a1 = v.b;
+#ifdef X3_TIMING_NOSPLIT
+    *(float4*)dst = a0; *(float4*)(dst + lo_off) = a1; return;
+#endif
+    if (RELU) { a0 = relu4(a0); a1 = relu4(a1); }
+    uint4 hi, lo;
+    split2(a0.x, a0.y, hi.x, lo.x); split2(a0.z, a0.w, hi.y, lo.y);
+    split2(a1.x, a1.y, hi.z, lo.z); split2(a1.z, a1.w, hi.w, lo.w);
+    *(uint4*)dst = hi;
+    *(uint4*)(dst + lo_off) = lo;
+}
+template <bool RELU>
+__device__ __forceinline__ void px_stage(const Px<bf16_t>& v, unsigned char* dst, int) {
+    uint4 hi = v.a;
+    if (RELU) { hi.x = relu_pk(hi.x); hi.y = relu_pk(hi.y); hi.z = relu_pk(hi.z); hi.w = relu_pk(hi.w); }
+    *(uint4*)dst = hi;
+}
+template <typename T> struct Geo;
+template <> struct Geo<float> { static constexpr int STR = 144, LO = 64, WL = 18 * 64 * 16, UPPX = 128, UPPC = 8; };
+template <> struct Geo<bf16_t> { static constexpr int STR = 80, LO = 0, WL = 0, UPPX = 64, UPPC = 4; };
+
+__device__ __forceinline__ int x3_stage_pix(int idx) { return ((idx >> 5) << 3) + (((idx >> 2) & 1) << 2) + ((idx >> 3) & 3); }
+
 #define PTTA_CHECK_LAUNCH() do { hipError_t e_ = hipGetLastError(); if (e_ != hipSuccess) return (int)e_; } while (0)
diff --git a/tta-depth-completion_amd/csrc/ptta_kernels.h b/tta-depth-completion_amd/csrc/ptta_kernels.h
--- a/tta-depth-completion_amd/csrc/ptta_kernels.h
+++ b/tta-depth-completion_amd/csrc/ptta_kernels.h
@@ -37,6 +37,8 @@
 };
 void ptta_pack_conv32(const float* src, const ConvW& w, int in_major, int flip, hipStream_t s, int row_stride = 32, int col_off = 0);
 int ptta_launch_conv32(const Conv32Args& a, hipStream_t s);
+bool ptta_conv32_pair_applies(const Conv32Args& first, const Conv32Args& second);
+int ptta_launch_conv32_pair(const Conv32Args& first, const Conv32Args& second, hipStream_t s);
 int ptta_launch_conv32_loop(const Conv32Args& a, void* buf_a, void* buf_b, int reps, unsigned* ctr, unsigned* base_io, int* err, int variant, hipStream_t s);
 
 struct Plane { const float* p = nullptr; int nb = 1; long bstride = 0;
diff --git a/tta-depth-completion_amd/csrc/ptta_ops.hip b/tta-depth-completion_amd/csrc/ptta_ops.hip
--- a/tta-depth-completion_amd/csrc/ptta_ops.hip
+++ b/tta-depth-completion_amd/csrc/ptta_ops.hip
@@ -94,6 +94,67 @@
         (void)hipStreamSynchronize(s);
     }
     (void)hipFree(tin); (void)hipFree(tout);
+    return rc;
+}
+
+int ptta_op_conv32_pair(const float* in, const float* weight1, const float* bias1, const float* weight2, const float* bias2, const float* up,
+                        const float* add0, const float* add1, const float* add2, const uint32_t* mask1_bits, const uint32_t* mask2_bits,
+                        float* out_raw, float* out_sum, float* mid_raw, float* mid_sum, uint32_t* mid_bits, int b, int in_nb,
+                        int hin, int win, int first_mode, int relu1, int relu2, int in_major, int flip, int dtype, int w2, int fused,
+                        int* fused_host, ptta_stream s_) {
+    hipStream_t s = (hipStream_t)s_;
+    if (!in || !weight1 || !weight2 || (!out_raw && !out_sum) || b < 1 || in_nb < 1 || in_nb > b || hin < 1 || win < 1 ||
+        (first_mode != CONV_S2 && first_mode != CONV_T2) || (add2 && !add1) || (add1 && !out_sum)) return -22;
+    const bool nar = dtype != PTTA_DTYPE_F32;
+    if (w2 && (!nar || relu1 || relu2 || up)) return -22;
+    const int hm = first_mode == CONV_S2 ? hin / 2 : hin * 2, wm = first_mode == CONV_S2 ? win / 2 : win * 2;
+    if (hm < 1 || wm < 1) return -22;
+    const long nin = (long)in_nb * hin * win * 32, nm = (long)b * hm * wm * 32, nu = (long)b * (hm / 2) * (wm / 2) * 32;
+    ScratchConvW sw1, sw2;
+    void* t[9] = {nullptr, nullptr, nullptr, nullptr, nullptr, nullptr, nullptr, nullptr, nullptr};
+    const long cnt[9] = {nin, up ? nu : 0, add0 ? nm : 0, add1 ? nm : 0, add2 ? nm : 0, nm, add0 ? nm : 0, out_raw ? nm : 0, out_sum ? nm : 0};
+    const float* src[5] = {in, up, add0, add1, add2};
+    const int es = nar ? 2 : 4;
+    int rc = (sw1.ok && sw2.ok) ? 0 : -12;
+    for (int k = 0; k < 9 && !rc; ++k) if (cnt[k] > 0 && hipMalloc(&t[k], (size_t)cnt[k] * es) != hipSuccess) rc = -12;
+    if (!rc) {
+        ptta_pack_conv32(weight1, sw1.w, in_major, flip, s);
+        ptta_pack_conv32(weight2, sw2.w, 0, 0, s);
+        for (int k = 0; k < 5; ++k) {
+            if (cnt[k] <= 0) continue;
+            if (nar) from_f32_launch(src[k], (bf16_t*)t[k], cnt[k], s);
+            else if (hipMemcpyAsync(t[k], src[k], (size_t)cnt[k] * 4, hipMemcpyDeviceToDevice, s) != hipSuccess) rc = -5;
+        }
+        (void)hipMemsetAsync(t[5], 0xff, (size_t)nm * es, s);
+        if (t[6]) (void)hipMemsetAsync(t[6], 0xff, (size_t)nm * es, s);
+    }
+    if (!rc) {
+        Conv32Args f, g;
+        f.in = t[0]; f.in_nb = in_nb; f.w = &sw1.w; f.bias = bias1; f.out_raw = t[5]; f.B = b; f.Hin = hin; f.Win = win; f.mode = first_mode;
+        f.relu_in = relu1; f.bf16 = nar ? 1 : 0; f.x3 = 1; f.w2 = w2;
+        if (add0) { f.add1 = t[2]; f.add1_nb = b; f.out_sum = t[6]; }
+        if (mask1_bits) { f.mask = mask1_bits; f.mask_nb = b; f.mask_bits = mask1_bits; }
+        if (!nar && mid_bits) { f.bits_out = mid_bits; f.bits_nb = b; }
+        g.in = add0 ? t[6] : t[5]; g.in_nb = b; g.w = &sw2.w; g.bias = bias2; g.up = t[1]; g.up_nb = b;
+        g.add1 = t[3]; g.add1_nb = b; g.add2 = t[4]; g.add2_nb = b;
+        if (mask2_bits) { g.mask = mask2_bits; g.mask_nb = b; g.mask_bits = mask2_bits; }
+        g.out_raw = t[7]; g.out_sum = t[8]; g.B = b; g.Hin = hm; g.Win = wm; g.mode = CONV_S1; g.relu_in = relu2; g.bf16 = nar ? 1 : 0; g.x3 = 1; g.w2 = w2;
+        int did = 0;
+        rc = fused ? ptta_launch_conv32_pair(f, g, s) : 1;
+        if (rc == 0) did = 1;
+        if (rc == 1) { rc = ptta_launch_conv32(f, s); if (!rc) rc = ptta_launch_conv32(g, s); }
+        if (fused_host) *fused_host = did;
+    }
+    if (!rc) {
+        float* dst[4] = {mid_raw, mid_sum, out_raw, out_sum};
+        for (int k = 0; k < 4; ++k) {
+            if (!dst[k] || !t[5 + k]) continue;
+            if (nar) to_f32_launch((const bf16_t*)t[5 + k], dst[k], nm, s);
+            else if (hipMemcpyAsync(dst[k], t[5 + k], (size_t)nm * 4, hipMemcpyDeviceToDevice, s) != hipSuccess) rc = -5;
+        }
+    }
+    if (hipStreamSynchronize(s) != hipSuccess && !rc) rc = -5;
+    for (int k = 0; k < 9; ++k) (void)hipFree(t[k]);
     return rc;
 }
 
diff --git a/tta-depth-completion_amd/proxytta/_lib.py b/tta-depth-completion_amd/proxytta/_lib.py
--- a/tta-depth-completion_amd/proxytta/_lib.py
+++ b/tta-depth-completion_amd/proxytta/_lib.py
@@ -120,6 +120,7 @@
     ('ptta_debug_tensor', c_int, [_P, c_char_p, _P, c_int64, POINTER(c_int64), _P]),
     ('ptta_op_conv32', c_int, [_P, _P, _P, _P, c_int, c_int, c_int, c_int, c_int, c_int, c_int, c_int, c_int, _P]),
     ('ptta_op_conv32_chain', c_int, [_P] * 6 + [c_int] * 7 + [POINTER(c_float), _P]),
+    ('ptta_op_conv32_pair', c_int, [_P] * 16 + [c_int] * 12 + [POINTER(c_int), _P]),
     ('ptta_op_gwgrad', c_int, [_P, _P, _P, _P] + [c_int] * 7 + [POINTER(c_float), _P]),
     ('ptta_op_gconv', c_int, [_P, c_int, c_int, _P, c_int, c_int, _P, _P, _P] + [c_int] * 16 + [POINTER(ctypes.c_double), POINTER(c_int), _P]),
     ('ptta_op_gconv_affine', c_int, [_P, c_int, c_int, _P, c_int, c_int, _P, _P, _P] + [c_int] * 16 + [POINTER(ctypes.c_double), POINTER(c_int),
```

After: 844.1, median of 6. 2.1% higher.
